# qcraftai/pillarnext

Hardware: AMD Instinct MI355X
Metric: frames/s PillarNeXt-B nuScenes 300k-pt cloud (inference, end-to-end) (higher is better)
Workload: dtype bf16

## Files before the change

include/pnx.h:

```cpp
#ifndef PNX_H
#define PNX_H

#include <stddef.h>
#include <stdint.h>

#ifdef __cplusplus
extern "C" {
#endif

typedef void* pnx_stream_t;

typedef enum pnx_status {
  PNX_OK = 0,
  PNX_ERR_INVALID = -1,
  PNX_ERR_UNSUPPORTED = -2,
  PNX_ERR_WORKSPACE = -3,
  PNX_ERR_HIP = -4
} pnx_status;

typedef enum pnx_dtype { PNX_F32 = 0, PNX_BF16 = 1, PNX_F16 = 2 } pnx_dtype;
typedef enum pnx_layout {
  PNX_NHWC = 0,
  PNX_NCHW = 1
} pnx_layout;

typedef struct pnx_geom {
  float pc_min[3];
  float voxel[3];
  int32_t gx, gy;
} pnx_geom;

const char* pnx_last_error(void);
const char* pnx_version(void);

int pnx_geom_init(const double* pc_range6_host, const double* voxel_size3_host, pnx_geom* geom_host);

#define PNX_PFN_FOLDED_FLOATS(F) (32 * ((F) + 5) + 32 + 64 * 64 + 64 + 64 * 121 + 64 * 71)

int pnx_pfn_fold_bn(int32_t num_point_features,
                    const float* w0, const float* gamma0, const float* beta0, const float* mean0, const float* var0,
                    const float* w1, const float* gamma1, const float* beta1, const float* mean1, const float* var1,
                    float eps, float* folded_out, pnx_stream_t stream);

size_t pnx_reader_workspace_bytes(int64_t n_points, int32_t batch, const pnx_geom* geom_host);

int pnx_reader_forward(const float* points, int64_t n_points, int32_t row_stride, int32_t batch, const pnx_geom* geom_host,
                       const float* pfn_folded, void* canvas, int32_t canvas_dtype, int32_t canvas_layout, uint8_t* occupancy,
                       float* feat_max, int32_t* coords, int64_t pillar_capacity, int64_t* unq_inv, int32_t* pillar_of_point,
                       int32_t* counts, void* workspace, size_t workspace_bytes, pnx_stream_t stream);

void pnx_reader_fill_split(int32_t* percent3_host);

int pnx_profile_begin(int32_t max_samples);
int pnx_profile_end(float* reader_us_avg_host, float* canvas_us_avg_host, int32_t* samples_host);
float pnx_profile_last_pfn_us(void);
float pnx_profile_last_voxelize_us(void);

size_t pnx_pfn_train_param_floats(int32_t num_point_features);
size_t pnx_pfn_train_partial_floats(int32_t num_point_features, int32_t which);
int pnx_pfn_forward_train(int32_t pass, const float* points, int64_t n_points, int32_t row_stride, int32_t batch, const pnx_geom* geom_host,
                          const float* params, float* partials, float* feat_max, int64_t pillar_capacity, int32_t* coords,
                          int32_t* pillar_of_point, int32_t* counts, void* workspace, size_t workspace_bytes, pnx_stream_t stream);
int pnx_pfn_backward(int32_t pass, int64_t n_points, int32_t row_stride, int32_t batch, const pnx_geom* geom_host, const float* params,
                     const float* grad_feat_max, const float* feat_max, float* partials, void* workspace, size_t workspace_bytes,
                     pnx_stream_t stream);

int pnx_voxelize(const float* points, int64_t n_points, int32_t row_stride, int32_t batch, const pnx_geom* geom_host,
                 float* features, int32_t* coords, int64_t pillar_capacity, int64_t* unq_inv, int32_t* pillar_of_point,
                 int32_t* counts, void* workspace, size_t workspace_bytes, pnx_stream_t stream);

typedef enum pnx_group_mode { PNX_GROUP_VOXEL = 0, PNX_GROUP_PILLAR_CLAMP = 1, PNX_GROUP_CYLINDER_CLAMP = 2 } pnx_group_mode;
typedef struct pnx_group_geom {
  float min[3], voxel[3];
  int32_t grid[3];
  int32_t mode;
  int32_t prefilter;
  float keep_min[3], keep_max[3];
} pnx_group_geom;
size_t pnx_group_workspace_bytes(int64_t n_points, int32_t row_stride, int32_t batch, const pnx_group_geom* geom_host);
int pnx_group_points(const float* points, int64_t n_points, int32_t row_stride, int32_t batch, const pnx_group_geom* geom_host, float* point_features,
                     int32_t feature_ld, int32_t* coords, int64_t group_capacity, int64_t* unq_inv, float* group_mean, int32_t* counts, void* workspace,
                     size_t workspace_bytes, pnx_stream_t stream);
int pnx_pfn_layer_eval(const float* xa, int32_t lda, int32_t ca, const float* gb, int32_t cb, const int64_t* inv, const float* wt, const float* shift,
                       int32_t cout, int64_t n, int64_t num_groups, float* y, int32_t ldy, float* gmax, pnx_stream_t stream);
int pnx_bilinear_gather(const void* image, int32_t dtype, int32_t batch, int32_t h, int32_t w, int32_t channels, const float* pos, int32_t pos_ld,
                        const float* pos_min2_host, const float* pos_voxel2_host, const int32_t* cell_coords, const int64_t* unq_inv, int32_t ds_rate,
                        int64_t n, float* out, int32_t out_ld, pnx_stream_t stream);
size_t pnx_bilinear_gather_backward_workspace_bytes(int64_t n, int32_t batch, int32_t h, int32_t w);
int pnx_bilinear_gather_backward(const float* grad_out, int32_t grad_ld, int32_t batch, int32_t h, int32_t w, int32_t channels, const float* pos,
                                 int32_t pos_ld, const float* pos_min2_host, const float* pos_voxel2_host, const int32_t* cell_coords,
                                 const int64_t* unq_inv, int32_t ds_rate, int64_t n, float* grad_image, void* workspace, size_t workspace_bytes,
                                 pnx_stream_t stream);

size_t pnx_scatter_max_workspace_bytes(int64_t n, int64_t num_pillars);
int pnx_scatter_max(const float* x, const int64_t* index, int64_t n, int32_t channels, int64_t num_pillars, float* out,
                    int64_t* argmax, void* workspace, size_t workspace_bytes, pnx_stream_t stream);
int pnx_scatter_max_backward(const float* grad_out, const int64_t* argmax, int64_t n, int32_t channels, int64_t num_pillars,
                             float* grad_x, pnx_stream_t stream);

size_t pnx_point_layer_workspace_bytes(int64_t n, int32_t cin, int32_t cout, int32_t backward);
int pnx_point_layer_stats(const float* x, int32_t ldx, int64_t n, int32_t cin, const float* w, int32_t cout, double* sums, void* workspace,
                          size_t workspace_bytes, pnx_stream_t stream);
int pnx_point_layer_forward(const float* x, int32_t ldx, int64_t n, int32_t cin, const float* w, int32_t cout, const float* prm, const int64_t* inv,
                            int64_t num_groups, float* y, int32_t ldy, float* gmax, int64_t* argmax, pnx_stream_t stream);
int pnx_point_layer_backward_stats(const float* x, int32_t ldx, int64_t n, int32_t cin, const float* w, int32_t cout, const float* prm, const float* dy,
                                   int32_t lddy, const int64_t* inv, int64_t num_groups, const float* dgmax, const int64_t* argmax, double* sums,
                                   void* workspace, size_t workspace_bytes, pnx_stream_t stream);
int pnx_point_layer_backward(const float* x, int32_t ldx, int64_t n, int32_t cin, const float* w, int32_t cout, const float* prm, const float* dy,
                             int32_t lddy, const int64_t* inv, int64_t num_groups, const float* dgmax, const int64_t* argmax, float* dx, int32_t lddx,
                             float* dw, void* workspace, size_t workspace_bytes, pnx_stream_t stream);

int pnx_scatter_canvas(const float* feat_max, const int32_t* coords, const int32_t* num_pillars_dev, int64_t pillar_capacity,
                       int32_t batch, int32_t gy, int32_t gx, void* canvas, int32_t canvas_dtype, int32_t canvas_layout,
                       pnx_stream_t stream);

size_t pnx_merge_sweeps_desc_bytes(void);
size_t pnx_merge_sweeps_workspace_bytes(int64_t n_raw);
int pnx_merge_sweeps(const float* raw, int64_t n_raw, int32_t raw_stride, int32_t n_copy, const void* seg_descs_dev, int32_t n_segments, float* out,
                     int32_t* n_out_dev, void* workspace, size_t workspace_bytes, pnx_stream_t stream);

int pnx_bias_act_mask(const void* x, const void* residual, const float* bias, const uint8_t* mask, void* out, int64_t sites,
                      int32_t channels, int32_t dtype, int32_t relu, pnx_stream_t stream);
int pnx_sum_bias_act(const void* const* srcs, int32_t n_src, const float* bias, void* out, int64_t sites, int32_t channels, int32_t dtype,
                     int32_t relu, pnx_stream_t stream);
int pnx_deconv2x2_bf16(const void* x, const void* wfrag, const float* bias, void* y, int32_t batch, int32_t h, int32_t w, int32_t cin, int32_t cout,
                       int32_t relu, pnx_stream_t stream);
int pnx_deconv2x2_f16(const void* x, const void* wfrag, const float* bias, void* y, int32_t batch, int32_t h, int32_t w, int32_t cin, int32_t cout,
                       int32_t relu, pnx_stream_t stream);
int pnx_conv3x3_bf16(const void* x, const void* wfrag, const float* bias, const void* residual, const uint8_t* mask, void* y, int32_t batch,
                     int32_t h, int32_t w, int32_t cin, int32_t cout, int32_t stride, int32_t relu, uint8_t* row_dirty, const int32_t* tile_list,
                     const int32_t* tile_count, pnx_stream_t stream);
int pnx_conv3x3_f16(const void* x, const void* wfrag, const float* bias, const void* residual, const uint8_t* mask, void* y, int32_t batch,
                    int32_t h, int32_t w, int32_t cin, int32_t cout, int32_t stride, int32_t relu, uint8_t* row_dirty, const int32_t* tile_list,
                    const int32_t* tile_count, pnx_stream_t stream);
size_t pnx_conv3x3_wgrad_workspace_bytes(int32_t cin, int32_t cout);
int pnx_conv3x3_wgrad_bf16(const void* x, const void* dy, const uint8_t* mask, float* dw, int32_t batch, int32_t h, int32_t w, int32_t cin, int32_t cout,
                           int32_t stride, void* workspace, size_t workspace_bytes, pnx_stream_t stream);
int pnx_conv3x3_wgrad_x3(const void* x_hi, const void* x_lo, const void* dy_hi, const void* dy_lo, const uint8_t* mask, float* dw, int32_t batch, int32_t h,
                         int32_t w, int32_t cin, int32_t cout, int32_t stride, void* workspace, size_t workspace_bytes, pnx_stream_t stream);
int pnx_conv3x3_wgrad_x6(const void* x_hi, const void* x_mid, const void* x_lo, const void* dy_hi, const void* dy_mid, const void* dy_lo, const uint8_t* mask,
                         float* dw, int32_t batch, int32_t h, int32_t w, int32_t cin, int32_t cout, int32_t stride, void* workspace, size_t workspace_bytes,
                         pnx_stream_t stream);
int pnx_conv3x3_pack_weights(const void* w, int32_t dtype, int32_t cout, int32_t cin, int32_t transposed, void* wfrag, pnx_stream_t stream);
int pnx_conv3x3_tile_rows(int32_t cin, int32_t cout, int32_t stride);
int pnx_conv_tile_list(const uint8_t* mask, const uint8_t* const* row_dirty, int32_t n_dirty, int32_t batch, int32_t h, int32_t w, int32_t tile_rows,
                       int32_t* tile_list, int32_t* tile_count, pnx_stream_t stream);
int pnx_sephead_out_bf16(const void* x, const void* wfrag, const float* bias, void* y, int32_t batch, int32_t h, int32_t w, int32_t n_branch,
                         pnx_stream_t stream);
int pnx_sephead_out_f16(const void* x, const void* wfrag, const float* bias, void* y, int32_t batch, int32_t h, int32_t w, int32_t n_branch,
                         pnx_stream_t stream);
typedef struct {
  const void* up;
  const void* wfrag1;
  const float* bias1;
  const float* w2c;
  const float* bias2;
  int32_t h, w;
} PnxLazyTask;
int pnx_sephead_lazy_bf16(const PnxLazyTask* tasks, int32_t n_tasks, const int32_t* class_task, int32_t nc_total, int32_t batch, const int64_t* local,
                          const int32_t* seg_len, int32_t pre_max, float* out, pnx_stream_t stream);
int pnx_sephead_lazy_f16(const PnxLazyTask* tasks, int32_t n_tasks, const int32_t* class_task, int32_t nc_total, int32_t batch, const int64_t* local,
                          const int32_t* seg_len, int32_t pre_max, float* out, pnx_stream_t stream);
int pnx_split_f32(const float* x, void* hi, void* lo, int64_t n, const uint8_t* mask, int32_t channels, pnx_stream_t stream);
int pnx_conv3x3_x3(const void* x_hi, const void* x_lo, const void* wfrag_hi, const void* wfrag_lo, const float* bias, const uint8_t* mask, float* y,
                   int32_t batch, int32_t h, int32_t w, int32_t cin, int32_t cout, int32_t stride, pnx_stream_t stream);
int pnx_split3_f32(const float* x, void* hi, void* mid, void* lo, int64_t n, const uint8_t* mask, int32_t channels, pnx_stream_t stream);
int pnx_conv3x3_x6(const void* x_hi, const void* x_mid, const void* x_lo, const void* wfrag_hi, const void* wfrag_mid, const void* wfrag_lo, const float* bias,
                   const uint8_t* mask, float* y, int32_t batch, int32_t h, int32_t w, int32_t cin, int32_t cout, int32_t stride, pnx_stream_t stream);
int pnx_conv3x3_dgrad_s2_bf16(const void* g, const void* wfrag_t, const uint8_t* mask_in, void* dx, int32_t batch, int32_t h, int32_t w, int32_t cin,
                              int32_t cout, pnx_stream_t stream);
int pnx_conv3x3_dgrad_s2_x3(const void* g_hi, const void* g_lo, const void* wfrag_t_hi, const void* wfrag_t_lo, const uint8_t* mask_in, float* dx, int32_t batch,
                            int32_t h, int32_t w, int32_t cin, int32_t cout, pnx_stream_t stream);
int pnx_conv3x3_dgrad_s2_x6(const void* g_hi, const void* g_mid, const void* g_lo, const void* wfrag_t_hi, const void* wfrag_t_mid, const void* wfrag_t_lo,
                            const uint8_t* mask_in, float* dx, int32_t batch, int32_t h, int32_t w, int32_t cin, int32_t cout, pnx_stream_t stream);
int pnx_conv3x3_smallk(const void* x, const float* weight, const float* bias, void* y, int32_t batch, int32_t h, int32_t w, int32_t cin, int32_t k,
                       int32_t dtype, pnx_stream_t stream);
size_t pnx_conv3x3_smallk_wgrad_workspace_bytes(int32_t k);
int pnx_conv3x3_smallk_wgrad(const void* x, const void* dy, float* dw, float* dbias, int32_t batch, int32_t h, int32_t w, int32_t cin, int32_t k,
                             int32_t dtype, void* workspace, size_t workspace_bytes, pnx_stream_t stream);
int pnx_mask_pool3(const uint8_t* mask_in, int32_t batch, int32_t h, int32_t w, int32_t stride, uint8_t* mask_out, pnx_stream_t stream);

int pnx_boxes_overlap_bev(const float* boxes_a, int64_t n, const float* boxes_b, int64_t m, float* out, pnx_stream_t stream);
int pnx_boxes_iou_bev(const float* boxes_a, int64_t n, const float* boxes_b, int64_t m, float* out, pnx_stream_t stream);
int pnx_boxes_aligned_overlap_bev(const float* boxes_a, const float* boxes_b, int64_t n, float* out, pnx_stream_t stream);
int pnx_boxes_aligned_iou3d(const float* boxes_a, const float* boxes_b, int64_t n, float* out, pnx_stream_t stream);

int pnx_boxes_iou_bev_cpu(const float* boxes_a_host, int64_t n, const float* boxes_b_host, int64_t m, float* out_host);
int pnx_boxes_aligned_iou_bev_cpu(const float* boxes_a_host, const float* boxes_b_host, int64_t n, float* out_host);
size_t pnx_nms_workspace_bytes(int64_t total_boxes, int32_t num_segments, int32_t max_seg_len);
int32_t pnx_debug_nms_pair_cap(int32_t cap);
int pnx_debug_detmath(const float* a, const float* b, int64_t n, float* sin_a, float* cos_a, float* atan2_ab, int32_t on_device, pnx_stream_t stream);
int pnx_nms_rotated_batched(const float* boxes, const int32_t* seg_offsets, const int32_t* seg_len, int32_t num_segments, int32_t max_seg_len,
                            const float* thresh, int32_t post_max, int32_t* keep, int32_t* keep_count, void* workspace,
                            size_t workspace_bytes, pnx_stream_t stream);
int pnx_nms_normal_batched(const float* boxes, const int32_t* seg_offsets, const int32_t* seg_len, int32_t num_segments, int32_t max_seg_len,
                           const float* thresh, int32_t post_max, int32_t* keep, int32_t* keep_count, void* workspace,
                           size_t workspace_bytes, pnx_stream_t stream);

size_t pnx_decode_task_desc_bytes(void);
size_t pnx_decode_topk_workspace_bytes(int64_t n_keys, int32_t num_segments);
int pnx_decode_topk(const uint64_t* keys, int64_t n_keys, int32_t num_segments, int32_t pre_max, uint64_t* sorted_keys, int64_t* order,
                    int64_t* seg_start, int32_t* seg_len, int32_t* seg_total, void* workspace, size_t workspace_bytes, pnx_stream_t stream);
int pnx_decode_keys(const void* packed, int32_t dtype, int32_t batch, int32_t n_classes_total, const void* task_desc_host, uint64_t* keys,
                    pnx_stream_t stream);
size_t pnx_sort_keys_workspace_bytes(int64_t n_keys);
int pnx_sort_keys(const uint64_t* keys, int64_t n_keys, int32_t num_segments, uint64_t* sorted_keys, int64_t* order, void* workspace,
                  size_t workspace_bytes, pnx_stream_t stream);
int pnx_decode_boxes(const void* const* task_ptrs_dev, const void* task_descs_dev, const int64_t* task_key_off_dev, int32_t n_tasks,
                     int32_t dtype, int32_t batch, const uint64_t* sorted_keys, const int64_t* order, const int64_t* seg_start,
                     const int32_t* seg_len, int32_t num_segments, int32_t pre_max, float* boxes9, float* boxes7, float* scores,
                     pnx_stream_t stream);
int pnx_decode_boxes_lazy(const void* task_descs_dev, const int64_t* task_key_off_dev, int32_t n_tasks, int32_t n_classes_total,
                          const uint64_t* sorted_keys, const int64_t* order, const int64_t* seg_start, int32_t* seg_len, const int32_t* seg_total,
                          int32_t num_segments, int32_t pre_max, const float* cand, float* boxes9, float* boxes7, float* scores, int32_t* flag_dev,
                          pnx_stream_t stream);
int pnx_gather_kept(const float* boxes9, const float* scores, const int32_t* keep, const int32_t* keep_count, int32_t num_segments,
                    int32_t pre_max, int32_t post_max, float* out, pnx_stream_t stream);

int32_t pnx_masked_bn_blocks(void);
int pnx_masked_bn_reduce(const float* partials, int32_t rows, int32_t cols, double* sums, pnx_stream_t stream);
int pnx_masked_bn_finalize(const double* sums, int32_t channels, const float* center, const float* weight, const float* bias, double eps, double momentum,
                           float* running_mean, float* running_var, int64_t* num_batches_tracked, float* mean, float* invstd, float* scale, float* shift,
                           float* count, pnx_stream_t stream);
int pnx_masked_bn_bwd_finalize(const double* sums_local, const double* sums_global, int32_t channels, const float* count, float* dgamma, float* dbeta,
                               float* mean_g, float* mean_gx, pnx_stream_t stream);
int pnx_masked_bn_stats(const void* x, int32_t dtype, const float* mask, int64_t n_sites, int32_t channels, const float* center, float* partials,
                        pnx_stream_t stream);
int pnx_masked_bn_apply(const void* x, const void* residual, int32_t dtype, const float* mask, int64_t n_sites, int32_t channels, const float* scale,
                        const float* shift, int32_t relu, void* y, pnx_stream_t stream);
int pnx_masked_bn_bwd_stats(const void* gy, const void* x, const void* residual, int32_t dtype, const float* mask, int64_t n_sites, int32_t channels,
                            const float* scale, const float* shift, const float* mean, const float* invstd, int32_t relu, float* partials,
                            pnx_stream_t stream);
int pnx_masked_bn_bwd_apply(const void* gy, const void* x, const void* residual, int32_t dtype, const float* mask, int64_t n_sites, int32_t channels,
                            const float* scale, const float* shift, const float* mean, const float* invstd, int32_t relu, const float* mean_g,
                            const float* mean_gx, void* dx, void* dresidual, pnx_stream_t stream);

size_t pnx_center_loss_workspace_bytes(int32_t batch, int32_t max_objs);
int pnx_center_loss_forward(const void* const* maps7, const float* hm_target, const int64_t* ind, const uint8_t* mask, const int64_t* cat,
                            const float* anno_box, const float* gt_boxes, int32_t batch, int32_t n_classes, int32_t h, int32_t w, int32_t max_objs,
                            const float* geom4_host, int32_t with_reg_iou, float* losses15, void* workspace, size_t workspace_bytes,
                            pnx_stream_t stream);
int pnx_center_loss_backward(const void* const* maps7, void* const* grads7, const float* hm_target, const int64_t* ind, const uint8_t* mask,
                             const int64_t* cat, const float* anno_box, const float* gt_boxes, int32_t batch, int32_t n_classes, int32_t h, int32_t w,
                             int32_t max_objs, const float* geom4_host, int32_t with_reg_iou, const float* losses15, const float* upstream13,
                             float* coef_scratch, void* workspace, size_t workspace_bytes, pnx_stream_t stream);

#define PNX_ASSIGN_MAX_TASKS 8
#define PNX_ASSIGN_MAX_CLASSES 32
typedef struct pnx_assign_desc {
  double lo[2];
  double voxel[2];
  double overlap;
  int32_t min_radius, max_objs, n_tasks, n_classes;
  int32_t osf[PNX_ASSIGN_MAX_TASKS], h[PNX_ASSIGN_MAX_TASKS], w[PNX_ASSIGN_MAX_TASKS], ncls[PNX_ASSIGN_MAX_TASKS];
  int32_t class_task[PNX_ASSIGN_MAX_CLASSES], class_cls[PNX_ASSIGN_MAX_CLASSES];
} pnx_assign_desc;
size_t pnx_assign_workspace_bytes(int32_t batch, int32_t n_tasks, int32_t max_objs);
int pnx_assign_labels(const float* gt_boxes, const int32_t* gt_cls, const int32_t* num_gt, int32_t batch, int32_t k, const pnx_assign_desc* desc_host,
                      float* const* hm_host, float* const* anno_box_host, int64_t* const* ind_host, uint8_t* const* mask_host, int64_t* const* cat_host,
                      float* const* gt_boxes_out_host, int32_t* counts, void* workspace, size_t workspace_bytes, pnx_stream_t stream);

enum { PNX_OP_MASK_POOL3 = 1, PNX_OP_TILE_LIST = 2, PNX_OP_CONV3X3 = 3, PNX_OP_DECONV2X2 = 4, PNX_OP_SEPHEAD_OUT = 5 };
typedef struct pnx_op {
  int32_t kind;
  int32_t i[9];
  const void* p[11];
} pnx_op;
int pnx_enqueue(const pnx_op* ops_host, int32_t n_ops, pnx_stream_t stream);
size_t pnx_op_bytes(void);

typedef struct pnx_lazy_decode {
  int32_t n_tasks, n_classes_total, batch, pre_max, post_max, dtype;
  const void* const* dense_host;
  const void* task_descs_host;
  const void* task_descs_dev;
  const int64_t* task_key_off_host;
  const int64_t* task_key_off_dev;
  const int64_t* list_key_off_dev;
  const PnxLazyTask* lazy_tasks_host;
  const int32_t* class_task_host;
  const int32_t* seg_off_dev;
// ... 89 lines not shown
```

pillarnext_amd/_lib.py:

```python
import ctypes
import os

_HERE = os.path.dirname(os.path.abspath(__file__))
LIB_PATH = os.environ.get("PNX_LIB") or os.path.join(_HERE, "libpnx_hip.so")

PNX_F32, PNX_BF16, PNX_F16 = 0, 1, 2
PNX_NHWC, PNX_NCHW = 0, 1


class PnxError(RuntimeError):
    pass


class PnxGeom(ctypes.Structure):
    _fields_ = [("pc_min", ctypes.c_float * 3), ("voxel", ctypes.c_float * 3), ("gx", ctypes.c_int32), ("gy", ctypes.c_int32)]


PNX_GROUP_VOXEL, PNX_GROUP_PILLAR_CLAMP, PNX_GROUP_CYLINDER_CLAMP = 0, 1, 2


class PnxGroupGeom(ctypes.Structure):
    _fields_ = [("min", ctypes.c_float * 3), ("voxel", ctypes.c_float * 3), ("grid", ctypes.c_int32 * 3), ("mode", ctypes.c_int32),
                ("prefilter", ctypes.c_int32), ("keep_min", ctypes.c_float * 3), ("keep_max", ctypes.c_float * 3)]


PNX_ASSIGN_MAX_TASKS, PNX_ASSIGN_MAX_CLASSES = 8, 32
PNX_PASTE_MAX_BOXES, PNX_PASTE_MAX_BATCH = 512, 64
PNX_AUG_ROTATE, PNX_AUG_SCALE, PNX_AUG_TRANSLATE, PNX_AUG_FLIP_X, PNX_AUG_FLIP_Y = 1, 2, 4, 8, 16


class PnxAssignDesc(ctypes.Structure):
    _fields_ = [("lo", ctypes.c_double * 2), ("voxel", ctypes.c_double * 2), ("overlap", ctypes.c_double), ("min_radius", ctypes.c_int32),
                ("max_objs", ctypes.c_int32), ("n_tasks", ctypes.c_int32), ("n_classes", ctypes.c_int32)] + \
               [(k, ctypes.c_int32 * PNX_ASSIGN_MAX_TASKS) for k in ("osf", "h", "w", "ncls")] + \
               [(k, ctypes.c_int32 * PNX_ASSIGN_MAX_CLASSES) for k in ("class_task", "class_cls")]


_vp = ctypes.c_void_p
_i64 = ctypes.c_int64
_i32 = ctypes.c_int32
_f32 = ctypes.c_float
_sz = ctypes.c_size_t
_i3p = ctypes.POINTER(ctypes.c_int32)

PROTOTYPES = {
    "pnx_last_error": (ctypes.c_char_p, []),
    "pnx_version": (ctypes.c_char_p, []),
    "pnx_geom_init": (ctypes.c_int, [ctypes.POINTER(ctypes.c_double), ctypes.POINTER(ctypes.c_double), ctypes.POINTER(PnxGeom)]),
    "pnx_pfn_fold_bn": (ctypes.c_int, [_i32] + [_vp] * 10 + [_f32, _vp, _vp]),
    "pnx_reader_workspace_bytes": (_sz, [_i64, _i32, ctypes.POINTER(PnxGeom)]),
    "pnx_reader_forward": (ctypes.c_int, [_vp, _i64, _i32, _i32, ctypes.POINTER(PnxGeom), _vp, _vp, _i32, _i32, _vp, _vp, _vp, _i64, _vp, _vp,
                                          _vp, _vp, _sz, _vp]),
    "pnx_reader_fill_split": (None, [ctypes.POINTER(ctypes.c_int32)]),
    "pnx_profile_begin": (ctypes.c_int, [_i32]),
    "pnx_profile_end": (ctypes.c_int, [ctypes.POINTER(ctypes.c_float), ctypes.POINTER(ctypes.c_float), ctypes.POINTER(ctypes.c_int32)]),
    "pnx_profile_last_pfn_us": (ctypes.c_float, []),
    "pnx_profile_last_voxelize_us": (ctypes.c_float, []),
    "pnx_pfn_train_param_floats": (_sz, [_i32]),
    "pnx_pfn_train_partial_floats": (_sz, [_i32, _i32]),
    "pnx_pfn_forward_train": (ctypes.c_int, [_i32, _vp, _i64, _i32, _i32, ctypes.POINTER(PnxGeom), _vp, _vp, _vp, _i64, _vp, _vp, _vp, _vp, _sz, _vp]),
    "pnx_pfn_backward": (ctypes.c_int, [_i32, _i64, _i32, _i32, ctypes.POINTER(PnxGeom), _vp, _vp, _vp, _vp, _vp, _sz, _vp]),
    "pnx_voxelize": (ctypes.c_int, [_vp, _i64, _i32, _i32, ctypes.POINTER(PnxGeom), _vp, _vp, _i64, _vp, _vp, _vp, _vp, _sz, _vp]),
    "pnx_group_workspace_bytes": (_sz, [_i64, _i32, _i32, ctypes.POINTER(PnxGroupGeom)]),
    "pnx_group_points": (ctypes.c_int, [_vp, _i64, _i32, _i32, ctypes.POINTER(PnxGroupGeom), _vp, _i32, _vp, _i64, _vp, _vp, _vp, _vp, _sz, _vp]),
    "pnx_pfn_layer_eval": (ctypes.c_int, [_vp, _i32, _i32, _vp, _i32, _vp, _vp, _vp, _i32, _i64, _i64, _vp, _i32, _vp, _vp]),
    "pnx_bilinear_gather": (ctypes.c_int, [_vp, _i32, _i32, _i32, _i32, _i32, _vp, _i32, ctypes.POINTER(ctypes.c_float), ctypes.POINTER(ctypes.c_float), _vp,
                                           _vp, _i32, _i64, _vp, _i32, _vp]),
    "pnx_bilinear_gather_backward_workspace_bytes": (_sz, [_i64, _i32, _i32, _i32]),
    "pnx_bilinear_gather_backward": (ctypes.c_int, [_vp, _i32, _i32, _i32, _i32, _i32, _vp, _i32, ctypes.POINTER(ctypes.c_float),
                                                    ctypes.POINTER(ctypes.c_float), _vp, _vp, _i32, _i64, _vp, _vp, _sz, _vp]),
    "pnx_scatter_max_workspace_bytes": (_sz, [_i64, _i64]),
    "pnx_scatter_max": (ctypes.c_int, [_vp, _vp, _i64, _i32, _i64, _vp, _vp, _vp, _sz, _vp]),
    "pnx_scatter_max_backward": (ctypes.c_int, [_vp, _vp, _i64, _i32, _i64, _vp, _vp]),
    "pnx_point_layer_workspace_bytes": (_sz, [_i64, _i32, _i32, _i32]),
    "pnx_point_layer_stats": (ctypes.c_int, [_vp, _i32, _i64, _i32, _vp, _i32, _vp, _vp, _sz, _vp]),
    "pnx_point_layer_forward": (ctypes.c_int, [_vp, _i32, _i64, _i32, _vp, _i32, _vp, _vp, _i64, _vp, _i32, _vp, _vp, _vp]),
    "pnx_point_layer_backward_stats": (ctypes.c_int, [_vp, _i32, _i64, _i32, _vp, _i32, _vp, _vp, _i32, _vp, _i64, _vp, _vp, _vp, _vp, _sz, _vp]),
    "pnx_point_layer_backward": (ctypes.c_int, [_vp, _i32, _i64, _i32, _vp, _i32, _vp, _vp, _i32, _vp, _i64, _vp, _vp, _vp, _i32, _vp, _vp, _sz, _vp]),
    "pnx_scatter_canvas": (ctypes.c_int, [_vp, _vp, _vp, _i64, _i32, _i32, _i32, _vp, _i32, _i32, _vp]),
    "pnx_merge_sweeps_desc_bytes": (_sz, []),
    "pnx_merge_sweeps_workspace_bytes": (_sz, [_i64]),
    "pnx_merge_sweeps": (ctypes.c_int, [_vp, _i64, _i32, _i32, _vp, _i32, _vp, _vp, _vp, _sz, _vp]),
    "pnx_bias_act_mask": (ctypes.c_int, [_vp, _vp, _vp, _vp, _vp, _i64, _i32, _i32, _i32, _vp]),
    "pnx_sum_bias_act": (ctypes.c_int, [_vp, _i32, _vp, _vp, _i64, _i32, _i32, _i32, _vp]),
    "pnx_deconv2x2_bf16": (ctypes.c_int, [_vp, _vp, _vp, _vp, _i32, _i32, _i32, _i32, _i32, _i32, _vp]),
    "pnx_deconv2x2_f16": (ctypes.c_int, [_vp, _vp, _vp, _vp, _i32, _i32, _i32, _i32, _i32, _i32, _vp]),
    "pnx_sephead_out_bf16": (ctypes.c_int, [_vp, _vp, _vp, _vp, _i32, _i32, _i32, _i32, _vp]),
    "pnx_sephead_out_f16": (ctypes.c_int, [_vp, _vp, _vp, _vp, _i32, _i32, _i32, _i32, _vp]),
    "pnx_masked_bn_blocks": (_i32, []),
    "pnx_masked_bn_reduce": (ctypes.c_int, [_vp, _i32, _i32, _vp, _vp]),
    "pnx_masked_bn_finalize": (ctypes.c_int, [_vp, _i32, _vp, _vp, _vp, ctypes.c_double, ctypes.c_double, _vp, _vp, _vp, _vp, _vp, _vp, _vp, _vp, _vp]),
    "pnx_masked_bn_bwd_finalize": (ctypes.c_int, [_vp, _vp, _i32, _vp, _vp, _vp, _vp, _vp, _vp]),
    "pnx_masked_bn_stats": (ctypes.c_int, [_vp, _i32, _vp, _i64, _i32, _vp, _vp, _vp]),
    "pnx_masked_bn_apply": (ctypes.c_int, [_vp, _vp, _i32, _vp, _i64, _i32, _vp, _vp, _i32, _vp, _vp]),
    "pnx_masked_bn_bwd_stats": (ctypes.c_int, [_vp, _vp, _vp, _i32, _vp, _i64, _i32, _vp, _vp, _vp, _vp, _i32, _vp, _vp]),
    "pnx_masked_bn_bwd_apply": (ctypes.c_int, [_vp, _vp, _vp, _i32, _vp, _i64, _i32, _vp, _vp, _vp, _vp, _i32, _vp, _vp, _vp, _vp, _vp]),
    "pnx_sephead_lazy_bf16": (ctypes.c_int, [_vp, _i32, _vp, _i32, _i32, _vp, _vp, _i32, _vp, _vp]),
    "pnx_sephead_lazy_f16": (ctypes.c_int, [_vp, _i32, _vp, _i32, _i32, _vp, _vp, _i32, _vp, _vp]),
    "pnx_conv3x3_bf16": (ctypes.c_int, [_vp, _vp, _vp, _vp, _vp, _vp, _i32, _i32, _i32, _i32, _i32, _i32, _i32, _vp, _vp, _vp, _vp]),
    "pnx_conv3x3_f16": (ctypes.c_int, [_vp, _vp, _vp, _vp, _vp, _vp, _i32, _i32, _i32, _i32, _i32, _i32, _i32, _vp, _vp, _vp, _vp]),
    "pnx_conv3x3_tile_rows": (ctypes.c_int, [_i32, _i32, _i32]),
    "pnx_conv3x3_pack_weights": (ctypes.c_int, [_vp, _i32, _i32, _i32, _i32, _vp, _vp]),
    "pnx_conv3x3_wgrad_workspace_bytes": (_sz, [_i32, _i32]),
    "pnx_conv3x3_wgrad_bf16": (ctypes.c_int, [_vp, _vp, _vp, _vp, _i32, _i32, _i32, _i32, _i32, _i32, _vp, _sz, _vp]),
    "pnx_conv3x3_wgrad_x3": (ctypes.c_int, [_vp, _vp, _vp, _vp, _vp, _vp, _i32, _i32, _i32, _i32, _i32, _i32, _vp, _sz, _vp]),
    "pnx_conv3x3_wgrad_x6": (ctypes.c_int, [_vp, _vp, _vp, _vp, _vp, _vp, _vp, _vp, _i32, _i32, _i32, _i32, _i32, _i32, _vp, _sz, _vp]),
    "pnx_conv3x3_dgrad_s2_bf16": (ctypes.c_int, [_vp, _vp, _vp, _vp, _i32, _i32, _i32, _i32, _i32, _vp]),
    "pnx_conv3x3_dgrad_s2_x3": (ctypes.c_int, [_vp, _vp, _vp, _vp, _vp, _vp, _i32, _i32, _i32, _i32, _i32, _vp]),
    "pnx_conv3x3_dgrad_s2_x6": (ctypes.c_int, [_vp, _vp, _vp, _vp, _vp, _vp, _vp, _vp, _i32, _i32, _i32, _i32, _i32, _vp]),
    "pnx_conv3x3_smallk": (ctypes.c_int, [_vp, _vp, _vp, _vp, _i32, _i32, _i32, _i32, _i32, _i32, _vp]),
    "pnx_conv3x3_smallk_wgrad_workspace_bytes": (_sz, [_i32]),
    "pnx_conv3x3_smallk_wgrad": (ctypes.c_int, [_vp, _vp, _vp, _vp, _i32, _i32, _i32, _i32, _i32, _i32, _vp, _sz, _vp]),
    "pnx_conv_tile_list": (ctypes.c_int, [_vp, _vp, _i32, _i32, _i32, _i32, _i32, _vp, _vp, _vp]),
    "pnx_mask_pool3": (ctypes.c_int, [_vp, _i32, _i32, _i32, _i32, _vp, _vp]),
    "pnx_split_f32": (ctypes.c_int, [_vp, _vp, _vp, _i64, _vp, _i32, _vp]),
    "pnx_conv3x3_x3": (ctypes.c_int, [_vp, _vp, _vp, _vp, _vp, _vp, _vp, _i32, _i32, _i32, _i32, _i32, _i32, _vp]),
    "pnx_split3_f32": (ctypes.c_int, [_vp, _vp, _vp, _vp, _i64, _vp, _i32, _vp]),
    "pnx_conv3x3_x6": (ctypes.c_int, [_vp, _vp, _vp, _vp, _vp, _vp, _vp, _vp, _vp, _i32, _i32, _i32, _i32, _i32, _i32, _vp]),
    "pnx_decode_task_desc_bytes": (_sz, []),
    "pnx_decode_topk_workspace_bytes": (_sz, [_i64, _i32]),
    "pnx_decode_topk": (ctypes.c_int, [_vp, _i64, _i32, _i32, _vp, _vp, _vp, _vp, _vp, _vp, _sz, _vp]),
    "pnx_decode_keys": (ctypes.c_int, [_vp, _i32, _i32, _i32, _vp, _vp, _vp]),
    "pnx_sort_keys_workspace_bytes": (ctypes.c_size_t, [_i64]),
    "pnx_sort_keys": (ctypes.c_int, [_vp, _i64, _i32, _vp, _vp, _vp, ctypes.c_size_t, _vp]),
    "pnx_decode_boxes": (ctypes.c_int, [_vp, _vp, _vp, _i32, _i32, _i32, _vp, _vp, _vp, _vp, _i32, _i32, _vp, _vp, _vp, _vp]),
    "pnx_decode_boxes_lazy": (ctypes.c_int, [_vp, _vp, _i32, _i32, _vp, _vp, _vp, _vp, _vp, _i32, _i32, _vp, _vp, _vp, _vp, _vp, _vp]),
    "pnx_gather_kept": (ctypes.c_int, [_vp, _vp, _vp, _vp, _i32, _i32, _i32, _vp, _vp]),
    "pnx_enqueue": (ctypes.c_int, [_vp, _i32, _vp]),
    "pnx_decode_lazy_enqueue": (ctypes.c_int, [_vp, _vp]),
    "pnx_op_bytes": (_sz, []),
    "pnx_lazy_decode_bytes": (_sz, []),
    "pnx_center_loss_workspace_bytes": (_sz, [_i32, _i32]),
    "pnx_center_loss_forward": (ctypes.c_int, [_vp, _vp, _vp, _vp, _vp, _vp, _vp, _i32, _i32, _i32, _i32, _i32, _vp, _i32, _vp, _vp, _sz, _vp]),
    "pnx_center_loss_backward": (ctypes.c_int, [_vp, _vp, _vp, _vp, _vp, _vp, _vp, _vp, _i32, _i32, _i32, _i32, _i32, _vp, _i32, _vp, _vp, _vp, _vp, _sz, _vp]),
    "pnx_assign_workspace_bytes": (_sz, [_i32, _i32, _i32]),
    "pnx_assign_labels": (ctypes.c_int, [_vp, _vp, _vp, _i32, _i32, ctypes.POINTER(PnxAssignDesc), _vp, _vp, _vp, _vp, _vp, _vp, _vp, _vp, _sz, _vp]),
    "pnx_paste_chunk_rows": (_i32, []),
    "pnx_paste_select": (ctypes.c_int, [_vp, _vp, _vp, _i32, _i32, _i32, _vp, _vp, _vp, _vp, _i32, _i32, _vp, _i32, _vp, _vp, _vp, _vp, _vp, _vp, _vp]),
    "pnx_paste_augment_workspace_bytes": (_sz, [_i64, _i32]),
    "pnx_paste_augment_points": (ctypes.c_int, [_vp, _i64, _i32, _i32, _vp, _vp, _vp, _vp, _i32, _i32, _vp, _vp, _i32, _i64, _vp, _vp, _i64, _vp, _vp, _vp,
                                                _sz, _vp]),
    "pnx_augment_boxes": (ctypes.c_int, [_vp, _vp, _i32, _i32, _i32, _vp, _vp]),
    "pnx_boxes_overlap_bev": (ctypes.c_int, [_vp, _i64, _vp, _i64, _vp, _vp]),
    "pnx_boxes_iou_bev": (ctypes.c_int, [_vp, _i64, _vp, _i64, _vp, _vp]),
    "pnx_boxes_aligned_overlap_bev": (ctypes.c_int, [_vp, _vp, _i64, _vp, _vp]),
    "pnx_boxes_aligned_iou3d": (ctypes.c_int, [_vp, _vp, _i64, _vp, _vp]),
    "pnx_boxes_iou_bev_cpu": (ctypes.c_int, [_vp, _i64, _vp, _i64, _vp]),
    "pnx_boxes_aligned_iou_bev_cpu": (ctypes.c_int, [_vp, _vp, _i64, _vp]),
    "pnx_nms_workspace_bytes": (_sz, [_i64, _i32, _i32]),
    "pnx_debug_nms_pair_cap": (_i32, [_i32]),
    "pnx_debug_detmath": (ctypes.c_int, [_vp, _vp, _i64, _vp, _vp, _vp, _i32, _vp]),
    "pnx_nms_rotated_batched": (ctypes.c_int, [_vp, _vp, _vp, _i32, _i32, _vp, _i32, _vp, _vp, _vp, _sz, _vp]),
    "pnx_nms_normal_batched": (ctypes.c_int, [_vp, _vp, _vp, _i32, _i32, _vp, _i32, _vp, _vp, _vp, _sz, _vp]),
    "pnx_sp3_index_bytes": (_sz, [_i32, _i3p]),
    "pnx_sp3_index_build": (ctypes.c_int, [_vp, _i64, _i32, _i3p, _vp, _sz, _vp, _vp, _vp]),
    "pnx_sp3_out_grid": (ctypes.c_int, [_i32, _i3p, _i3p, _i3p, _i3p, _i3p]),
    "pnx_sp3_out_index": (ctypes.c_int, [_vp, _i64, _i32, _i3p, _i3p, _i3p, _i3p, _vp, _sz, _vp, _vp]),
    "pnx_sp3_index_coords": (ctypes.c_int, [_vp, _sz, _i32, _i3p, _vp, _i64, _vp]),
    "pnx_sp3_neighbor_map": (ctypes.c_int, [_vp, _i64, _vp, _sz, _i32, _i3p, _vp, _i3p, _i3p, _i3p, _vp, _vp]),
    "pnx_sp3_packed_weight_floats": (_sz, [_i32, _i32, _i32]),
    "pnx_sp3_conv": (ctypes.c_int, [_vp, _i64, _i32, _vp, _i64, _i32, _vp, _vp, _vp, _i32, _vp, _i32, _vp]),
    "pnx_sp3_conv_train": (ctypes.c_int, [_vp, _i64, _i32, _vp, _i64, _i32, _vp, _vp, _vp, _i32, _vp, _i32, _vp]),
    "pnx_sp3_dense": (ctypes.c_int, [_vp, _vp, _i64, _i32, _i32, _i3p, _vp, _vp]),
    "pnx_sp3_packed_weight_halfs": (_sz, [_i32, _i32, _i32]),
    "pnx_sp3_conv_h": (ctypes.c_int, [_vp, _i64, _i32, _i32, _vp, _i64, _i32, _vp, _vp, _vp, _i32, _vp, _i32, _i32, _i32, _vp]),
    "pnx_sp3_dense_h": (ctypes.c_int, [_vp, _i32, _vp, _i64, _i32, _i32, _i32, _i3p, _vp, _vp]),
    "pnx_sp3_transpose_map": (ctypes.c_int, [_vp, _i64, _i32, _i64, _vp, _vp]),
    "pnx_sp3_wgrad_workspace_bytes": (_sz, [_i64, _i32, _i32, _i32]),
    "pnx_sp3_wgrad": (ctypes.c_int, [_vp, _i64, _i32, _vp, _i32, _vp, _i64, _i32, _vp, _vp, _sz, _vp]),
    "pnx_sp3_conv_h_f32": (ctypes.c_int, [_vp, _i64, _i32, _i32, _vp, _i64, _i32, _vp, _vp, _i32, _i32, _vp]),
    "pnx_sp3_wgrad_h_partials_bytes": (_sz, [_i64, _i32, _i32, _i32]),
    "pnx_sp3_wgrad_h": (ctypes.c_int, [_vp, _i64, _i32, _i32, _vp, _i32, _i32, _vp, _i64, _i32, _vp, _i32, _vp, _sz, _vp]),
    "pnx_sp3_dense_backward": (ctypes.c_int, [_vp, _vp, _i64, _i32, _i32, _i3p, _vp, _vp]),
    "pnx_sp3_bn_split": (ctypes.c_int, [_i64, _i32, _i3p]),
    "pnx_sp3_bn_partials_bytes": (_sz, [_i64, _i32, _i32]),
    "pnx_sp3_bn_stats": (ctypes.c_int, [_vp, _i64, _i32, _vp, _vp, _sz, _vp]),
    "pnx_sp3_bn_apply": (ctypes.c_int, [_vp, _i64, _i32, _vp, _vp, _vp, _i32, _i32, _vp, _vp, _i32, _vp]),
    "pnx_sp3_bn_bwd_stats": (ctypes.c_int, [_vp, _vp, _vp, _i32, _i64, _i32, _vp, _vp, _vp, _vp, _i32, _vp, _sz, _vp]),
    "pnx_sp3_bn_bwd_apply": (ctypes.c_int, [_vp, _vp, _vp, _i32, _i64, _i32, _vp, _vp, _vp, _vp, _i32, _vp, _vp, _vp, _vp, _vp]),
}

_LIB = None


def lib():
    global _LIB
    if _LIB is None:
        if not os.path.exists(LIB_PATH):
            raise PnxError(f"{LIB_PATH} is missing: run `python -m pillarnext_amd.build` (hipcc, gfx950). "
                           "There is no CPU fallback for the product path.")
        L = ctypes.CDLL(LIB_PATH)
        for name, (res, args) in PROTOTYPES.items():
            fn = getattr(L, name)
            fn.restype = res
            fn.argtypes = args
        _LIB = L
    return _LIB


def check(rc, what=""):
    if rc != 0:
        msg = lib().pnx_last_error().decode(errors="replace")
        raise PnxError(f"{what} failed with status {rc}: {msg}")


def make_geom(pc_range, voxel_size):
    pr = (ctypes.c_double * 6)(*[float(v) for v in pc_range])
    vs = (ctypes.c_double * 3)(*[float(v) for v in voxel_size])
    g = PnxGeom()
    check(lib().pnx_geom_init(pr, vs, ctypes.byref(g)), "pnx_geom_init")
    return g


def ptr(t):
    return None if t is None else ctypes.c_void_p(t.data_ptr())


def stream_ptr():
    import torch

    return ctypes.c_void_p(torch.cuda.current_stream().cuda_stream)
```

pillarnext_amd/csrc/conv3x3.hip:

```cpp
#include "pnx_common.h"

namespace {

#include "conv_tile.h"

template <int CIN, int COUT, int STRIDE, bool W_LDS>
__global__ __launch_bounds__(256, 2) void k_conv3x3(const uint16_t* __restrict__ x, const uint4* __restrict__ wfrag,
                                                 const float* __restrict__ bias, const uint16_t* __restrict__ res,
                                                 const uint8_t* __restrict__ mask, uint16_t* __restrict__ y, int B, int H, int W, int Ho,
                                                 int Wo, int relu, uint8_t* __restrict__ row_dirty) {
  constexpr int CB = CIN / 16, MT = COUT / 32, KSTEPS = 9 * CB;
  constexpr int NT = (MT <= 2) ? 4 : 2;
  extern __shared__ uint4 s_w[];
  const int lane = threadIdx.x & 63, wv = threadIdx.x >> 6;
  const int px = lane & 31, kb = lane >> 5;
  if (W_LDS) {
    for (int i = threadIdx.x; i < KSTEPS * MT * 64; i += 256) s_w[i] = wfrag[i];
    __syncthreads();
  }
  const int tiles_x = (Wo + 31) >> 5, tiles_y = (Ho + NT - 1) / NT;
  const int64_t n_tiles = (int64_t)B * tiles_y * tiles_x;
  for (int64_t tile = (int64_t)blockIdx.x * 4 + wv; tile < n_tiles; tile += (int64_t)gridDim.x * 4) {
    const int tx = (int)(tile % tiles_x);
    const int ty = (int)((tile / tiles_x) % tiles_y);
    const int b = (int)(tile / ((int64_t)tiles_x * tiles_y));
    const int ox = tx * 32 + px, oy0 = ty * NT;
    bool act[NT];
    bool any_row[NT];
    bool any = false;
#pragma unroll
    for (int j = 0; j < NT; j++) {
      const int oy = oy0 + j;
      const bool in = ox < Wo && oy < Ho;
      act[j] = in && (mask == nullptr || mask[((int64_t)b * Ho + oy) * Wo + ox] != 0);
      any_row[j] = __ballot(act[j]) != 0;
      any = any || any_row[j];
    }
    bool row_store[NT];
#pragma unroll
    for (int j = 0; j < NT; j++) {
      const int oy = oy0 + j;
      row_store[j] = oy < Ho;
      if (row_dirty != nullptr && oy < Ho) {
        uint8_t* d = row_dirty + ((int64_t)b * Ho + oy) * tiles_x + tx;
        const bool was = __builtin_amdgcn_readfirstlane((int)*d) != 0;
        row_store[j] = any_row[j] || was;
        if (lane == 0 && was != any_row[j]) *d = any_row[j] ? 1 : 0;
      }
    }
    v16f acc[NT][MT];
#pragma unroll
    for (int m = 0; m < MT; m++) {
      const v16f bq = bias_tile(bias, m * 32, kb);
#pragma unroll
      for (int j = 0; j < NT; j++) acc[j][m] = bq;
    }

    if (res != nullptr) {
#pragma unroll
      for (int j = 0; j < NT; j++) {
        const bool in = ox < Wo && oy0 + j < Ho;
        const uint16_t* rp = res + (in ? (((int64_t)b * Ho + oy0 + j) * Wo + ox) * COUT : 0);
#pragma unroll
        for (int m0 = 0; m0 < MT; m0 += 2) {
          uint4 rq[2][2];
          load_residual(rq, rp + m0 * 32, act[j], kb);
          v16f a2[2] = {acc[j][m0], acc[j][m0 + 1]};
          add_residual(a2, rq);
          acc[j][m0] = a2[0], acc[j][m0 + 1] = a2[1];
        }
      }
    }

    if (any) {
      for (int tap = 0; tap < 9; tap++) {
        const int dy = tap / 3 - 1, dx = tap % 3 - 1;
        const uint16_t* src[NT];
        bool ok[NT];
#pragma unroll
        for (int j = 0; j < NT; j++) {
          const int iy = (oy0 + j) * STRIDE + dy, ix = ox * STRIDE + dx;
          ok[j] = any_row[j] && ox < Wo && (oy0 + j) < Ho && iy >= 0 && iy < H && ix >= 0 && ix < W;
          src[j] = x + (((int64_t)b * H + (ok[j] ? iy : 0)) * W + (ok[j] ? ix : 0)) * CIN + 8 * kb;
        }
#pragma unroll
        for (int cb = 0; cb < CB; cb++) {
          const int ks = tap * CB + cb;
          el8 af[MT];
#pragma unroll
          for (int m = 0; m < MT; m++) {
            const uint4 wq = W_LDS ? s_w[(ks * MT + m) * 64 + lane] : wfrag[(ks * MT + m) * 64 + lane];
            af[m] = __builtin_bit_cast(el8, wq);
          }
#pragma unroll
          for (int j = 0; j < NT; j++) {
            if (!any_row[j]) continue;
            uint4 q = make_uint4(0, 0, 0, 0);
            if (ok[j]) q = *reinterpret_cast<const uint4*>(src[j] + cb * 16);
            const el8 bfr = __builtin_bit_cast(el8, q);
#pragma unroll
            for (int m = 0; m < MT; m++) acc[j][m] = PNX_MFMA32(af[m], bfr, acc[j][m]);
          }
        }
      }
    }
    const int n_valid = Wo - tx * 32;
#pragma unroll
    for (int j = 0; j < NT; j++) {
      const bool row_in = row_store[j];
      if (!row_in) continue;
      uint16_t* row = y + (((int64_t)b * Ho + (oy0 + j)) * Wo + tx * 32) * COUT;
#pragma unroll
      for (int m0 = 0; m0 < MT; m0 += 2) {
        uint4 R[4];
#pragma unroll
        for (int m = 0; m < 2; m++) {
          uint4 pk[2];
          pack_tile(acc[j][m0 + m], act[j], relu, pk);
          R[2 * m] = pk[0], R[2 * m + 1] = pk[1];
        }
        transpose_row64(R, lane);
        store_row64<COUT>(R, row + m0 * 32, row_in ? n_valid : 0, lane);
      }
    }
  }
}

#include "conv_taps.h"
#include "conv_rows.h"
#include "conv_s2.h"
#include "sephead.h"

struct DirtySet {
  const uint8_t* p[4];
};
__global__ __launch_bounds__(256) void k_tile_list(const uint8_t* __restrict__ mask, DirtySet ds, int B, int H, int W, int th, int32_t* __restrict__ list,
                                                   int32_t* __restrict__ count) {
  __shared__ int s_wave[4];
  __shared__ int s_base;
  const int t = threadIdx.x, lane = t & 63, wv = t >> 6;
  const int tiles_x = (W + 31) >> 5, tiles_y = (H + th - 1) / th;
  const int64_t n_tiles = (int64_t)B * tiles_y * tiles_x;
  const int r = lane & 15;
  const int64_t tile = ((int64_t)blockIdx.x * 4 + wv) * 4 + (lane >> 4);
  uint32_t acc = 0;
  if (tile < n_tiles && r < th) {
    const int tx = (int)(tile % tiles_x);
    const int ty = (int)((tile / tiles_x) % tiles_y);
    const int b = (int)(tile / ((int64_t)tiles_x * tiles_y));
    const int x0 = tx * 32, oy = ty * th + r;
    if (oy < H) {
      const uint8_t* row = mask + ((int64_t)b * H + oy) * W + x0;
      if ((W & 15) == 0 && x0 + 32 <= W) {
        const uint4 a = reinterpret_cast<const uint4*>(row)[0], c = reinterpret_cast<const uint4*>(row)[1];
        acc |= a.x | a.y | a.z | a.w | c.x | c.y | c.z | c.w;
      } else {
        for (int k = 0; k < 32 && x0 + k < W; k++) acc |= row[k];
      }
#pragma unroll
      for (int k = 0; k < 4; k++)
        if (ds.p[k] != nullptr) acc |= ds.p[k][((int64_t)b * H + oy) * tiles_x + tx];
    }
  }
  acc |= (uint32_t)__shfl_xor((int)acc, 1);
  acc |= (uint32_t)__shfl_xor((int)acc, 2);
  acc |= (uint32_t)__shfl_xor((int)acc, 4);
  acc |= (uint32_t)__shfl_xor((int)acc, 8);
  const bool any = acc != 0 && r == 0 && tile < n_tiles;
  const unsigned long long bal = __ballot(any);
  if (lane == 0) s_wave[wv] = __popcll(bal);
  __syncthreads();
  if (t == 0) {
    const int tot = s_wave[0] + s_wave[1] + s_wave[2] + s_wave[3];
    s_base = tot > 0 ? atomicAdd(count, tot) : 0;
  }
  __syncthreads();
  if (any) {
    int off = s_base + __popcll(bal & ((1ull << lane) - 1ull));
    for (int w = 0; w < wv; w++) off += s_wave[w];
    list[off] = (int32_t)tile;
  }
}

template <int COUT>
int launch_lds(const ConvArgs& a) {
  constexpr int TH = LDS_TH;
  const int64_t n_tiles = (int64_t)a.B * ((a.H + TH - 1) / TH) * ((a.W + 31) / 32);
  int64_t nb = n_tiles;
  const int64_t cap = 256 * 2;
  if (nb > cap) nb = cap;
  const int slot = a.mask != nullptr ? next_sched_slot() : -1;
  if constexpr (COUT == 64) {
    if (a.res != nullptr) {
      k_conv3x3_lds<COUT, true><<<(unsigned)nb, 256, 0, a.st>>>(a.x, a.wfrag, a.bias, a.res, a.mask, a.y, a.B, a.H, a.W, a.relu, a.row_dirty, slot, a.tlist,
                                                               a.tcount);
      PNX_LAUNCH_CHECK();
      return PNX_OK;
    }
  } else {
    PNX_REQUIRE(a.res == nullptr, PNX_ERR_UNSUPPORTED, "residual with %d output channels", COUT);
  }
  k_conv3x3_lds<COUT, false><<<(unsigned)nb, 256, 0, a.st>>>(a.x, a.wfrag, a.bias, nullptr, a.mask, a.y, a.B, a.H, a.W, a.relu, a.row_dirty, slot, a.tlist,
                                                            a.tcount);
  PNX_LAUNCH_CHECK();
  return PNX_OK;
}

#include "conv_pc.h"

template <int CIN, int COUT, int STRIDE>
int launch(const ConvArgs& a, int Ho, int Wo) {
  constexpr size_t wbytes = (size_t)9 * (CIN / 16) * (COUT / 32) * 64 * 16;
  constexpr bool W_LDS = wbytes <= 76 * 1024;
  constexpr int NT = (COUT / 32 <= 2) ? 4 : 2;
  const int64_t n_tiles = (int64_t)a.B * ((Ho + NT - 1) / NT) * ((Wo + 31) / 32);
  int64_t nb = (n_tiles + 3) / 4;
  if (nb > 512) nb = 512;
  constexpr auto kern = k_conv3x3<CIN, COUT, STRIDE, W_LDS>;
  if (W_LDS) {
    if (const int rc = pnx_lds_optin<kern>(wbytes); rc != PNX_OK) return rc;
  }
  kern<<<(unsigned)nb, 256, W_LDS ? wbytes : 0, a.st>>>(a.x, a.wfrag, a.bias, a.res, a.mask, a.y, a.B, a.H, a.W, Ho, Wo, a.relu, a.row_dirty);
  PNX_LAUNCH_CHECK();
  return PNX_OK;
}

}

extern "C" {

#if defined(PNX_CONV_TIMERS) && !defined(PNX_CONV_F16)
int pnx_debug_conv_timers(unsigned long long* out) {
  unsigned long long z[8] = {0, 0, 0, 0, 0, 0, 0, 0};
  PNX_CHECK_HIP(hipDeviceSynchronize());
  PNX_CHECK_HIP(hipMemcpyFromSymbol(out, HIP_SYMBOL(g_conv_T), sizeof(z)));
  PNX_CHECK_HIP(hipMemcpyToSymbol(HIP_SYMBOL(g_conv_T), z, sizeof(z)));
  return PNX_OK;
}
#endif

int PNX_CONV_FN(pnx_sephead_out)(const void* x, const void* wfrag, const float* bias, void* y, int32_t batch, int32_t h, int32_t w, int32_t n_branch,
                         pnx_stream_t stream) {
  PNX_REQUIRE(x && wfrag && bias && y && batch > 0 && h > 0 && w > 0, PNX_ERR_INVALID, "bad arguments");
  PNX_REQUIRE((((uintptr_t)x | (uintptr_t)y | (uintptr_t)wfrag | (uintptr_t)bias) & 15) == 0, PNX_ERR_INVALID, "16-byte alignment required");
  hipStream_t st = (hipStream_t)stream;
  switch (n_branch) {
    case 1: return launch_sephead<1>(x, wfrag, bias, y, batch, h, w, st);
    case 2: return launch_sephead<2>(x, wfrag, bias, y, batch, h, w, st);
    case 5: return launch_sephead<5>(x, wfrag, bias, y, batch, h, w, st);
    case 6: return launch_sephead<6>(x, wfrag, bias, y, batch, h, w, st);
    case 7: return launch_sephead<7>(x, wfrag, bias, y, batch, h, w, st);
    default: break;
  }
  pnx_set_error("pnx_sephead_out: no kernel for %d branches", n_branch);
  return PNX_ERR_UNSUPPORTED;
}

int PNX_CONV_FN(pnx_deconv2x2)(const void* x, const void* wfrag, const float* bias, void* y, int32_t batch, int32_t h, int32_t w, int32_t cin, int32_t cout,
                       int32_t relu, pnx_stream_t stream) {
  PNX_REQUIRE(x && wfrag && bias && y && batch > 0 && h > 0 && w > 0, PNX_ERR_INVALID, "bad arguments");
  PNX_REQUIRE((((uintptr_t)x | (uintptr_t)y | (uintptr_t)wfrag | (uintptr_t)bias) & 15) == 0, PNX_ERR_INVALID, "16-byte alignment required");
  if (cin != 64 || cout != 64) {
    pnx_set_error("pnx_deconv2x2: no kernel for %d -> %d channels", cin, cout);
    return PNX_ERR_UNSUPPORTED;
  }
  const int64_t n_seg = (int64_t)batch * h * ((w + 31) / 32);
  int64_t nb = (n_seg + 3) / 4;
  if (nb > 512) nb = 512;
  k_deconv2x2_64<<<(unsigned)nb, 256, 0, (hipStream_t)stream>>>((const uint16_t*)x, (const uint4*)wfrag, bias, (uint16_t*)y, batch, h, w, relu);
  PNX_LAUNCH_CHECK();
  return PNX_OK;
}

#ifndef PNX_CONV_F16
int pnx_conv3x3_tile_rows(int32_t cin, int32_t cout, int32_t stride) {
  if (stride != 1) return 0;
  if (cin == 64 && (cout == 64 || cout == 320 || cout == 384 || cout == 448)) return LDS_TH;
  if ((cin == 128 && cout == 128) || (cin == 256 && (cout == 256 || cout == 64))) return L128_TH;
  return 0;
}

static int conv_tile_list_impl(const uint8_t* mask, const uint8_t* const* row_dirty, int32_t n_dirty, int32_t batch, int32_t h, int32_t w, int32_t tile_rows,
                               int32_t* tile_list, int32_t* tile_count, pnx_stream_t stream, bool zero_count) {
  PNX_REQUIRE(mask && tile_list && tile_count && batch > 0 && h > 0 && w > 0 && tile_rows > 0, PNX_ERR_INVALID, "bad arguments");
  PNX_REQUIRE(n_dirty >= 0 && n_dirty <= 4 && (n_dirty == 0 || row_dirty != nullptr), PNX_ERR_INVALID, "0..4 row_dirty arrays");
  DirtySet ds;
  for (int k = 0; k < 4; k++) ds.p[k] = k < n_dirty ? row_dirty[k] : nullptr;
  hipStream_t st = (hipStream_t)stream;
  if (zero_count) PNX_CHECK_HIP(hipMemsetAsync(tile_count, 0, sizeof(int32_t), st));
  const int64_t n_tiles = (int64_t)batch * ((h + tile_rows - 1) / tile_rows) * ((w + 31) / 32);
  PNX_REQUIRE(tile_rows <= 16, PNX_ERR_UNSUPPORTED, "tile_rows %d (at most 16: one lane per row)", tile_rows);
  k_tile_list<<<(unsigned)((n_tiles + 15) / 16), 256, 0, st>>>(mask, ds, batch, h, w, tile_rows, tile_list, tile_count);
  PNX_LAUNCH_CHECK();
  return PNX_OK;
}
int pnx_conv_tile_list(const uint8_t* mask, const uint8_t* const* row_dirty, int32_t n_dirty, int32_t batch, int32_t h, int32_t w, int32_t tile_rows,
                       int32_t* tile_list, int32_t* tile_count, pnx_stream_t stream) {
  return conv_tile_list_impl(mask, row_dirty, n_dirty, batch, h, w, tile_rows, tile_list, tile_count, stream, true);
}
int pnx_conv_tile_list_prezeroed(const uint8_t* mask, const uint8_t* const* row_dirty, int32_t n_dirty, int32_t batch, int32_t h, int32_t w, int32_t tile_rows,
                                 int32_t* tile_list, int32_t* tile_count, pnx_stream_t stream) {
  return conv_tile_list_impl(mask, row_dirty, n_dirty, batch, h, w, tile_rows, tile_list, tile_count, stream, false);
}

#endif

int PNX_CONV_FN(pnx_conv3x3)(const void* x, const void* wfrag, const float* bias, const void* residual, const uint8_t* mask, void* y, int32_t batch,
                     int32_t h, int32_t w, int32_t cin, int32_t cout, int32_t stride, int32_t relu, uint8_t* row_dirty, const int32_t* tile_list,
                     const int32_t* tile_count, pnx_stream_t stream) {
  PNX_REQUIRE((tile_list == nullptr) == (tile_count == nullptr), PNX_ERR_INVALID, "tile_list and tile_count come together");
  PNX_REQUIRE(tile_list == nullptr || (mask != nullptr && pnx_conv3x3_tile_rows(cin, cout, stride) > 0), PNX_ERR_INVALID,
              "a tile list needs a mask and a kernel that takes one (pnx_conv3x3_tile_rows)");
  PNX_REQUIRE(x && wfrag && bias && y && batch > 0 && h > 0 && w > 0, PNX_ERR_INVALID, "bad arguments");
  PNX_REQUIRE(stride == 1 || stride == 2, PNX_ERR_UNSUPPORTED, "stride %d", stride);
  PNX_REQUIRE(row_dirty == nullptr || mask != nullptr, PNX_ERR_INVALID, "row_dirty needs an active-site mask");
  PNX_REQUIRE((((uintptr_t)x | (uintptr_t)y | (uintptr_t)wfrag | (uintptr_t)bias | (uintptr_t)residual) & 15) == 0, PNX_ERR_INVALID,
              "16-byte alignment required");
  const int ho = (h + 2 - 3) / stride + 1, wo = (w + 2 - 3) / stride + 1;
  hipStream_t st = (hipStream_t)stream;
  const ConvArgs a = {(const uint16_t*)x, (const uint4*)wfrag, bias, (const uint16_t*)residual, mask, (uint16_t*)y, batch, h, w, relu, row_dirty, tile_list,
                      tile_count, st};
  if (stride == 1 && getenv("PNX_CONV_DIRECT") == nullptr) {
    static const int pc_mode = getenv("PNX_CONV_PC") != nullptr ? atoi(getenv("PNX_CONV_PC")) : 1;
    static const int pack_mode = getenv("PNX_CONV_PACK") != nullptr ? atoi(getenv("PNX_CONV_PACK")) : 3;
    if (pc_mode != 0) {
      if (cin == 64 && cout == 64) return launch_pc<64, 64>(a, (pack_mode & 2) != 0);
      if (residual == nullptr && (pc_mode & 4)) {
        if (cin == 64 && cout == 320) return launch_pc<64, 320>(a);
        if (cin == 64 && cout == 384) return launch_pc<64, 384>(a);
        if (cin == 64 && cout == 448) return launch_pc<64, 448>(a);
      }
      if (pc_mode & 2) {
        if (cin == 128 && cout == 128) return launch_pc<128, 128>(a);
        if (cin == 256 && cout == 256) return launch_pc<256, 256>(a);
      }
    }
    if (cin == 64 && cout == 64) return launch_lds<64>(a);
    const bool pack = (pack_mode & 1) != 0;
    if (cin == 128 && cout == 128) return launch_ldsx<128, 128>(a, pack);
    if (cin == 256 && cout == 64) return launch_ldsx<256, 64>(a);
    if (cin == 256 && cout == 256) return launch_ldsx<256, 256>(a, pack);
    if (cin == 64 && cout == 384) return launch_lds<384>(a);
    if (cin == 64 && cout == 320) return launch_lds<320>(a);
    if (cin == 64 && cout == 448) return launch_lds<448>(a);
  }
  if (stride == 2 && residual == nullptr && getenv("PNX_CONV_DIRECT") == nullptr) {
    if (cin == 64 && cout == 128) return launch_s2<64, 128, 1>(x, wfrag, bias, mask, y, batch, h, w, ho, wo, relu, row_dirty, st);
    if (cin == 128 && cout == 256) return launch_s2<128, 256, 1>(x, wfrag, bias, mask, y, batch, h, w, ho, wo, relu, row_dirty, st);
    if (cin == 256 && cout == 256) return launch_s2<256, 256, 1>(x, wfrag, bias, mask, y, batch, h, w, ho, wo, relu, row_dirty, st);
  }
#define PNX_CONV_CASE(CI, CO)                             \
  if (cin == CI && cout == CO) {                          \
    if (stride == 1) return launch<CI, CO, 1>(a, ho, wo); \
    return launch<CI, CO, 2>(a, ho, wo);                  \
  }
  PNX_CONV_CASE(64, 64)
  PNX_CONV_CASE(64, 128)
  PNX_CONV_CASE(128, 128)
#undef PNX_CONV_CASE
  pnx_set_error("pnx_conv3x3: no kernel for %d -> %d channels", cin, cout);
  return PNX_ERR_UNSUPPORTED;
}

#ifndef PNX_CONV_F16
}
namespace {
#include "conv_dgrad_s2.h"

template <int NP>
int dgrad_s2_impl(const char* name, PnxPieces<NP> g, PnxPieces<NP> wfrag_t, const uint8_t* mask_in, void* dx, int32_t batch, int32_t h, int32_t w, int32_t cin,
                  int32_t cout, pnx_stream_t stream) {
  PNX_REQUIRE(g.complete() && wfrag_t.complete() && mask_in && dx && batch > 0 && h > 0 && w > 0, PNX_ERR_INVALID, "%s: bad arguments", name);
  PNX_REQUIRE(((g.bits() | wfrag_t.bits() | (uintptr_t)dx) & 15) == 0, PNX_ERR_INVALID, "16-byte alignment required");
  hipStream_t st = (hipStream_t)stream;
  if (cin == 64 && cout == 128) return launch_dgrad_s2<128, 64, NP>(g, wfrag_t, mask_in, dx, batch, h, w, st);
  if (cin == 128 && cout == 256) return launch_dgrad_s2<256, 128, NP>(g, wfrag_t, mask_in, dx, batch, h, w, st);
  if (cin == 256 && cout == 256) return launch_dgrad_s2<256, 256, NP>(g, wfrag_t, mask_in, dx, batch, h, w, st);
  pnx_set_error("%s: no kernel for %d -> %d channels", name, cin, cout);
  return PNX_ERR_UNSUPPORTED;
}

template <int NP>
int conv3x3_f32_impl(const char* name, PnxPieces<NP> x, PnxPieces<NP> wfrag, const float* bias, const uint8_t* mask, float* y, int32_t batch, int32_t h, int32_t w,
                     int32_t cin, int32_t cout, int32_t stride, pnx_stream_t stream) {
  PNX_REQUIRE(x.complete() && wfrag.complete() && y, PNX_ERR_INVALID, "null pointer");
  PNX_REQUIRE(batch > 0 && h > 0 && w > 0, PNX_ERR_INVALID, "bad shape");
  PNX_REQUIRE(stride == 1 || stride == 2, PNX_ERR_UNSUPPORTED, "stride %d", stride);
  PNX_REQUIRE(((x.bits() | wfrag.bits() | (uintptr_t)y | (uintptr_t)bias) & 15) == 0, PNX_ERR_INVALID, "16-byte alignment required");
  hipStream_t st = (hipStream_t)stream;
  if (stride == 1) {
    if (cin == 64 && cout == 64) return launch_pc_f32<64, 64, NP>(x, wfrag, bias, mask, y, batch, h, w, st);
    if (cin == 128 && cout == 128) return launch_pc_f32<128, 128, NP>(x, wfrag, bias, mask, y, batch, h, w, st);
    if (cin == 256 && cout == 256) return launch_pc_f32<256, 256, NP>(x, wfrag, bias, mask, y, batch, h, w, st);
  } else {
    const int ho = (h - 1) / 2 + 1, wo = (w - 1) / 2 + 1;
    if (cin == 64 && cout == 128) return launch_s2<64, 128, NP>(x, wfrag, bias, mask, y, batch, h, w, ho, wo, 0, nullptr, st);
    if (cin == 128 && cout == 256) return launch_s2<128, 256, NP>(x, wfrag, bias, mask, y, batch, h, w, ho, wo, 0, nullptr, st);
    if (cin == 256 && cout == 256) return launch_s2<256, 256, NP>(x, wfrag, bias, mask, y, batch, h, w, ho, wo, 0, nullptr, st);
  }
  pnx_set_error("%s: no kernel for %d -> %d channels, stride %d", name, cin, cout, stride);
  return PNX_ERR_UNSUPPORTED;
}

}
extern "C" {

int pnx_conv3x3_dgrad_s2_bf16(const void* g, const void* wfrag_t, const uint8_t* mask_in, void* dx, int32_t batch, int32_t h, int32_t w, int32_t cin, int32_t cout,
                              pnx_stream_t stream) {
  return dgrad_s2_impl<1>("pnx_conv3x3_dgrad_s2_bf16", {g}, {wfrag_t}, mask_in, dx, batch, h, w, cin, cout, stream);
}

int pnx_conv3x3_dgrad_s2_x3(const void* g_hi, const void* g_lo, const void* wfrag_t_hi, const void* wfrag_t_lo, const uint8_t* mask_in, float* dx, int32_t batch,
                            int32_t h, int32_t w, int32_t cin, int32_t cout, pnx_stream_t stream) {
  return dgrad_s2_impl<2>("pnx_conv3x3_dgrad_s2_x3", {g_hi, g_lo}, {wfrag_t_hi, wfrag_t_lo}, mask_in, dx, batch, h, w, cin, cout, stream);
}

int pnx_conv3x3_dgrad_s2_x6(const void* g_hi, const void* g_mid, const void* g_lo, const void* wfrag_t_hi, const void* wfrag_t_mid, const void* wfrag_t_lo,
                            const uint8_t* mask_in, float* dx, int32_t batch, int32_t h, int32_t w, int32_t cin, int32_t cout, pnx_stream_t stream) {
  return dgrad_s2_impl<3>("pnx_conv3x3_dgrad_s2_x6", {g_hi, g_mid, g_lo}, {wfrag_t_hi, wfrag_t_mid, wfrag_t_lo}, mask_in, dx, batch, h, w, cin, cout, stream);
}

int pnx_conv3x3_x3(const void* x_hi, const void* x_lo, const void* wfrag_hi, const void* wfrag_lo, const float* bias, const uint8_t* mask, float* y,
                   int32_t batch, int32_t h, int32_t w, int32_t cin, int32_t cout, int32_t stride, pnx_stream_t stream) {
  return conv3x3_f32_impl<2>("pnx_conv3x3_x3", {x_hi, x_lo}, {wfrag_hi, wfrag_lo}, bias, mask, y, batch, h, w, cin, cout, stride, stream);
}

int pnx_conv3x3_x6(const void* x_hi, const void* x_mid, const void* x_lo, const void* wfrag_hi, const void* wfrag_mid, const void* wfrag_lo, const float* bias,
                   const uint8_t* mask, float* y, int32_t batch, int32_t h, int32_t w, int32_t cin, int32_t cout, int32_t stride, pnx_stream_t stream) {
  return conv3x3_f32_impl<3>("pnx_conv3x3_x6", {x_hi, x_mid, x_lo}, {wfrag_hi, wfrag_mid, wfrag_lo}, bias, mask, y, batch, h, w, cin, cout, stride, stream);
}
#endif

}

namespace {

constexpr int kLzG = 32, kLzN = kLzG * 9, kLzNT = kLzN / 32;
constexpr int kLzPatch = kLzG * 25 * 8;
constexpr int kLzW2 = 10 * 9 * 32 * 3;
constexpr int kLzMaxTasks = 8, kLzMaxClasses = 32;
constexpr int kLzAhead = 2;

#include "sephead_lazy.h"

}

extern "C" int PNX_CONV_FN(pnx_sephead_lazy)(const PnxLazyTask* tasks, int32_t n_tasks, const int32_t* class_task, int32_t nc_total, int32_t batch,
                                     const int64_t* local, const int32_t* seg_len, int32_t pre_max, float* out, pnx_stream_t stream) {
  PNX_REQUIRE(tasks && class_task && local && seg_len && out && batch > 0 && pre_max > 0, PNX_ERR_INVALID, "bad arguments");
  PNX_REQUIRE(n_tasks >= 1 && n_tasks <= kLzMaxTasks && nc_total >= 1 && nc_total <= kLzMaxClasses, PNX_ERR_UNSUPPORTED, "at most 8 tasks / 32 classes");
  LazyArgs a;
  for (int i = 0; i < n_tasks; i++) {
    const PnxLazyTask& s = tasks[i];
    PNX_REQUIRE(s.up && s.wfrag1 && s.bias1 && s.w2c && s.bias2 && s.h > 0 && s.w > 0, PNX_ERR_INVALID, "bad task");
    PNX_REQUIRE((int64_t)batch * s.h * s.w < ((int64_t)1 << 31), PNX_ERR_UNSUPPORTED, "map too large for 32-bit cell indices");
    PNX_REQUIRE((((uintptr_t)s.up | (uintptr_t)s.wfrag1 | (uintptr_t)s.w2c) & 15) == 0, PNX_ERR_INVALID, "16-byte alignment required");
    a.t[i] = LazyTaskDev{(const uint16_t*)s.up, (const uint4*)s.wfrag1, s.bias1, s.w2c, s.bias2, s.h, s.w};
  }
  for (int c = 0; c < nc_total; c++) {
    PNX_REQUIRE(class_task[c] >= 0 && class_task[c] < n_tasks, PNX_ERR_INVALID, "class_task out of range");
    a.class_task[c] = (signed char)class_task[c];
  }
  a.nc_total = nc_total, a.pre_max = pre_max, a.bps = (pre_max + kLzG - 1) / kLzG;
  if (const int rc = pnx_lds_optin<&k_sephead_lazy>(kLzLds); rc != PNX_OK) return rc;
  const unsigned nb = (unsigned)((int64_t)batch * nc_total * a.bps);
  k_sephead_lazy<<<nb, 512, kLzLds, (hipStream_t)stream>>>(a, local, seg_len, out);
  PNX_LAUNCH_CHECK();
  return PNX_OK;
}
```

pillarnext_amd/csrc/conv_pc.h:

```cpp
#pragma once

__device__ __forceinline__ void pc_barrier_lds() { asm volatile("s_waitcnt lgkmcnt(0)\n\ts_barrier" ::: "memory"); }
__device__ __forceinline__ void pc_barrier_all() { asm volatile("s_waitcnt vmcnt(0) lgkmcnt(0)\n\ts_barrier" ::: "memory"); }

#ifdef PNX_CONV_TIMERS
#define PC_T_DECL unsigned long long pc_T[8] = {0, 0, 0, 0, 0, 0, 0, 0}; unsigned long long pc_tk = __builtin_amdgcn_s_memtime();
#define PC_TOCK(k)                                               \
  {                                                              \
    const unsigned long long _n = __builtin_amdgcn_s_memtime();  \
    pc_T[k] += _n - pc_tk;                                       \
    pc_tk = _n;                                                  \
  }
#define PC_T_FLUSH                                                   \
  if ((threadIdx.x & 63) == 0) {                                     \
    for (int k = 0; k < 8; k++) atomicAdd(&g_conv_T[k], pc_T[k]);    \
  }
#else
#define PC_T_DECL
#define PC_TOCK(k)
#define PC_T_FLUSH
#endif

template <int NR, int CIN, int COUT, bool HAS_RES, int NRG, int NSLOT, int SLOT_N, int NP = 1>
__device__ __forceinline__ void pc_rows(const uint4* __restrict__ s_ring, int& g, const uint4* __restrict__ wfrag, const uint4* __restrict__ wfrag2,
// ... 14 lines not shown
#pragma unroll 1
  for (int pass = 0; pass < NPASS; pass++) {
    const int mt = pass * NCG + cg;
    v16f acc[NRA][1];
    if (NR > 0) {
      v16f bq;
      if (F32 && bias == nullptr) {
#pragma unroll
        for (int i = 0; i < 16; i++) bq[i] = 0.f;
      } else {
        bq = bias_tile(bias, mt * 32, kb);
      }
#pragma unroll
      for (int j = 0; j < NR; j++) acc[j][0] = bq;
    }
    uint4 rq[2];
#pragma unroll 1
    for (int sq = 0; sq < NSLAB * NP; sq++) {
      const int sl = F32 ? sq % NSLAB : sq;
      if (NR > 0) {
        if (HAS_RES && sl == NSLAB - 1) {
          const bool a0 = (rmask[0] >> px) & 1u;
          const char* rp = reinterpret_cast<const char*>(res_t + ((int64_t)rrow[0] * W) * COUT + mt * 32) + res_off;
#pragma unroll
          for (int t = 0; t < 2; t++) {
            rq[t] = make_uint4(0, 0, 0, 0);
            if (a0) rq[t] = *reinterpret_cast<const uint4*>(rp + 32 * t);
          }
        }
        if constexpr (NP == 3) {
          const int q = sq / NSLAB;
#pragma unroll 1
          for (int k = q; k >= 0; k--)
            conv_taps<NRA, MTALL, CB, 1, 1>(acc, s_ring + (g % NSLOT) * SLOT_N, k == 0 ? wfrag : k == 1 ? wfrag2 : wfrag3, rbase, mt, px, kb, lane, 4 * sl);
        } else {
          conv_taps<NRA, MTALL, CB, 1, 1>(acc, s_ring + (g % NSLOT) * SLOT_N, wfrag, rbase, mt, px, kb, lane, 4 * sl);
          if constexpr (X3) {
            if (sq < NSLAB) conv_taps<NRA, MTALL, CB, 1, 1>(acc, s_ring + (g % NSLOT) * SLOT_N, wfrag2, rbase, mt, px, kb, lane, 4 * sl);
          }
        }
      }
      PC_TOCK(1)
      if (F32 || NSLAB > 1 || pass == NPASS - 1) {
        pc_barrier_lds();
        g++;
      }
      PC_TOCK(2)
    }
    if (NR > 0) {
#pragma unroll
      for (int j = 0; j < NR; j++) {
        const bool act = (rmask[j] >> px) & 1u;
        if constexpr (F32) {
          store_tile_f32<COUT>(acc[j][0], act, reinterpret_cast<float*>(y_t) + ((int64_t)rrow[j] * W) * COUT + mt * 32, n_valid, px, kb);
          continue;
        }
        uint4 rc[2];
        if (HAS_RES) {
          rc[0] = rq[0], rc[1] = rq[1];
          if (j + 1 < NR) {
            const bool a1 = (rmask[j + 1] >> px) & 1u;
            const char* rp = reinterpret_cast<const char*>(res_t + ((int64_t)rrow[j + 1] * W) * COUT + mt * 32) + res_off;
#pragma unroll
            for (int t = 0; t < 2; t++) {
              rq[t] = make_uint4(0, 0, 0, 0);
              if (a1) rq[t] = *reinterpret_cast<const uint4*>(rp + 32 * t);
            }
          }
        }
        uint4 pk[2];
        pack_tile(acc[j][0], act, relu, pk, HAS_RES ? rc : nullptr);
        transpose_row32(pk, lane);
        store_row32<COUT>(pk, y_t + ((int64_t)rrow[j] * W) * COUT + mt * 32, n_valid, lane);
      }
    }
    PC_TOCK(3)
  }
}

__device__ __forceinline__ uint32_t pc_pix_off64(int code, int W) { return (uint32_t)(((code >> 5) * W + (code & 31)) * 64) * 2u; }

template <int NR, bool HAS_RES, int NSLOT, int SLOT_N>
__device__ __forceinline__ void pc_pix64(const uint4* __restrict__ s_ring, int& g, const uint4* __restrict__ wfrag, const float* __restrict__ bias,
                                         const uint16_t* __restrict__ res_t, uint16_t* __restrict__ y_t, const int (&codes)[2], const int (&n_g)[4], int W,
                                         int cg, int relu, int px, int kb, int lane
#ifdef PNX_CONV_TIMERS
                                         , unsigned long long (&pc_T)[8], unsigned long long& pc_tk
#endif
) {
  constexpr int NRA = NR > 0 ? NR : 1;
  v16f acc[NRA][1];
  uint4 rq[2];
  if (NR > 0) {
    const v16f bq = bias_tile(bias, cg * 32, kb);
#pragma unroll
    for (int j = 0; j < NR; j++) acc[j][0] = bq;
    auto code = [&](int j) { return (codes[j >> 1] >> (16 * (j & 1))) & 0xffff; };
    const char* const rp = reinterpret_cast<const char*>(res_t + cg * 32) + 16 * kb;
    if (HAS_RES) {
      const uint32_t o = pc_pix_off64(code(0), W);
#pragma unroll
      for (int t = 0; t < 2; t++) {
        rq[t] = make_uint4(0, 0, 0, 0);
        if (px < n_g[0]) rq[t] = *reinterpret_cast<const uint4*>(rp + o + 32 * t);
      }
    }
    const int cw[4] = {codes[0], codes[1], 0, 0};
    conv_taps<NRA, 2, 4, 1, 1, TAPS_WD, true, 16>(acc, s_ring + (g % NSLOT) * SLOT_N, wfrag, cw, cg, px, kb, lane, 0);
  }
  PC_TOCK(1)
  pc_barrier_lds();
  g++;
  PC_TOCK(2)
  if (NR > 0) {
    auto code = [&](int j) { return (codes[j >> 1] >> (16 * (j & 1))) & 0xffff; };
    const char* const rp = reinterpret_cast<const char*>(res_t + cg * 32) + 16 * kb;
    char* const yp = reinterpret_cast<char*>(y_t + cg * 32);
#pragma unroll
    for (int j = 0; j < NR; j++) {
      const bool act = px < n_g[j];
      uint4 rc[2];
      if (HAS_RES) {
        rc[0] = rq[0], rc[1] = rq[1];
        if (j + 1 < NR) {
          const uint32_t o = pc_pix_off64(code(j + 1), W);
#pragma unroll
          for (int t = 0; t < 2; t++) {
            rq[t] = make_uint4(0, 0, 0, 0);
            if (px < n_g[j + 1]) rq[t] = *reinterpret_cast<const uint4*>(rp + o + 32 * t);
          }
        }
      }
      uint4 pk[2];
      pack_tile(acc[j][0], act, relu, pk, HAS_RES ? rc : nullptr);
      transpose_row32(pk, lane);
      int l = lane;
      asm volatile("" : "+v"(l));
      const int cj = code(j);
#pragma unroll
      for (int d = 0; d < 2; d++) {
        const int P = 16 * d + (l >> 2);
        const int pc = __builtin_amdgcn_ds_bpermute(P << 2, cj);
        if (P < n_g[j]) *reinterpret_cast<uint4*>(yp + pc_pix_off64(pc, W) + (uint32_t)((l & 3) * 16)) = pk[d];
      }
    }
  }
  PC_TOCK(3)
}

template <int CIN, int COUT, bool HAS_RES, int NP = 1, bool PACK = false>
__global__ __launch_bounds__(768, 3) void k_conv3x3_pc(const uint16_t* __restrict__ x, const uint16_t* __restrict__ x2, const uint4* __restrict__ wfrag,
                                                       const uint4* __restrict__ wfrag2, const float* __restrict__ bias,
                                                       const uint16_t* __restrict__ res, const uint8_t* __restrict__ mask, uint16_t* __restrict__ y,
                                                       int B, int H, int W, int relu, uint8_t* __restrict__ row_dirty, int slot,
                                                       const int32_t* __restrict__ tlist, const int32_t* __restrict__ tcount,
                                                       const uint16_t* __restrict__ x3 = nullptr, const uint4* __restrict__ wfrag3 = nullptr) {
  constexpr bool X3 = NP == 2, F32 = NP > 1;
  constexpr int TH = CIN == 64 ? 16 : 8;
  constexpr int NRG = TH / 4, NCG = 8 / NRG, PASS_C = NCG * 32, NPASS = COUT / PASS_C, NSLAB = CIN / 64;
  constexpr int NSLOT = CIN == 64 ? 2 : 3, DEPTH = NSLOT - 1;
  constexpr int NFILL = F32 ? NPASS * NSLAB * NP : CIN == 64 ? 1 : NPASS * NSLAB;
  constexpr int YS = F32 ? 2 : 1;
  static_assert(!F32 || (!HAS_RES && (CIN > 64 || NPASS == 1)), "fp32 product: no residual; one pass when the tile is filled once per source");
  constexpr int SLOT_N = (TH + 2) * LDS_HW * 8;
  static_assert(COUT % PASS_C == 0 && CIN % 64 == 0, "passes of NCG x 32 output channels over 64-channel input slabs");
  static_assert(!PACK || (CIN == 64 && COUT == 64 && NP == 1), "the packed-pixel form serves the bf16 / f16 64 -> 64 layers");
  __shared__ uint4 s_ring[NSLOT * SLOT_N];
  __shared__ uint16_t s_list[PACK ? 4 * TH * 32 : 1];
  __shared__ int4 s_tile[4];
  __shared__ uint32_t s_rowmask[4][TH];
  __shared__ int4 s_drow[4][NRG];
  __shared__ uint4 s_dmask[4][NRG];
  __shared__ unsigned int s_tick[4];
  const int lane = threadIdx.x & 63, wv = __builtin_amdgcn_readfirstlane((int)(threadIdx.x >> 6));
  const int tiles_x = (W + 31) >> 5, tiles_y = (H + TH - 1) / TH;
  const int64_t n_tiles = tlist != nullptr ? (int64_t)__builtin_amdgcn_readfirstlane(*tcount) : (int64_t)B * tiles_y * tiles_x;
  PC_T_DECL

  if (wv >= 8) {
    const int pw = wv - 8;
    uint32_t voff[5];
    int colv[5];
#pragma unroll
    for (int i = 0; i < 5; i++) {
      const int col = 8 * i + (lane >> 3), k = lane & 7;
      colv[i] = col;
      voff[i] = (uint32_t)(col * CIN + ((k ^ lds_swz(col)) * 8)) * 2u;
    }
    typedef __attribute__((address_space(1))) const void* gptr_t;
    typedef __attribute__((address_space(3))) void* lptr_t;

    auto tile_index = [&](int n) -> int64_t {
      const int64_t idx = (n < 3 || slot < 0) ? (int64_t)blockIdx.x + (int64_t)n * gridDim.x : (int64_t)s_tick[n & 3] + 3 * (int64_t)gridDim.x;
      return tile_at(tlist, idx, n_tiles);
    };
    uint32_t mb[TH / 2];
    uint32_t dirty = 0;
    auto load_meta = [&](int64_t t) {
#pragma unroll
      for (int k = 0; k < TH / 2; k++) mb[k] = 0;
      dirty = 0;
      if (t < 0) return;
      const int tx = (int)(t % tiles_x), ty = (int)((t / tiles_x) % tiles_y), b = (int)(t / ((int64_t)tiles_x * tiles_y));
      const int ox = tx * 32 + (lane & 31);
#pragma unroll
      for (int k = 0; k < TH / 2; k++) {
        const int oy = ty * TH + 2 * k + (lane >> 5);
        if (ox < W && oy < H) mb[k] = mask != nullptr ? (uint32_t)mask[((int64_t)b * H + oy) * W + ox] : 1u;
      }
      const int oy2 = ty * TH + lane;
      if (lane < TH && oy2 < H) dirty = row_dirty != nullptr ? (uint32_t)row_dirty[((int64_t)b * H + oy2) * tiles_x + tx] : 1u;
    };

    int n = 0, f = 0, nf = 0, g = 0;
    int64_t t_next = tile_index(0);
    load_meta(t_next);
    int cb = 0, cy0 = 0, cx0 = 0;
    uint32_t am = 0;

    auto advance = [&]() -> bool {
      const int64_t t = t_next;
      if (t < 0) {
        if (pw == 0 && lane == 0) s_tile[n & 3] = make_int4(-1, 0, 0, 0);
        return false;
      }
      const int tx = (int)(t % tiles_x), ty = (int)((t / tiles_x) % tiles_y);
      cb = (int)(t / ((int64_t)tiles_x * tiles_y));
      cx0 = tx * 32, cy0 = ty * TH;
      uint32_t my_rm = 0;
      am = 0;
      int n_px = 0;
#pragma unroll
      for (int k = 0; k < TH / 2; k++) {
        const unsigned long long bal = __ballot(mb[k] != 0);
        const uint32_t lo = (uint32_t)bal, hi = (uint32_t)(bal >> 32);
        if constexpr (PACK) {
          if (pw == 0 && mb[k] != 0)
            s_list[(n & 3) * (TH * 32) + n_px + __popcll(bal & ((1ull << lane) - 1ull))] = (uint16_t)(((2 * k + (lane >> 5)) << 5) | (lane & 31));
          n_px += __popcll(bal);
        }
        if (lane == 2 * k) my_rm = lo;
        if (lane == 2 * k + 1) my_rm = hi;
        am |= (lo != 0 ? 1u : 0u) << (2 * k) | (hi != 0 ? 1u : 0u) << (2 * k + 1);
      }
      const uint32_t was = (uint32_t)__ballot(dirty != 0) & ((1u << TH) - 1u);
      if (pw == 0) {
        if (lane < TH) s_rowmask[n & 3][lane] = my_rm;
        if (lane == 0) s_tile[n & 3] = make_int4(cb, cy0, cx0, (int)(am | (uint32_t)n_px << 16));
        if (lane < NRG * 4) {
          uint32_t rest = am;
          for (int k = 0; k < lane && rest; k++) rest &= rest - 1;
          const int row = rest != 0 ? __builtin_ctz(rest) : -1;
          const uint32_t m = row >= 0 ? s_rowmask[n & 3][row] : 0u;
          reinterpret_cast<int*>(&s_drow[n & 3][lane % NRG])[lane / NRG] = row;
          reinterpret_cast<uint32_t*>(&s_dmask[n & 3][lane % NRG])[lane / NRG] = m;
        }
      }
      if (slot >= 0 && pw == 0 && lane == 0) s_tick[(n + 3) & 3] = atomicAdd(&g_tile_ctr[slot][0], 1u);
      t_next = tile_index(n + 1);
      load_meta(t_next);
#pragma unroll 1
      for (int r = pw; r < TH; r += 4) {
        const int oy = cy0 + r;
        if (oy >= H) break;
        const bool active = (am >> r) & 1u, w = (was >> r) & 1u;
        if (!active && w) {
          char* dst = reinterpret_cast<char*>(y + (((int64_t)cb * H + oy) * W + cx0) * COUT * YS);
          const int nbytes = (W - cx0 < 32 ? W - cx0 : 32) * COUT * 2 * YS;
#pragma unroll 1
          for (int o = lane * 16; o < nbytes; o += 1024) *reinterpret_cast<uint4*>(dst + o) = make_uint4(0, 0, 0, 0);
        }
        if constexpr (PACK) {
          if (active && w) {
            const uint32_t cols = W - cx0 >= 32 ? 0xffffffffu : (1u << (W - cx0)) - 1u;
            const uint32_t idle = ~(uint32_t)__builtin_amdgcn_readlane((int)my_rm, r) & cols;
            char* dst = reinterpret_cast<char*>(y + (((int64_t)cb * H + oy) * W + cx0) * COUT);
#pragma unroll 1
            for (int c0 = 0; c0 < 32; c0 += 8) {
              if (((idle >> c0) & 255u) == 0) continue;
              const int p = c0 + (lane >> 3);
              if ((idle >> p) & 1u) *reinterpret_cast<uint4*>(dst + p * (COUT * 2) + (lane & 7) * 16) = make_uint4(0, 0, 0, 0);
            }
          }
        }
        if (row_dirty != nullptr && lane == 0 && w != active) row_dirty[((int64_t)cb * H + oy) * tiles_x + tx] = active ? 1 : 0;
      }
      nf = am != 0 ? NFILL : 1;
      f = 0;
      n++;
      return true;
    };

    auto next_fill = [&]() -> bool {
      if (f == nf && !advance()) return false;
      if (am != 0) {
        const int sl = f % NSLAB;
        uint4* dstslot = s_ring + (g % NSLOT) * SLOT_N;
        const uint16_t* xs = X3 && (f / NSLAB) % 2 == 1 ? x2 : x;
        if constexpr (NP == 3) {
          const int q = (f / NSLAB) % 3;
          xs = q == 0 ? x3 : q == 1 ? x2 : x;
        }
        const uint16_t* xt = xs + (((int64_t)cb * H + (cy0 - 1)) * W + (cx0 - 1)) * CIN + 64 * sl;
        bool col_ok[5];
#pragma unroll
        for (int i = 0; i < 5; i++) col_ok[i] = (unsigned)(cx0 - 1 + colv[i]) < (unsigned)W && (i < 4 || lane < 16);
#pragma unroll 1
        for (int r = pw; r < TH + 2; r += 4) {
          const int iy = cy0 - 1 + r;
          const bool row_ok = iy >= 0 && iy < H;
          const char* rowp = reinterpret_cast<const char*>(xt + (int64_t)r * W * CIN);
#pragma unroll
          for (int i = 0; i < 5; i++) {
            if (row_ok && col_ok[i]) {
              __builtin_amdgcn_global_load_lds((gptr_t)(rowp + voff[i]), (lptr_t)(dstslot + r * LDS_HW * 8 + 64 * i), 16, 0, 0);
            } else if (i < 4 || lane < 16) {
              dstslot[r * LDS_HW * 8 + 64 * i + lane] = make_uint4(0, 0, 0, 0);
            }
          }
        }
      }
      f++;
      g++;
      return true;
    };

    bool alive = true;
    int nbar = 0, nbar_total = 0x7fffffff;
    PC_TOCK(7)
    for (int d = 0; d < DEPTH - 1 && alive; d++) {
      alive = next_fill();
      if (!alive) nbar_total = g + 1;
    }
    for (;;) {
      if (alive) {
        alive = next_fill();
        if (!alive) nbar_total = g + 1;
      }
      PC_TOCK(5)
      pc_barrier_all();
      PC_TOCK(6)
      if (++nbar == nbar_total) break;
    }
    PC_T_FLUSH
    return;
  }

  const int rg = wv % NRG, cg = wv / NRG;
  const int px = lane & 31, kb = lane >> 5;
  pc_barrier_lds();
  int g = 0;
  PC_TOCK(7)
  for (int n = 0;; n++) {
    const int4 ti = s_tile[n & 3];
    const int b = __builtin_amdgcn_readfirstlane(ti.x);
    if (b < 0) break;
    const int y0 = __builtin_amdgcn_readfirstlane(ti.y), x0 = __builtin_amdgcn_readfirstlane(ti.z);
    if (__builtin_amdgcn_readfirstlane(ti.w) == 0) {
      pc_barrier_lds();
      g++;
      PC_TOCK(2)
      continue;
    }
    if constexpr (PACK) {
      const int n_px = __builtin_amdgcn_readfirstlane(ti.w) >> 16, n_grp = (n_px + 31) >> 5, rgu = __builtin_amdgcn_readfirstlane(rg);
      const int nr = n_grp > rgu ? (n_grp - rgu + 3) >> 2 : 0;
      int codes[2] = {0, 0}, n_g[4];
#pragma unroll
      for (int j = 0; j < 4; j++) {
        const int gi = rgu + 4 * j;
        n_g[j] = min(max(n_px - 32 * gi, 0), 32);
        if (px < n_g[j]) codes[j >> 1] |= (int)s_list[(n & 3) * (TH * 32) + 32 * gi + px] << (16 * (j & 1));
      }
      const int64_t t0 = (((int64_t)b * H + y0) * W + x0) * COUT;
      const uint16_t* res_t = HAS_RES ? res + t0 : nullptr;
      uint16_t* y_t = y + t0;
      PC_TOCK(0)
#ifdef PNX_CONV_TIMERS
#define PC_PIX(N_) pc_pix64<N_, HAS_RES, NSLOT, SLOT_N>(s_ring, g, wfrag, bias, res_t, y_t, codes, n_g, W, cg, relu, px, kb, lane, pc_T, pc_tk)
#else
#define PC_PIX(N_) pc_pix64<N_, HAS_RES, NSLOT, SLOT_N>(s_ring, g, wfrag, bias, res_t, y_t, codes, n_g, W, cg, relu, px, kb, lane)
#endif
      switch (nr) {
        case 0: PC_PIX(0); break;
        case 1: PC_PIX(1); break;
        case 2: PC_PIX(2); break;
        case 3: PC_PIX(3); break;
        default: PC_PIX(4); break;
      }
#undef PC_PIX
      continue;
    }
    const int4 dr = s_drow[n & 3][rg];
    const uint4 dm = s_dmask[n & 3][rg];
    int rrow[4] = {__builtin_amdgcn_readfirstlane(dr.x), __builtin_amdgcn_readfirstlane(dr.y), __builtin_amdgcn_readfirstlane(dr.z),
                   __builtin_amdgcn_readfirstlane(dr.w)};
    const uint32_t rmask[4] = {(uint32_t)__builtin_amdgcn_readfirstlane((int)dm.x), (uint32_t)__builtin_amdgcn_readfirstlane((int)dm.y),
                               (uint32_t)__builtin_amdgcn_readfirstlane((int)dm.z), (uint32_t)__builtin_amdgcn_readfirstlane((int)dm.w)};
    int nr = 0;
#pragma unroll
    for (int j = 0; j < 4; j++) {
      nr += rrow[j] >= 0 ? 1 : 0;
      rrow[j] = rrow[j] >= 0 ? rrow[j] : 0;
    }
    const uint16_t* res_t = HAS_RES ? res + (((int64_t)b * H + y0) * W + x0) * COUT : nullptr;
    uint16_t* y_t = y + (((int64_t)b * H + y0) * W + x0) * COUT * YS;
    const int n_valid = W - x0;
    PC_TOCK(0)
#ifdef PNX_CONV_TIMERS
#define PC_ROWS(N_) pc_rows<N_, CIN, COUT, HAS_RES, NRG, NSLOT, SLOT_N, NP>(s_ring, g, wfrag, wfrag2, wfrag3, bias, res_t, y_t, rrow, rmask, W, n_valid, cg, relu, px, kb, lane, pc_T, pc_tk)
#else
#define PC_ROWS(N_) pc_rows<N_, CIN, COUT, HAS_RES, NRG, NSLOT, SLOT_N, NP>(s_ring, g, wfrag, wfrag2, wfrag3, bias, res_t, y_t, rrow, rmask, W, n_valid, cg, relu, px, kb, lane)
#endif
    switch (nr) {
      case 0: PC_ROWS(0); break;
      case 1: PC_ROWS(1); break;
      case 2: PC_ROWS(2); break;
      case 3: PC_ROWS(3); break;
      default: PC_ROWS(4); break;
    }
#undef PC_ROWS
  }
  if (threadIdx.x == 0) sched_done(slot);
  PC_T_FLUSH
}

template <int CIN, int COUT>
int launch_pc(const ConvArgs& a, bool pack = false) {
  constexpr int TH = CIN == 64 ? 16 : 8;
  int64_t nb = (int64_t)a.B * ((a.H + TH - 1) / TH) * ((a.W + 31) / 32);
  if (nb > 256) nb = 256;
  const int slot = a.mask != nullptr ? next_sched_slot() : -1;
  if constexpr (CIN == 64 && COUT == 64) {
    if (pack && a.mask != nullptr) {
      if (a.res != nullptr)
        k_conv3x3_pc<64, 64, true, 1, true><<<(unsigned)nb, 768, 0, a.st>>>(a.x, nullptr, a.wfrag, nullptr, a.bias, a.res, a.mask, a.y, a.B, a.H, a.W, a.relu,
                                                                          a.row_dirty, slot, a.tlist, a.tcount);
      else
        k_conv3x3_pc<64, 64, false, 1, true><<<(unsigned)nb, 768, 0, a.st>>>(a.x, nullptr, a.wfrag, nullptr, a.bias, nullptr, a.mask, a.y, a.B, a.H, a.W, a.relu,
                                                                           a.row_dirty, slot, a.tlist, a.tcount);
      PNX_LAUNCH_CHECK();
      return PNX_OK;
    }
  }
  if (a.res != nullptr)
    k_conv3x3_pc<CIN, COUT, true><<<(unsigned)nb, 768, 0, a.st>>>(a.x, nullptr, a.wfrag, nullptr, a.bias, a.res, a.mask, a.y, a.B, a.H, a.W, a.relu, a.row_dirty,
                                                                slot, a.tlist, a.tcount);
  else
    k_conv3x3_pc<CIN, COUT, false><<<(unsigned)nb, 768, 0, a.st>>>(a.x, nullptr, a.wfrag, nullptr, a.bias, nullptr, a.mask, a.y, a.B, a.H, a.W, a.relu, a.row_dirty,
                                                                 slot, a.tlist, a.tcount);
  PNX_LAUNCH_CHECK();
  return PNX_OK;
}

template <int CIN, int COUT, int NP>
int launch_pc_f32(PnxPieces<NP> x, PnxPieces<NP> w, const float* bias, const uint8_t* mask, float* y, int B, int H, int W, hipStream_t st) {
  constexpr int TH = CIN == 64 ? 16 : 8;
  int64_t nb = (int64_t)B * ((H + TH - 1) / TH) * ((W + 31) / 32);
  if (nb > 256) nb = 256;
  const int slot = mask != nullptr ? next_sched_slot() : -1;
  k_conv3x3_pc<CIN, COUT, false, NP><<<(unsigned)nb, 768, 0, st>>>((const uint16_t*)x.hi, (const uint16_t*)x.slot2(), (const uint4*)w.hi, (const uint4*)w.slot2(),
                                                                   bias, nullptr, mask, (uint16_t*)y, B, H, W, 0, nullptr, slot, nullptr, nullptr,
                                                                   (const uint16_t*)x.slot3(), (const uint4*)w.slot3());
  PNX_LAUNCH_CHECK();
  return PNX_OK;
}
```

pillarnext_amd/csrc/conv_rows.h:

```cpp
#pragma once


template <int NR, int COUT, bool HAS_RES>
__device__ __forceinline__ void conv_rows(const uint4* __restrict__ s_in, const uint4* __restrict__ wfrag, const float* __restrict__ bias,
                                          const uint16_t* const (&rrow_res)[4], uint32_t res_off, const int (&rbase)[4], const uint32_t (&rmask)[4],
                                          uint16_t* const (&yrow)[4], int n_valid, int relu, int px, int kb, int lane) {
  constexpr int MTALL = COUT / 32;
#pragma unroll 1
  for (int mg = 0; mg < MTALL; mg += 2) {
    v16f acc[NR][2];
#pragma unroll
    for (int m = 0; m < 2; m++) {
      const v16f bq = bias_tile(bias, (mg + m) * 32, kb);
#pragma unroll
      for (int j = 0; j < NR; j++) acc[j][m] = bq;
    }
    uint4 rq[2][2];
    if (HAS_RES) load_residual_u(rq, rrow_res[0], res_off, rmask[0] >> px & 1u);
    conv_taps<NR, MTALL, 4, 1, 2, COUT == 64 ? 2 : TAPS_WD>(acc, s_in, wfrag, rbase, mg, px, kb, lane);
#pragma unroll
    for (int j = 0; j < NR; j++) {
      const bool act = (rmask[j] >> px) & 1u;
      uint4 rc[2][2];
      if (HAS_RES) {
#pragma unroll
        for (int m = 0; m < 2; m++)
#pragma unroll
          for (int t = 0; t < 2; t++) rc[m][t] = rq[m][t];
        if (j + 1 < NR) load_residual_u(rq, rrow_res[j + 1], res_off, rmask[j + 1] >> px & 1u);
      }
      uint4 D[4];
#pragma unroll
      for (int m = 0; m < 2; m++) {
        uint4 pk[2];
        pack_tile(acc[j][m], act, relu, pk, HAS_RES ? rc[m] : nullptr);
        D[2 * m] = pk[0], D[2 * m + 1] = pk[1];
      }
      transpose_row64(D, lane);
      store_row64<COUT>(D, yrow[j] + mg * 32, n_valid, lane);
    }
  }
}

template <int COUT, bool HAS_RES>
__global__ __launch_bounds__(256, 2) void k_conv3x3_lds(const uint16_t* __restrict__ x, const uint4* __restrict__ wfrag,
                                                     const float* __restrict__ bias, const uint16_t* __restrict__ res,
                                                     const uint8_t* __restrict__ mask, uint16_t* __restrict__ y, int B, int H, int W,
                                                     int relu, uint8_t* __restrict__ row_dirty, int slot, const int32_t* __restrict__ tlist,
                                                      const int32_t* __restrict__ tcount) {
  constexpr int CIN = 64;
  constexpr int TH = LDS_TH, HW_ = LDS_HW;
  static_assert(!HAS_RES || COUT == 64, "the residual is folded into the accumulators of a single 64-channel pass");
  __shared__ uint4 s_in[LDS_NSTAGE];
  __shared__ uint32_t s_rowmask2[2 * TH];
  __shared__ unsigned int s_next[2];
  const int lane = threadIdx.x & 63, wv = threadIdx.x >> 6;
  const int px = lane & 31, kb = lane >> 5;
  const int tiles_x = (W + 31) >> 5, tiles_y = (H + TH - 1) / TH;
  const int64_t n_tiles = tlist != nullptr ? (int64_t)__builtin_amdgcn_readfirstlane(*tcount) : (int64_t)B * tiles_y * tiles_x;
  auto load_mask = [&](int64_t t, bool (&a)[4], int (&wz)[4]) {
#pragma unroll
    for (int j = 0; j < 4; j++) a[j] = false, wz[j] = 1;
    if (t < 0) return;
    const int tx = (int)(t % tiles_x);
    const int ty = (int)((t / tiles_x) % tiles_y);
    const int b = (int)(t / ((int64_t)tiles_x * tiles_y));
    const int ox = tx * 32 + px;
#pragma unroll
    for (int j = 0; j < 4; j++) {
      const int oy = ty * TH + wv * 4 + j;
      a[j] = ox < W && oy < H && (mask == nullptr || mask[((int64_t)b * H + oy) * W + ox] != 0);
      if (row_dirty != nullptr && oy < H) wz[j] = (int)row_dirty[((int64_t)b * H + oy) * tiles_x + tx];
    }
  };
  int64_t idxB = (int64_t)blockIdx.x + gridDim.x, idxC = 0;
  int64_t tileA = tile_at(tlist, blockIdx.x, n_tiles), tileB = tile_at(tlist, idxB, n_tiles), tileC = -1;
  bool aP[4], aN[4];
  int wasP[4], wasN[4];
  load_mask(tileA, aP, wasP);
#pragma unroll
  for (int j = 0; j < 4; j++) aN[j] = false, wasN[j] = 1;
  CT_DECL
  int it = 0;
  for (; tileA >= 0; tileA = tileB, tileB = tileC, idxB = idxC, it++) {
    const int64_t tile = (int64_t)__builtin_amdgcn_readfirstlane((int)tileA);
    sched_draw(s_next, it, slot);
    uint32_t* const s_rowmask = s_rowmask2 + (it & 1) * TH;
    const int tx = (int)(tile % tiles_x);
    const int ty = (int)((tile / tiles_x) % tiles_y);
    const int b = (int)(tile / ((int64_t)tiles_x * tiles_y));
    const int x0 = tx * 32, y0 = ty * TH;
    const int ox = x0 + px;
    CT_TOCK(7)
    bool was[4];
#pragma unroll
    for (int j = 0; j < 4; j++) {
      was[j] = __builtin_amdgcn_readfirstlane(wasP[j]) != 0;
      const uint32_t bal = (uint32_t)__ballot(aP[j]);
      if (lane == 0) s_rowmask[wv * 4 + j] = bal;
    }
    __syncthreads();
    idxC = sched_next2(s_next, it, slot, idxB);
    tileC = tile_at(tlist, idxC, n_tiles);
    load_mask(tileB, aN, wasN);
#pragma unroll
    for (int j = 0; j < 4; j++) aP[j] = aN[j], wasP[j] = wasN[j];
    CT_TOCK(0)
    const uint32_t my_rm = s_rowmask[lane & 15];
    const uint32_t am = (uint32_t)__ballot(my_rm != 0) & 0xffffu;
#pragma unroll
    for (int j = 0; j < 4; j++) {
      const int rr = wv * 4 + j, oy = y0 + rr;
      const bool active = (am >> rr) & 1u;
      if (!active && was[j] && oy < H && ox < W) {
        uint4* dst = reinterpret_cast<uint4*>(y + (((int64_t)b * H + oy) * W + ox) * COUT);
#pragma unroll 1
        for (int ch = kb; ch < COUT / 8; ch += 2) dst[ch] = make_uint4(0, 0, 0, 0);
      }
      if (row_dirty != nullptr && oy < H && lane == 0 && was[j] != active) row_dirty[((int64_t)b * H + oy) * tiles_x + tx] = active ? 1 : 0;
    }
    if (am == 0) continue;
    int nr = 0;
    int rbase[4], rrow[4];
    {
      uint32_t rest = am;
      for (int k = 0; k < wv && rest; k++) rest &= rest - 1;
#pragma unroll
      for (int j = 0; j < 4; j++) {
        const bool has = rest != 0;
        rrow[j] = has ? __builtin_ctz(rest) : 0;
        nr += has ? 1 : 0;
        for (int k = 0; k < 4 && rest; k++) rest &= rest - 1;
      }
    }
    nr = __builtin_amdgcn_readfirstlane(nr);
    uint32_t rmask[4];
    uint16_t* yrow[4];
#pragma unroll
    for (int j = 0; j < 4; j++) {
      rrow[j] = __builtin_amdgcn_readfirstlane(rrow[j]);
      rbase[j] = rrow[j] * HW_ * 8;
      rmask[j] = j < nr ? __builtin_amdgcn_readfirstlane(s_rowmask[rrow[j]]) : 0u;
      yrow[j] = y + (((int64_t)b * H + (y0 + rrow[j])) * W + x0) * COUT;
    }
    const uint32_t need = am | (am << 1) | (am << 2);
    CT_TOCK(1)
    const uint16_t* rres[4];
#pragma unroll
    for (int j = 0; j < 4; j++) rres[j] = HAS_RES ? res + (((int64_t)b * H + (y0 + rrow[j])) * W + x0) * COUT : nullptr;
    const uint32_t res_off = (uint32_t)(px * COUT + 8 * kb) * 2u;
    stage_tile64<CIN>(s_in, x, b, H, W, 0, y0, x0, need);
    CT_TOCK(2)
    __syncthreads();
    CT_TOCK(3)
    const int n_valid = W - x0;
    switch (nr) {
      case 1: conv_rows<1, COUT, HAS_RES>(s_in, wfrag, bias, rres, res_off, rbase, rmask, yrow, n_valid, relu, px, kb, lane); break;
      case 2: conv_rows<2, COUT, HAS_RES>(s_in, wfrag, bias, rres, res_off, rbase, rmask, yrow, n_valid, relu, px, kb, lane); break;
      case 3: conv_rows<3, COUT, HAS_RES>(s_in, wfrag, bias, rres, res_off, rbase, rmask, yrow, n_valid, relu, px, kb, lane); break;
      case 4: conv_rows<4, COUT, HAS_RES>(s_in, wfrag, bias, rres, res_off, rbase, rmask, yrow, n_valid, relu, px, kb, lane); break;
      default: break;
    }
    CT_TOCK(4)
  }
  sched_done(slot);
  CT_FLUSH
}

constexpr int L128_TH = 8;
constexpr int L128_NSTAGE = (L128_TH + 2) * LDS_HW * 8;

int next_sched_slot() {
  static unsigned int n = 0;
  return (int)(n++ & 63u);
}

constexpr int LDSX_RES_WD = 2;
template <int NR, int CIN, int COUT, bool HAS_RES>
__device__ __forceinline__ void conv_rows_x(uint4* __restrict__ s_in, const uint16_t* __restrict__ x, const uint4* __restrict__ wfrag,
                                            const float* __restrict__ bias, const uint16_t* __restrict__ res, const int (&rrow)[4],
                                            const int (&rbase)[4], const uint32_t (&rmask)[4], uint16_t* const (&yrow)[4], int b, int H, int W,
                                            int y0, int x0, uint32_t need, int mg0, int relu, int px, int kb, int lane, int hsel) {
  constexpr int NS = CIN / 64, NRA = NR > 0 ? NR : 1;
  const int ox = x0 + px;
  {
    const int h = hsel;
    const int mg = mg0 + 4 * h;
    v16f acc[NRA][2];
    if (NR > 0) {
#pragma unroll
      for (int m = 0; m < 2; m++) {
        const v16f bq = bias_tile(bias, (mg + m) * 32, kb);
#pragma unroll
        for (int j = 0; j < NR; j++) acc[j][m] = bq;
      }
    }
    const uint16_t* rres[NRA];
    const uint32_t res_off = (uint32_t)(px * COUT + 8 * kb) * 2u;
    uint4 rq[2][2];
    if (NR > 0 && HAS_RES) {
#pragma unroll
      for (int j = 0; j < NR; j++) rres[j] = res + (((int64_t)b * H + (y0 + rrow[j])) * W + x0) * COUT + mg * 32;
    }
#pragma unroll 1
    for (int sl = 0; sl < NS; sl++) {
      if (sl) {
        __syncthreads();
        stage_tile64<CIN, L128_TH>(s_in, x, b, H, W, 64 * sl, y0, x0, need);
        __syncthreads();
      }
      if (NR > 0 && HAS_RES && sl == NS - 1) load_residual_u(rq, rres[0], res_off, rmask[0] >> px & 1u);
      if (NR > 0) conv_taps<NRA, COUT / 32, CIN / 16, 1, 2, HAS_RES ? LDSX_RES_WD : TAPS_WD>(acc, s_in, wfrag, rbase, mg, px, kb, lane, 4 * sl);
    }
    if (NR > 0) {
      const int n_valid = W - x0;
#pragma unroll
      for (int j = 0; j < NR; j++) {
        const bool act = (rmask[j] >> px) & 1u;
        uint4 rc[2][2];
        if (HAS_RES) {
#pragma unroll
          for (int m = 0; m < 2; m++)
#pragma unroll
            for (int t = 0; t < 2; t++) rc[m][t] = rq[m][t];
          if (j + 1 < NR) load_residual_u(rq, rres[j + 1], res_off, rmask[j + 1] >> px & 1u);
        }
        uint4 D[4];
#pragma unroll
        for (int m = 0; m < 2; m++) {
          uint4 pk[2];
          pack_tile(acc[j][m], act, relu, pk, HAS_RES ? rc[m] : nullptr);
          D[2 * m] = pk[0], D[2 * m + 1] = pk[1];
        }
        transpose_row64(D, lane);
        store_row64<COUT>(D, yrow[j] + mg * 32, n_valid, lane);
      }
    }
  }
}

__device__ __forceinline__ int pix_code(int row, int col) { return (row << 5) | col; }
template <int CSTRIDE>
__device__ __forceinline__ uint32_t pix_off(int code, int W) { return (uint32_t)(((code >> 5) * W + (code & 31)) * CSTRIDE) * 2u; }

template <int CSTRIDE>
__device__ __forceinline__ void store_pix64(const uint4 (&D)[4], uint16_t* __restrict__ tile, int code, int n_valid, int W, int lane) {
  int l = lane;
  asm volatile("" : "+v"(l));
#pragma unroll
  for (int d = 0; d < 4; d++) {
    const int P = 8 * d + (l >> 3);
    const int pc = __builtin_amdgcn_ds_bpermute(P << 2, code);
    if (P < n_valid) *reinterpret_cast<uint4*>(reinterpret_cast<char*>(tile) + pix_off<CSTRIDE>(pc, W) + (uint32_t)((l & 7) * 16)) = D[d];
  }
}

template <int NR, int CIN, int COUT, bool HAS_RES>
__device__ __forceinline__ void conv_pix_x(uint4* __restrict__ s_in, const uint16_t* __restrict__ x, const uint4* __restrict__ wfrag,
                                           const float* __restrict__ bias, const uint16_t* __restrict__ rtile, int codes, const int (&n_g)[4],
                                           uint16_t* __restrict__ ytile, int b, int H, int W, int y0, int x0, uint32_t need, int mg0, int relu, int px,
                                           int kb, int lane, int hsel) {
  constexpr int NS = CIN / 64, NRA = NR > 0 ? NR : 1;
  const int mg = mg0 + 4 * hsel;
  v16f acc[NRA][2];
  if (NR > 0) {
#pragma unroll
    for (int m = 0; m < 2; m++) {
      const v16f bq = bias_tile(bias, (mg + m) * 32, kb);
#pragma unroll
      for (int j = 0; j < NR; j++) acc[j][m] = bq;
    }
  }
  const uint16_t* const rres = HAS_RES ? rtile + mg * 32 : nullptr;
  auto code = [&](int j) { return (codes >> (8 * j)) & 255; };
  auto res_off = [&](int j) { return pix_off<COUT>(code(j), W) + (uint32_t)(16 * kb); };
  const int cw[4] = {codes, 0, 0, 0};
  uint4 rq[2][2];
#pragma unroll 1
  for (int sl = 0; sl < NS; sl++) {
    if (sl) {
      __syncthreads();
      stage_tile64<CIN, L128_TH>(s_in, x, b, H, W, 64 * sl, y0, x0, need);
      __syncthreads();
    }
    if (NR > 0 && HAS_RES && sl == NS - 1) load_residual_u(rq, rres, res_off(0), px < n_g[0]);
    if (NR > 0) conv_taps<NRA, COUT / 32, CIN / 16, 1, 2, HAS_RES ? LDSX_RES_WD : TAPS_WD, true>(acc, s_in, wfrag, cw, mg, px, kb, lane, 4 * sl);
  }
  if (NR > 0) {
#pragma unroll
    for (int j = 0; j < NR; j++) {
      const bool act = px < n_g[j];
      uint4 rc[2][2];
      if (HAS_RES) {
#pragma unroll
        for (int m = 0; m < 2; m++)
#pragma unroll
          for (int t = 0; t < 2; t++) rc[m][t] = rq[m][t];
        if (j + 1 < NR) load_residual_u(rq, rres, res_off(j + 1), px < n_g[j + 1]);
      }
      uint4 D[4];
#pragma unroll
      for (int m = 0; m < 2; m++) {
        uint4 pk[2];
        pack_tile(acc[j][m], act, relu, pk, HAS_RES ? rc[m] : nullptr);
        D[2 * m] = pk[0], D[2 * m + 1] = pk[1];
      }
      transpose_row64(D, lane);
      store_pix64<COUT>(D, ytile + mg * 32, code(j), n_g[j], W, lane);
    }
  }
}

template <int CIN, int COUT, bool HAS_RES, bool PACK = false>
__global__ __launch_bounds__(256, 2) void k_conv3x3_ldsx(const uint16_t* __restrict__ x, const uint4* __restrict__ wfrag,
                                                      const float* __restrict__ bias, const uint16_t* __restrict__ res,
                                                      const uint8_t* __restrict__ mask, uint16_t* __restrict__ y, int B, int H, int W,
                                                      int relu, uint8_t* __restrict__ row_dirty, int slot, const int32_t* __restrict__ tlist,
                                                      const int32_t* __restrict__ tcount) {
  static_assert(CIN % 64 == 0 && (COUT % 128 == 0 || COUT == 64), "64-channel input slabs, 128-channel output passes (or one of 64)");
  constexpr int TH = L128_TH, HW_ = LDS_HW;
  constexpr int NRG = COUT == 64 ? 4 : 2, NRMAX = TH / NRG;
  static_assert(!PACK || (CIN == COUT && NRG == 2), "the packed-pixel form serves 128 -> 128 and 256 -> 256");
  __shared__ uint4 s_in[L128_NSTAGE];
  __shared__ uint16_t s_list[PACK ? TH * 32 : 1];
  __shared__ uint32_t s_rowmask2[2 * TH];
  __shared__ unsigned int s_next[2];
  const int lane = threadIdx.x & 63, wv = threadIdx.x >> 6;
  const int px = lane & 31, kb = lane >> 5;
  const int rg = wv % NRG, mg0 = 2 * (wv / NRG);
  const int tiles_x = (W + 31) >> 5, tiles_y = (H + TH - 1) / TH;
  const int n_tiles = tlist != nullptr ? __builtin_amdgcn_readfirstlane(*tcount) : B * tiles_y * tiles_x;
  constexpr int NH = (COUT + 127) / 128;
  const int n_units = n_tiles * NH;
  auto unit_at = [&](int64_t idx) -> int {
    if (idx >= n_units) return -1;
    const int i = (int)idx;
    const int t = tlist != nullptr ? tlist[i / NH] : i / NH;
    return t * NH + i % NH;
  };
  auto load_mask = [&](int t, bool (&a)[2], int (&wz)[2]) {
#pragma unroll
    for (int j = 0; j < 2; j++) a[j] = false, wz[j] = 1;
    if (t < 0) return;
    const int tx = (int)(t % tiles_x);
    const int ty = (int)((t / tiles_x) % tiles_y);
    const int b = (int)(t / ((int64_t)tiles_x * tiles_y));
    const int ox = tx * 32 + px;
#pragma unroll
    for (int j = 0; j < 2; j++) {
      const int oy = ty * TH + wv * 2 + j;
      a[j] = ox < W && oy < H && (mask == nullptr || mask[((int64_t)b * H + oy) * W + ox] != 0);
      if (row_dirty != nullptr && oy < H) wz[j] = (int)row_dirty[((int64_t)b * H + oy) * tiles_x + tx];
    }
  };
  int64_t idxB = (int64_t)blockIdx.x + gridDim.x, idxC = 0;
  int tileA = unit_at(blockIdx.x), tileB = unit_at(idxB), tileC = -1;
  bool aP[2], aN[2];
  int wasP[2], wasN[2];
  load_mask(tileA >= 0 ? tileA / NH : -1, aP, wasP);
#pragma unroll
  for (int j = 0; j < 2; j++) aN[j] = false, wasN[j] = 1;
  int it = 0;
  for (; tileA >= 0; tileA = tileB, tileB = tileC, idxB = idxC, it++) {
    const int unit = __builtin_amdgcn_readfirstlane(tileA);
    const int tile = unit / NH;
    const int hsel = unit - tile * NH;
    sched_draw(s_next, it, slot);
    uint32_t* const s_rowmask = s_rowmask2 + (it & 1) * TH;
    const int tx = (int)(tile % tiles_x);
    const int ty = (int)((tile / tiles_x) % tiles_y);
    const int b = (int)(tile / ((int64_t)tiles_x * tiles_y));
    const int x0 = tx * 32, y0 = ty * TH;
    const int ox = x0 + px;
    bool was[2];
    uint32_t bal[2];
#pragma unroll
    for (int j = 0; j < 2; j++) {
      was[j] = __builtin_amdgcn_readfirstlane(wasP[j]) != 0;
      bal[j] = (uint32_t)__ballot(aP[j]);
      if (lane == 0) s_rowmask[wv * 2 + j] = bal[j];
    }
    __syncthreads();
    idxC = sched_next2(s_next, it, slot, idxB);
    tileC = unit_at(idxC);
    load_mask(tileB >= 0 ? tileB / NH : -1, aN, wasN);
#pragma unroll
    for (int j = 0; j < 2; j++) aP[j] = aN[j], wasP[j] = wasN[j];
    const uint32_t my_rm = s_rowmask[lane & 7];
    const uint32_t am = (uint32_t)__ballot(my_rm != 0) & 0xffu;
#pragma unroll
    for (int j = 0; j < 2; j++) {
      const int rr = wv * 2 + j, oy = y0 + rr;
      const bool active = (am >> rr) & 1u;
      if (hsel != 0) continue;
      if (!active && was[j] && oy < H && ox < W) {
        uint4* dst = reinterpret_cast<uint4*>(y + (((int64_t)b * H + oy) * W + ox) * COUT);
#pragma unroll 1
        for (int ch = kb; ch < COUT / 8; ch += 2) dst[ch] = make_uint4(0, 0, 0, 0);
      }
      if (row_dirty != nullptr && oy < H && lane == 0 && was[j] != active) row_dirty[((int64_t)b * H + oy) * tiles_x + tx] = active ? 1 : 0;
    }
    if (am == 0) continue;
    if constexpr (PACK) {
      const int wvu = __builtin_amdgcn_readfirstlane(wv);
      int n_px = 0, pos = 0;
#pragma unroll
      for (int k = 0; k < TH; k++) {
        const int n = __builtin_popcount(__builtin_amdgcn_readlane(my_rm, k));
        n_px += n;
        pos += k < 2 * wvu ? n : 0;
      }
#pragma unroll
      for (int j = 0; j < 2; j++) {
        if (kb == 0 && ((bal[j] >> px) & 1u)) s_list[pos + __builtin_popcount(bal[j] & ((1u << px) - 1u))] = (uint16_t)pix_code(wvu * 2 + j, px);
        pos += __builtin_popcount(bal[j]);
      }
      const int n_grp = (n_px + 31) >> 5, rgu = __builtin_amdgcn_readfirstlane(rg);
      const int nr = n_grp > rgu ? (n_grp - rgu + 1) >> 1 : 0;
      const uint32_t need = am | (am << 1) | (am << 2);
      stage_tile64<CIN, TH>(s_in, x, b, H, W, 0, y0, x0, need);
      __syncthreads();
      int codes = 0, n_g[4];
#pragma unroll
      for (int j = 0; j < 4; j++) {
        const int g = rgu + 2 * j;
        n_g[j] = min(max(n_px - 32 * g, 0), 32);
        if (j < nr && px < n_g[j]) codes |= (int)s_list[32 * g + px] << (8 * j);
      }
      const int64_t t0 = (((int64_t)b * H + y0) * W + x0) * COUT;
#define PNX_PIX_X(N_) conv_pix_x<N_, CIN, COUT, HAS_RES>(s_in, x, wfrag, bias, HAS_RES ? res + t0 : nullptr, codes, n_g, y + t0, b, H, W, y0, x0, need, mg0, relu, px, kb, lane, hsel)
      switch (nr) {
        case 0: PNX_PIX_X(0); break;
        case 1: PNX_PIX_X(1); break;
        case 2: PNX_PIX_X(2); break;
        case 3: PNX_PIX_X(3); break;
        default: PNX_PIX_X(4); break;
      }
#undef PNX_PIX_X
      int l = lane;
      asm volatile("" : "+v"(l));
      const uint32_t cols = W - x0 >= 32 ? 0xffffffffu : (1u << (W - x0)) - 1u;
#pragma unroll
      for (int j = 0; j < 2; j++) {
        const int rr = wvu * 2 + j;
        const uint32_t idle = ~bal[j] & cols;
        if (!((am >> rr) & 1u) || !was[j] || y0 + rr >= H || idle == 0) continue;
        char* const row = reinterpret_cast<char*>(y + t0) + (uint32_t)(rr * W * COUT * 2 + hsel * 256);
#pragma unroll 1
        for (int c0 = 0; c0 < 32; c0 += 4) {
          if (((idle >> c0) & 15u) == 0) continue;
          const int p = c0 + (l >> 4);
          if ((idle >> p) & 1u) *reinterpret_cast<uint4*>(row + (uint32_t)(p * COUT * 2 + (l & 15) * 16)) = make_uint4(0, 0, 0, 0);
        }
      }
      continue;
    }
    int nr = 0;
    int rbase[4], rrow[4];
    {
      uint32_t rest = am;
      for (int k = 0; k < rg && rest; k++) rest &= rest - 1;
#pragma unroll
      for (int j = 0; j < 4; j++) {
        const bool has = j < NRMAX && rest != 0;
        rrow[j] = has ? __builtin_ctz(rest) : 0;
        nr += has ? 1 : 0;
        for (int k = 0; k < NRG && rest; k++) rest &= rest - 1;
      }
    }
    nr = __builtin_amdgcn_readfirstlane(nr);
    uint32_t rmask[4];
    uint16_t* yrow[4];
#pragma unroll
    for (int j = 0; j < 4; j++) {
      rrow[j] = __builtin_amdgcn_readfirstlane(rrow[j]);
      rbase[j] = rrow[j] * HW_ * 8;
      rmask[j] = j < nr ? __builtin_amdgcn_readfirstlane(s_rowmask[rrow[j]]) : 0u;
      yrow[j] = y + (((int64_t)b * H + (y0 + rrow[j])) * W + x0) * COUT;
    }
    const uint32_t need = am | (am << 1) | (am << 2);
    stage_tile64<CIN, TH>(s_in, x, b, H, W, 0, y0, x0, need);
    __syncthreads();
#define PNX_ROWS_X(N_) conv_rows_x<(N_ <= NRMAX ? N_ : NRMAX), CIN, COUT, HAS_RES>(s_in, x, wfrag, bias, res, rrow, rbase, rmask, yrow, b, H, W, y0, x0, need, mg0, relu, px, kb, lane, hsel)
    switch (nr) {
      case 0: PNX_ROWS_X(0); break;
      case 1: PNX_ROWS_X(1); break;
      case 2: PNX_ROWS_X(2); break;
      case 3: PNX_ROWS_X(3); break;
      default: PNX_ROWS_X(4); break;
    }
#undef PNX_ROWS_X
  }
  sched_done(slot);
}

template <int CIN, int COUT>
int launch_ldsx(const ConvArgs& a, bool pack = false) {
  const int slot = a.mask != nullptr ? next_sched_slot() : -1;
  int64_t nb = (int64_t)a.B * ((a.H + L128_TH - 1) / L128_TH) * ((a.W + 31) / 32) * ((COUT + 127) / 128);
  if (nb > 512) nb = 512;
  if constexpr (CIN == COUT) {
    if (pack && a.mask != nullptr) {
      if (a.res != nullptr)
        k_conv3x3_ldsx<CIN, COUT, true, true><<<(unsigned)nb, 256, 0, a.st>>>(a.x, a.wfrag, a.bias, a.res, a.mask, a.y, a.B, a.H, a.W, a.relu, a.row_dirty, slot,
                                                                            a.tlist, a.tcount);
      else
        k_conv3x3_ldsx<CIN, COUT, false, true><<<(unsigned)nb, 256, 0, a.st>>>(a.x, a.wfrag, a.bias, nullptr, a.mask, a.y, a.B, a.H, a.W, a.relu, a.row_dirty, slot,
                                                                             a.tlist, a.tcount);
      PNX_LAUNCH_CHECK();
      return PNX_OK;
    }
  }
  if (a.res != nullptr)
    k_conv3x3_ldsx<CIN, COUT, true><<<(unsigned)nb, 256, 0, a.st>>>(a.x, a.wfrag, a.bias, a.res, a.mask, a.y, a.B, a.H, a.W, a.relu, a.row_dirty, slot, a.tlist,
                                                                   a.tcount);
  else
    k_conv3x3_ldsx<CIN, COUT, false><<<(unsigned)nb, 256, 0, a.st>>>(a.x, a.wfrag, a.bias, nullptr, a.mask, a.y, a.B, a.H, a.W, a.relu, a.row_dirty, slot, a.tlist,
                                                                    a.tcount);
  PNX_LAUNCH_CHECK();
  return PNX_OK;
}
```

pillarnext_amd/csrc/conv_s2.h:

```cpp
#pragma once

constexpr int S2_TH = 4;
constexpr int S2_ROWS = 2 * S2_TH + 1;
constexpr int S2_NSTAGE = S2_ROWS * S2_RS * 8;

template <int CSTRIDE>
__device__ __forceinline__ void stage_tile64_s2(uint4* __restrict__ s_in, const uint16_t* __restrict__ x, int b, int H, int W, int ch0, int iy0,
                                                int ix0, uint32_t need) {
  typedef __attribute__((address_space(1))) const void* gptr_t;
  typedef __attribute__((address_space(3))) void* lptr_t;
  int tid = threadIdx.x;
  asm volatile("" : "+v"(tid));
  const int slot = tid & 7, col = tid >> 3, wbase = (tid >> 6) * 8;
  const uint16_t* xb = x + (int64_t)b * H * W * CSTRIDE + ch0;
#pragma unroll
  for (int pl = 0; pl < 2; pl++) {
    const int ls = pl * 32 + col;
    const int ix = ix0 + 2 * col + (1 - pl);
    const bool col_ok = (unsigned)ix < (unsigned)W;
    const int chunk = slot ^ lds_swz(ls);
#pragma unroll
    for (int r = 0; r < S2_ROWS; r++) {
      if (!((need >> r) & 1u)) continue;
      const int iy = iy0 + r;
      if ((unsigned)iy < (unsigned)H && col_ok) {
        __builtin_amdgcn_global_load_lds((gptr_t)(xb + ((int64_t)iy * W + ix) * CSTRIDE + chunk * 8),
                                         (lptr_t)(s_in + (r * S2_RS + pl * 32 + wbase) * 8), 16, 0, 0);
      } else {
        s_in[(r * S2_RS + ls) * 8 + slot] = make_uint4(0, 0, 0, 0);
      }
    }
  }
  if (tid < S2_ROWS * 8) {
    const int re = tid >> 3, ce = tid & 7;
    if ((need >> re) & 1u) {
      const int iy = iy0 + re, ix = ix0 + 64;
      uint4 qe = make_uint4(0, 0, 0, 0);
      if ((unsigned)iy < (unsigned)H && (unsigned)ix < (unsigned)W) qe = *reinterpret_cast<const uint4*>(xb + ((int64_t)iy * W + ix) * CSTRIDE + ce * 8);
      s_in[(re * S2_RS + 64) * 8 + (ce ^ lds_swz(64))] = qe;
    }
  }
}

template <int NR, int CIN, int COUT, int MB, int NP = 1>
__device__ __forceinline__ void conv_rows_s2(uint4* __restrict__ s_in, const uint16_t* __restrict__ x, const uint16_t* __restrict__ x2,
                                             const uint16_t* __restrict__ x3, const uint4* __restrict__ wfrag, const uint4* __restrict__ wfrag2,
                                             const uint4* __restrict__ wfrag3, const float* __restrict__ bias, const int (&rbase)[4], const uint32_t (&rmask)[4],
                                             uint16_t* const (&yrow)[4], int b, int H, int W, int iy0, int ix0, int n_valid, uint32_t need, int mg,
                                             int relu, int px, int kb, int lane) {
  constexpr int NS = CIN / 64, NRA = NR > 0 ? NR : 1;
  constexpr bool X3 = NP == 2, F32 = NP > 1;
  v16f acc[NRA][MB];
  if (NR > 0) {
#pragma unroll
    for (int m = 0; m < MB; m++) {
      v16f bq;
      if (F32 && bias == nullptr) {
#pragma unroll
        for (int i = 0; i < 16; i++) bq[i] = 0.f;
      } else {
        bq = bias_tile(bias, (mg + m) * 32, kb);
      }
#pragma unroll
      for (int j = 0; j < NR; j++) acc[j][m] = bq;
    }
  }
#pragma unroll 1
  for (int sq = 0; sq < NS * NP; sq++) {
    const int sl = F32 ? sq % NS : sq;
    if (sq) {
      __syncthreads();
      const uint16_t* xs = X3 && sq >= NS ? x2 : x;
      if constexpr (NP == 3) xs = sq < NS ? x3 : sq < 2 * NS ? x2 : x;
      stage_tile64_s2<CIN>(s_in, xs, b, H, W, 64 * sl, iy0, ix0, need);
      __syncthreads();
    }
    if (NR > 0) {
      if constexpr (NP == 3) {
        const int q = sq / NS;
#pragma unroll 1
        for (int k = q; k >= 0; k--)
          conv_taps<NRA, COUT / 32, CIN / 16, 2, MB>(acc, s_in, k == 0 ? wfrag : k == 1 ? wfrag2 : wfrag3, rbase, mg, px, kb, lane, 4 * sl);
      } else {
        conv_taps<NRA, COUT / 32, CIN / 16, 2, MB>(acc, s_in, wfrag, rbase, mg, px, kb, lane, 4 * sl);
        if constexpr (X3) {
          if (sq < NS) conv_taps<NRA, COUT / 32, CIN / 16, 2, MB>(acc, s_in, wfrag2, rbase, mg, px, kb, lane, 4 * sl);
        }
      }
    }
  }
  if (NR > 0) {
#pragma unroll
    for (int j = 0; j < NR; j++) {
      const bool act = (rmask[j] >> px) & 1u;
      if constexpr (F32) {
#pragma unroll
        for (int m = 0; m < MB; m++) store_tile_f32<COUT>(acc[j][m], act, reinterpret_cast<float*>(yrow[j]) + (mg + m) * 32, n_valid, px, kb);
      } else if constexpr (MB == 2) {
        uint4 D[4];
#pragma unroll
        for (int m = 0; m < 2; m++) {
          uint4 pk[2];
          pack_tile(acc[j][m], act, relu, pk);
          D[2 * m] = pk[0], D[2 * m + 1] = pk[1];
        }
        transpose_row64(D, lane);
        store_row64<COUT>(D, yrow[j] + mg * 32, n_valid, lane);
      } else {
        uint4 pk[2];
        pack_tile(acc[j][0], act, relu, pk);
        transpose_row32(pk, lane);
        store_row32<COUT>(pk, yrow[j] + mg * 32, n_valid, lane);
      }
    }
  }
}

template <int CIN, int COUT, int NP = 1>
__global__ __launch_bounds__(256, 2) void k_conv3x3_s2(const uint16_t* __restrict__ x, const uint16_t* __restrict__ x2, const uint4* __restrict__ wfrag,
                                                    const uint4* __restrict__ wfrag2, const float* __restrict__ bias,
                                                    const uint8_t* __restrict__ mask, uint16_t* __restrict__ y, int B, int H, int W, int Ho, int Wo,
                                                    int relu, uint8_t* __restrict__ row_dirty, int slot, const uint16_t* __restrict__ x3 = nullptr,
                                                    const uint4* __restrict__ wfrag3 = nullptr) {
  static_assert(CIN % 64 == 0 && (COUT == 128 || COUT == 256), "64-channel input slabs; 4 groups of 32 or of 64 output channels");
  constexpr int TH = S2_TH, MB = COUT / 128, NCG = 4, NRG = 1, NRMAX = TH / NRG;
  constexpr int YS = NP > 1 ? 2 : 1;
  extern __shared__ uint4 s_in[];
  __shared__ uint32_t s_rowmask2[2 * TH];
  __shared__ unsigned int s_next[2];
  const int lane = threadIdx.x & 63, wv = threadIdx.x >> 6;
  const int px = lane & 31, kb = lane >> 5;
  const int rg = wv % NRG, mg = MB * (wv / NRG);
  static_assert(NCG * NRG == 4, "four waves");
  const int tiles_x = (Wo + 31) >> 5, tiles_y = (Ho + TH - 1) / TH;
  const int64_t n_tiles = (int64_t)B * tiles_y * tiles_x;
  int64_t next = 0;
  int it = 0;
  for (int64_t tile = blockIdx.x; tile < n_tiles; tile = next, it++) {
    sched_draw(s_next, it, slot);
    uint32_t* const s_rowmask = s_rowmask2 + (it & 1) * TH;
    const int tx = (int)(tile % tiles_x);
    const int ty = (int)((tile / tiles_x) % tiles_y);
    const int b = (int)(tile / ((int64_t)tiles_x * tiles_y));
    const int x0 = tx * 32, y0 = ty * TH;
    const int ox = x0 + px;
    bool was = true;
    {
      const int oy = y0 + wv;
      const bool a = ox < Wo && oy < Ho && (mask == nullptr || mask[((int64_t)b * Ho + oy) * Wo + ox] != 0);
      if (row_dirty != nullptr && oy < Ho) was = __builtin_amdgcn_readfirstlane((int)row_dirty[((int64_t)b * Ho + oy) * tiles_x + tx]) != 0;
      const uint32_t bal = (uint32_t)__ballot(a);
      if (lane == 0) s_rowmask[wv] = bal;
    }
    __syncthreads();
    next = sched_next(s_next, it, slot, tile);
    const uint32_t my_rm = s_rowmask[lane & 3];
    const uint32_t am = (uint32_t)__ballot(my_rm != 0) & 0xfu;
    {
      const int oy = y0 + wv;
      const bool active = (am >> wv) & 1u;
      if (!active && was && oy < Ho && ox < Wo) {
        uint4* dst = reinterpret_cast<uint4*>(y + (((int64_t)b * Ho + oy) * Wo + ox) * COUT * YS);
#pragma unroll 1
        for (int ch = kb; ch < COUT * YS / 8; ch += 2) dst[ch] = make_uint4(0, 0, 0, 0);
      }
      if (row_dirty != nullptr && oy < Ho && lane == 0 && was != active) row_dirty[((int64_t)b * Ho + oy) * tiles_x + tx] = active ? 1 : 0;
    }
    if (am == 0) continue;
    int nr = 0;
    int rbase[4], rrow[4];
    {
      uint32_t rest = am;
      for (int k = 0; k < rg && rest; k++) rest &= rest - 1;
#pragma unroll
      for (int j = 0; j < 4; j++) {
        const bool has = j < NRMAX && rest != 0;
        rrow[j] = has ? __builtin_ctz(rest) : 0;
        nr += has ? 1 : 0;
        for (int k = 0; k < NRG && rest; k++) rest &= rest - 1;
      }
    }
    nr = __builtin_amdgcn_readfirstlane(nr);
    uint32_t rmask[4];
    uint16_t* yrow[4];
#pragma unroll
    for (int j = 0; j < 4; j++) {
      rrow[j] = __builtin_amdgcn_readfirstlane(rrow[j]);
      rbase[j] = 2 * rrow[j] * S2_RS * 8;
      rmask[j] = j < nr ? __builtin_amdgcn_readfirstlane(s_rowmask[rrow[j]]) : 0u;
      yrow[j] = y + (((int64_t)b * Ho + (y0 + rrow[j])) * Wo + x0) * COUT * YS;
    }
    uint32_t need = 0;
#pragma unroll
    for (int r = 0; r < TH; r++)
      if ((am >> r) & 1u) need |= 7u << (2 * r);
    const int iy0 = 2 * y0 - 1, ix0 = 2 * x0 - 1;
    stage_tile64_s2<CIN>(s_in, NP == 3 ? x3 : x, b, H, W, 0, iy0, ix0, need);
    __syncthreads();
#define PNX_ROWS_S2(N_) conv_rows_s2<(N_ <= NRMAX ? N_ : NRMAX), CIN, COUT, MB, NP>(s_in, x, x2, x3, wfrag, wfrag2, wfrag3, bias, rbase, rmask, yrow, b, H, W, iy0, ix0, Wo - x0, need, mg, relu, px, kb, lane)
    switch (nr) {
      case 0: PNX_ROWS_S2(0); break;
      case 1: PNX_ROWS_S2(1); break;
      case 2: PNX_ROWS_S2(2); break;
      case 3: PNX_ROWS_S2(3); break;
      default: PNX_ROWS_S2(4); break;
    }
#undef PNX_ROWS_S2
  }
  sched_done(slot);
}

template <int CIN, int COUT, int NP>
int launch_s2(PnxPieces<NP> x, PnxPieces<NP> wfrag, const float* bias, const uint8_t* mask, void* y, int B, int H, int W, int Ho, int Wo, int relu,
              uint8_t* row_dirty, hipStream_t st) {
  const int slot = mask != nullptr ? next_sched_slot() : -1;
  int64_t nb = (int64_t)B * ((Ho + S2_TH - 1) / S2_TH) * ((Wo + 31) / 32);
  if (nb > 512) nb = 512;
  constexpr auto kern = k_conv3x3_s2<CIN, COUT, NP>;
  constexpr int lds = S2_NSTAGE * 16;
  if (const int rc = pnx_lds_optin<kern>(lds); rc != PNX_OK) return rc;
  kern<<<(unsigned)nb, 256, lds, st>>>((const uint16_t*)x.hi, (const uint16_t*)x.slot2(), (const uint4*)wfrag.hi, (const uint4*)wfrag.slot2(), bias, mask,
                                       (uint16_t*)y, B, H, W, Ho, Wo, relu, row_dirty, slot, (const uint16_t*)x.slot3(), (const uint4*)wfrag.slot3());
  PNX_LAUNCH_CHECK();
  return PNX_OK;
}
```

pillarnext_amd/csrc/conv_tile.h:

```cpp
#pragma once

typedef float v16f __attribute__((ext_vector_type(16)));
typedef float f32x2 __attribute__((ext_vector_type(2)));

#ifdef PNX_CONV_F16
typedef _Float16 el8 __attribute__((ext_vector_type(8)));
typedef _Float16 el2 __attribute__((ext_vector_type(2)));
#define PNX_MFMA32(a, b, c) __builtin_amdgcn_mfma_f32_32x32x16_f16(a, b, c, 0, 0, 0)
#define PNX_MFMA16(a, b, c) __builtin_amdgcn_mfma_f32_16x16x32_f16(a, b, c, 0, 0, 0)
#define PNX_CONV_FN(name) name##_f16
__device__ __forceinline__ uint32_t el_lo_bits(uint32_t w) { return __float_as_uint((float)__builtin_bit_cast(el2, w)[0]); }
__device__ __forceinline__ uint32_t el_hi_bits(uint32_t w) { return __float_as_uint((float)__builtin_bit_cast(el2, w)[1]); }
#else
typedef __bf16 el8 __attribute__((ext_vector_type(8)));
typedef __bf16 el2 __attribute__((ext_vector_type(2)));
#define PNX_MFMA32(a, b, c) __builtin_amdgcn_mfma_f32_32x32x16_bf16(a, b, c, 0, 0, 0)
#define PNX_MFMA16(a, b, c) __builtin_amdgcn_mfma_f32_16x16x32_bf16(a, b, c, 0, 0, 0)
#define PNX_CONV_FN(name) name##_bf16
__device__ __forceinline__ uint32_t el_lo_bits(uint32_t w) { return w << 16; }
__device__ __forceinline__ uint32_t el_hi_bits(uint32_t w) { return w & 0xffff0000u; }
#endif
__device__ __forceinline__ uint32_t pack_el(float lo, float hi) {
  const f32x2 v = {lo, hi};
  return __builtin_bit_cast(uint32_t, __builtin_convertvector(v, el2));
}
__device__ __forceinline__ float round_el(float x) { return __uint_as_float(el_lo_bits(pack_el(x, 0.f))); }

typedef unsigned int u32x2 __attribute__((ext_vector_type(2)));
__device__ __forceinline__ void pack_tile(const v16f& a, bool act, int relu, uint4 (&out)[2], const uint4* res = nullptr) {
#pragma unroll
  for (int t = 0; t < 2; t++) {
    float v[8];
#pragma unroll
    for (int i = 0; i < 4; i++) {
      const u32x2 r = __builtin_amdgcn_permlane32_swap(__float_as_uint(a[8 * t + i]), __float_as_uint(a[8 * t + 4 + i]), false, false);
      v[i] = __uint_as_float(r.x);
      v[4 + i] = __uint_as_float(r.y);
    }
    if (res != nullptr) {
      const uint4 q = res[t];
      v[0] += __uint_as_float(el_lo_bits(q.x)), v[1] += __uint_as_float(el_hi_bits(q.x)), v[2] += __uint_as_float(el_lo_bits(q.y)), v[3] += __uint_as_float(el_hi_bits(q.y));
      v[4] += __uint_as_float(el_lo_bits(q.z)), v[5] += __uint_as_float(el_hi_bits(q.z)), v[6] += __uint_as_float(el_lo_bits(q.w)), v[7] += __uint_as_float(el_hi_bits(q.w));
    }
    if (relu) {
#pragma unroll
      for (int i = 0; i < 8; i++) v[i] = fmaxf(v[i], 0.f);
    }
    uint4 p;
    p.x = pack_el(v[0], v[1]);
    p.y = pack_el(v[2], v[3]);
    p.z = pack_el(v[4], v[5]);
    p.w = pack_el(v[6], v[7]);
    if (!act) p = make_uint4(0, 0, 0, 0);
    out[t] = p;
  }
}

__device__ __forceinline__ void cswap(bool c, uint4& x, uint4& y) {
  const uint4 a = x, b = y;
  x.x = c ? b.x : a.x, x.y = c ? b.y : a.y, x.z = c ? b.z : a.z, x.w = c ? b.w : a.w;
  y.x = c ? a.x : b.x, y.y = c ? a.y : b.y, y.z = c ? a.z : b.z, y.w = c ? a.w : b.w;
}

__device__ __forceinline__ void transpose_row64(uint4 (&R)[4], int lane) {
  const int a_src = (lane & 31) >> 3;
  const int s_dst = (lane & 7) >> 1;
  cswap(a_src & 1, R[0], R[1]);
  cswap(a_src & 1, R[2], R[3]);
  cswap(a_src & 2, R[0], R[2]);
  cswap(a_src & 2, R[1], R[3]);
#pragma unroll
  for (int k = 0; k < 4; k++) {
    const int src = (8 * (k ^ s_dst) + (lane >> 3)) + 32 * (lane & 1);
    R[k].x = (uint32_t)__builtin_amdgcn_ds_bpermute(src << 2, (int)R[k].x);
    R[k].y = (uint32_t)__builtin_amdgcn_ds_bpermute(src << 2, (int)R[k].y);
    R[k].z = (uint32_t)__builtin_amdgcn_ds_bpermute(src << 2, (int)R[k].z);
    R[k].w = (uint32_t)__builtin_amdgcn_ds_bpermute(src << 2, (int)R[k].w);
  }
  cswap(s_dst & 1, R[0], R[1]);
  cswap(s_dst & 1, R[2], R[3]);
  cswap(s_dst & 2, R[0], R[2]);
  cswap(s_dst & 2, R[1], R[3]);
}

template <int CSTRIDE>
__device__ __forceinline__ void store_row64(const uint4 (&D)[4], uint16_t* __restrict__ row, int n_valid, int lane) {
  const uint32_t voff = (uint32_t)((lane >> 3) * CSTRIDE + (lane & 7) * 8) * 2u;
#pragma unroll
  for (int d = 0; d < 4; d++) {
    const int P = 8 * d + (lane >> 3);
    if (P < n_valid) *reinterpret_cast<uint4*>(reinterpret_cast<char*>(row) + voff + (uint32_t)(d * 8 * CSTRIDE * 2)) = D[d];
  }
}

__device__ __forceinline__ void transpose_row32(uint4 (&R)[2], int lane) {
  cswap((lane & 16) != 0, R[0], R[1]);
  const int T = (lane >> 1) & 1;
#pragma unroll
  for (int k = 0; k < 2; k++) {
    const int src = 16 * (k ^ T) + (lane >> 2) + 32 * (lane & 1);
    R[k].x = (uint32_t)__builtin_amdgcn_ds_bpermute(src << 2, (int)R[k].x);
    R[k].y = (uint32_t)__builtin_amdgcn_ds_bpermute(src << 2, (int)R[k].y);
    R[k].z = (uint32_t)__builtin_amdgcn_ds_bpermute(src << 2, (int)R[k].z);
    R[k].w = (uint32_t)__builtin_amdgcn_ds_bpermute(src << 2, (int)R[k].w);
  }
  cswap(T != 0, R[0], R[1]);
}

template <int CSTRIDE>
__device__ __forceinline__ void store_row32(const uint4 (&D)[2], uint16_t* __restrict__ row, int n_valid, int lane) {
  const uint32_t voff = (uint32_t)((lane >> 2) * CSTRIDE + (lane & 3) * 8) * 2u;
#pragma unroll
  for (int d = 0; d < 2; d++) {
    const int P = 16 * d + (lane >> 2);
    if (P < n_valid) *reinterpret_cast<uint4*>(reinterpret_cast<char*>(row) + voff + (uint32_t)(d * 16 * CSTRIDE * 2)) = D[d];
  }
}

template <int COUT>
__device__ __forceinline__ void store_tile_f32(const v16f& a, bool act, float* __restrict__ row, int n_valid, int px, int kb) {
  if (px >= n_valid) return;
  float* p = row + (int64_t)px * COUT + 4 * kb;
#pragma unroll
  for (int g = 0; g < 4; g++) {
    float4 v = make_float4(a[4 * g], a[4 * g + 1], a[4 * g + 2], a[4 * g + 3]);
    if (!act) v = make_float4(0.f, 0.f, 0.f, 0.f);
    *reinterpret_cast<float4*>(p + 8 * g) = v;
  }
}

__device__ __forceinline__ v16f bias_tile(const float* __restrict__ bias, int cbase, int kb) {
  v16f r;
#pragma unroll
  for (int g = 0; g < 4; g++) {
    const float4 q = *reinterpret_cast<const float4*>(bias + cbase + 8 * g + 4 * kb);
    r[4 * g + 0] = q.x, r[4 * g + 1] = q.y, r[4 * g + 2] = q.z, r[4 * g + 3] = q.w;
  }
  return r;
}

__device__ __forceinline__ void load_residual(uint4 (&rq)[2][2], const uint16_t* __restrict__ res_px, bool act, int kb) {
#pragma unroll
  for (int m = 0; m < 2; m++)
#pragma unroll
    for (int t = 0; t < 2; t++) {
      rq[m][t] = make_uint4(0, 0, 0, 0);
      if (act) rq[m][t] = *reinterpret_cast<const uint4*>(res_px + m * 32 + 16 * t + 8 * kb);
    }
}
__device__ __forceinline__ void load_residual_u(uint4 (&rq)[2][2], const uint16_t* __restrict__ row, uint32_t lane_off, bool act) {
#pragma unroll
  for (int m = 0; m < 2; m++)
#pragma unroll
    for (int t = 0; t < 2; t++) {
      rq[m][t] = make_uint4(0, 0, 0, 0);
      if (act) rq[m][t] = *reinterpret_cast<const uint4*>(reinterpret_cast<const char*>(row) + lane_off + (uint32_t)((m * 32 + 16 * t) * 2));
    }
}
__device__ __forceinline__ void add_residual(v16f (&acc2)[2], const uint4 (&rq)[2][2]) {
#pragma unroll
  for (int m = 0; m < 2; m++)
#pragma unroll
    for (int t = 0; t < 2; t++) {
      const uint4 r = rq[m][t];
      const uint32_t lo[4] = {el_lo_bits(r.x), el_hi_bits(r.x), el_lo_bits(r.y), el_hi_bits(r.y)};
      const uint32_t hi[4] = {el_lo_bits(r.z), el_hi_bits(r.z), el_lo_bits(r.w), el_hi_bits(r.w)};
#pragma unroll
      for (int i = 0; i < 4; i++) {
        const u32x2 q = __builtin_amdgcn_permlane32_swap(lo[i], hi[i], false, false);
        acc2[m][8 * t + i] += __uint_as_float(q.x);
        acc2[m][8 * t + 4 + i] += __uint_as_float(q.y);
      }
    }
}

struct ConvArgs {
  const uint16_t* x;
  const uint4* wfrag;
  const float* bias;
  const uint16_t* res;
  const uint8_t* mask;
  uint16_t* y;
  int B, H, W, relu;
  uint8_t* row_dirty;
  const int32_t *tlist, *tcount;
  hipStream_t st;
};
```

pillarnext_amd/ops.py:

```python
import ctypes

import torch

from . import _lib
from ._lib import PNX_BF16, PNX_F16, PNX_F32, PNX_NCHW, PNX_NHWC, PnxError, check, lib, ptr, stream_ptr

_DT = {torch.float32: PNX_F32, torch.bfloat16: PNX_BF16, torch.float16: PNX_F16}


def _need_cuda(t, name):
    if not t.is_cuda:
        raise PnxError(f"{name} must be a CUDA (ROCm) tensor; the PillarNeXt hot path has no CPU implementation")
    if not t.is_contiguous():
        raise PnxError(f"{name} must be contiguous")


class Workspace:

    def __init__(self, headroom=1.25):
        self._bufs, self._headroom = {}, headroom

    @staticmethod
    def _key(device=None):
        dev = torch.cuda.current_device() if device is None or device.index is None else device.index
# ... 557 lines not shown
    return arr


def sephead_lazy(tasks, class_task, batch, local, seg_len, pre_max):
    dt = tasks[0][0].dtype
    arr = lazy_task_table(tasks, batch, dt)
    nc = len(class_task)
    ct = (ctypes.c_int32 * nc)(*[int(v) for v in class_task])
    S = batch * nc
    if not (local.is_cuda and local.dtype == torch.int64 and local.numel() == S * pre_max and seg_len.dtype == torch.int32 and seg_len.numel() == S):
        raise PnxError("sephead_lazy: local must be int64 (lists*pre_max), seg_len int32 (lists)")
    local, seg_len = local.contiguous(), seg_len.contiguous()
    out = torch.empty((S, pre_max, 10), dtype=torch.float32, device=local.device)
    check(_conv_fn("sephead_lazy", dt)(arr, len(tasks), ct, nc, batch, ptr(local), ptr(seg_len), pre_max, ptr(out), stream_ptr()), "pnx_sephead_lazy_bf16")
    return out


_PARTIALS_WS = Workspace(headroom=1.0)


_PIECES_TAG = {1: "bf16", 2: "x3", 3: "x6"}


def _pieces(t):
    return (t,) if isinstance(t, torch.Tensor) else tuple(t)


def _bf16_maps(tensors, what):
    for tns in tensors:
        if not (tns.is_cuda and tns.dtype == torch.bfloat16 and tns.dim() == 4 and tns.is_contiguous(memory_format=torch.channels_last)
                and tns.shape == tensors[0].shape):
            raise PnxError(f"{what} needs channels_last bf16 CUDA pieces of one shape")


def _bf16_packs(wfrags, n, what):
    if len(wfrags) != n or any(w.dtype != torch.bfloat16 or w.numel() != wfrags[0].numel() for w in wfrags):
        raise PnxError(f"{what}: the weights must be {n} packed bf16 piece(s) of one size, one per piece of the other operand")


def split_f32(x, mask=None, pieces=2):
    if pieces not in (2, 3):
        raise PnxError(f"split_f32: 2 or 3 pieces, got {pieces!r}")
    if not (x.is_cuda and x.dtype == torch.float32 and x.numel() % 8 == 0):
        raise PnxError("split_f32 needs an fp32 CUDA tensor with a multiple of 8 elements")
    if not (x.is_contiguous() or (x.dim() == 4 and x.is_contiguous(memory_format=torch.channels_last))):
        raise PnxError("split_f32 needs a dense tensor (contiguous or channels_last)")
    c = 0
    if mask is not None:
        if not (x.dim() == 4 and x.is_contiguous(memory_format=torch.channels_last) and mask.dtype == torch.uint8 and mask.is_contiguous()
                and tuple(mask.shape) == (x.shape[0], x.shape[2], x.shape[3]) and x.shape[1] % 8 == 0):
            raise PnxError("split_f32: mask needs a channels_last (B,C,H,W) tensor with C % 8 == 0 and a contiguous uint8 (B,H,W) mask")
        c = x.shape[1]
    out = tuple(torch.empty_like(x, dtype=torch.bfloat16) for _ in range(pieces))
    name = "pnx_split_f32" if pieces == 2 else "pnx_split3_f32"
    check(getattr(lib(), name)(ptr(x), *map(ptr, out), x.numel(), ptr(mask), c, stream_ptr()), name)
    return out


CONV3X3_X3_SHAPES = {1: {(64, 64), (128, 128), (256, 256)}, 2: {(64, 128), (128, 256), (256, 256)}}


def conv3x3_f32(x_pieces, wfrag_pieces, cout, stride, mask, bias=None):
    xs, ws = tuple(x_pieces), tuple(wfrag_pieces)
    if len(xs) not in (2, 3):
        raise PnxError(f"conv3x3_f32: 2 or 3 pieces per operand, got {len(xs)}")
    if bias is not None and not (bias.is_cuda and bias.dtype == torch.float32 and bias.numel() == cout and bias.is_contiguous()):
        raise PnxError("conv3x3_f32: bias must be a contiguous fp32 CUDA vector of Cout values")
    _bf16_maps(xs, "conv3x3_f32")
    _bf16_packs(ws, len(xs), "conv3x3_f32")
    B, ci, H, W = xs[0].shape
    Ho, Wo = (H - 1) // stride + 1, (W - 1) // stride + 1
    if mask is not None and (tuple(mask.shape) != (B, Ho, Wo) or mask.dtype != torch.uint8):
        raise PnxError("conv3x3_f32: mask must be uint8 (B,Ho,Wo)")
    y = torch.empty((B, cout, Ho, Wo), dtype=torch.float32, device=xs[0].device, memory_format=torch.channels_last)
    name = "pnx_conv3x3_" + _PIECES_TAG[len(xs)]
    check(getattr(lib(), name)(*map(ptr, xs), *map(ptr, ws), ptr(bias), ptr(mask), ptr(y), B, H, W, ci, cout, stride, stream_ptr()), name)
    return y


def conv3x3_wgrad(x, dy, mask, stride=1):
    xs, gs = _pieces(x), _pieces(dy)
    if len(xs) not in _PIECES_TAG or len(gs) != len(xs):
        raise PnxError("conv3x3_wgrad: x and dy must be one bf16 tensor each or tuples of 2 or 3 pieces of equal length")
    _bf16_maps(xs, "conv3x3_wgrad: x")
    _bf16_maps(gs, "conv3x3_wgrad: dy")
    B, ci, H, W = xs[0].shape
    co = gs[0].shape[1]
    Ho, Wo = (H - 1) // stride + 1, (W - 1) // stride + 1
    if stride not in (1, 2) or tuple(gs[0].shape) != (B, co, Ho, Wo) or tuple(mask.shape) != (B, Ho, Wo) or mask.dtype != torch.uint8:
        raise PnxError("conv3x3_wgrad: stride 1 or 2, dy (B,Cout,Ho,Wo) and a uint8 (B,Ho,Wo) mask of the output sites")
    nbytes = int(lib().pnx_conv3x3_wgrad_workspace_bytes(ci, co))
    if nbytes == 0:
        raise PnxError(f"conv3x3_wgrad: no kernel for {ci} -> {co} channels")
    ws = _PARTIALS_WS.get(nbytes, xs[0].device)
    dw = torch.empty((co, ci, 3, 3), dtype=torch.float32, device=xs[0].device)
    name = "pnx_conv3x3_wgrad_" + _PIECES_TAG[len(xs)]
    check(getattr(lib(), name)(*map(ptr, xs), *map(ptr, gs), ptr(mask), ptr(dw), B, H, W, ci, co, stride, ptr(ws), ws.numel(), stream_ptr()), name)
    return dw


def conv3x3_dgrad_s2(g, wfrag_t, cin, in_hw, mask_in):
    gs, ws = _pieces(g), _pieces(wfrag_t)
    if len(gs) not in _PIECES_TAG:
        raise PnxError("conv3x3_dgrad_s2: g must be one bf16 tensor or a tuple of 2 or 3 pieces")
    _bf16_maps(gs, "conv3x3_dgrad_s2")
    _bf16_packs(ws, len(gs), "conv3x3_dgrad_s2")
    H, W = in_hw
    B, co, Ho, Wo = gs[0].shape
    if (Ho, Wo) != ((H - 1) // 2 + 1, (W - 1) // 2 + 1) or tuple(mask_in.shape) != (B, H, W) or mask_in.dtype != torch.uint8 or not mask_in.is_contiguous():
        raise PnxError("conv3x3_dgrad_s2: g (B,cout,Ho,Wo) with Ho = (H - 1) // 2 + 1 and a contiguous uint8 (B,H,W) mask of the input sites")
    dx = torch.empty((B, cin, H, W), dtype=torch.bfloat16 if len(gs) == 1 else torch.float32, device=gs[0].device, memory_format=torch.channels_last)
    name = "pnx_conv3x3_dgrad_s2_" + _PIECES_TAG[len(gs)]
    check(getattr(lib(), name)(*map(ptr, gs), *map(ptr, ws), ptr(mask_in), ptr(dx), B, H, W, cin, co, stream_ptr()), name)
    return dx


def _smallk_check(x, what):
    if not (x.is_cuda and x.dim() == 4 and x.dtype in (torch.float32, torch.bfloat16) and x.is_contiguous(memory_format=torch.channels_last)):
        raise PnxError(f"{what} must be a channels_last fp32 / bf16 CUDA tensor")


def conv3x3_smallk(x, weight, bias=None):
    _smallk_check(x, "conv3x3_smallk: x")
    k = weight.shape[0]
    if not (weight.is_cuda and weight.dtype == torch.float32 and tuple(weight.shape[1:]) == (64, 3, 3) and weight.is_contiguous() and 1 <= k <= 4
            and x.shape[1] == 64 and (bias is None or (bias.is_cuda and bias.dtype == torch.float32 and bias.numel() == k and bias.is_contiguous()))):
        raise PnxError("conv3x3_smallk: weight must be a contiguous fp32 (k,64,3,3) with k <= 4, bias fp32 (k)")
    B, _, H, W = x.shape
    y = torch.empty((B, k, H, W), dtype=x.dtype, device=x.device, memory_format=torch.channels_last)
    if k == 1:
        y = torch.empty((B, H, W, 1), dtype=x.dtype, device=x.device).permute(0, 3, 1, 2)
    check(lib().pnx_conv3x3_smallk(ptr(x), ptr(weight), ptr(bias), ptr(y), B, H, W, 64, k, 0 if x.dtype == torch.float32 else 1, stream_ptr()), "pnx_conv3x3_smallk")
    return y


def conv3x3_smallk_wgrad(x, dy, want_bias=True):
    _smallk_check(x, "conv3x3_smallk_wgrad: x")
    B, c, H, W = x.shape
    k = dy.shape[1]
    if not (c == 64 and 1 <= k <= 4 and dy.is_cuda and dy.dtype == x.dtype and tuple(dy.shape) == (B, k, H, W)):
        raise PnxError("conv3x3_smallk_wgrad: x (B,64,H,W), dy (B,k,H,W) of the same dtype, k <= 4")
    dyc = dy.permute(0, 2, 3, 1).contiguous()
    nbytes = int(lib().pnx_conv3x3_smallk_wgrad_workspace_bytes(k))
    ws = _PARTIALS_WS.get(nbytes, x.device)
    dw = torch.empty((k, 64, 3, 3), dtype=torch.float32, device=x.device)
    db = torch.empty((k,), dtype=torch.float32, device=x.device) if want_bias else None
    check(lib().pnx_conv3x3_smallk_wgrad(ptr(x), ptr(dyc), ptr(dw), ptr(db), B, H, W, 64, k, 0 if x.dtype == torch.float32 else 1, ptr(ws), ws.numel(), stream_ptr()),
          "pnx_conv3x3_smallk_wgrad")
    return dw, db


def conv3x3_workspace(batch, cout, ho, wo, device, dtype=torch.bfloat16):
    y = torch.zeros((batch, cout, ho, wo), dtype=dtype, device=device).contiguous(memory_format=torch.channels_last)
    return y, torch.zeros((batch, ho, (wo + 31) // 32), dtype=torch.uint8, device=device)


def conv_tile_rows(cin, cout, stride=1):
    return int(lib().pnx_conv3x3_tile_rows(cin, cout, stride))


def conv_tile_buffers(mask, tile_rows, out=None):
    B, H, W = _like(mask).shape
    n_tiles = B * ((H + tile_rows - 1) // tile_rows) * ((W + 31) // 32)
    if out is None:
        return torch.empty((n_tiles,), dtype=torch.int32, device=mask.device), torch.zeros((1,), dtype=torch.int32, device=mask.device)
    if out[0].numel() < n_tiles or out[0].dtype != torch.int32 or out[1].dtype != torch.int32:
        raise PnxError("conv_tile_list: needs an int32 list of >= n_tiles entries + an int32 count")
    return out


def conv_tile_list(mask, dirties, tile_rows, out=None):
    B, H, W = mask.shape
    out = conv_tile_buffers(mask, tile_rows, out)
    arr = (ctypes.c_void_p * max(len(dirties), 1))(*[d.data_ptr() for d in dirties])
    check(lib().pnx_conv_tile_list(ptr(mask), arr, len(dirties), B, H, W, tile_rows, ptr(out[0]), ptr(out[1]), stream_ptr()), "pnx_conv_tile_list")
    return out


def _conv3x3_dims(x, wfrag, cout, stride, mask, residual, out, cuda=False):
    xs = _half_nhwc(x, "conv3x3", cuda=cuda)
    if wfrag.dtype != xs.dtype or (residual is not None and _like(residual).dtype != xs.dtype):
        raise PnxError("conv3x3: weights / residual of another dtype than the input")
    B, ci, H, W = xs.shape
    Ho, Wo = _out_hw(H, W, stride)
    if out is not None:
        y, dirty = out
        if (tuple(_half_nhwc(y, "conv3x3 output", xs.dtype).shape) != (B, cout, Ho, Wo)
                or (dirty is not None and (mask is None or tuple(dirty.shape) != (B, Ho, (Wo + 31) // 32)))):
            raise PnxError("conv3x3: output / workspace of the wrong shape (a workspace needs a mask)")
    return B, H, W, ci, _DT[xs.dtype], Ho, Wo


def conv3x3_masked(x, wfrag, bias, cout, stride=1, mask=None, residual=None, relu=True, out=None, tiles=None):
    B, H, W, ci, _, Ho, Wo = _conv3x3_dims(x, wfrag, cout, stride, mask, residual, out, cuda=True)
    y, dirty = out if out is not None else (torch.empty((B, cout, Ho, Wo), dtype=x.dtype, device=x.device, memory_format=torch.channels_last), None)
    tl, tc = tiles if tiles is not None else (None, None)
    check(_conv_fn("conv3x3", x.dtype)(ptr(x), ptr(wfrag), ptr(bias), ptr(residual), ptr(mask), ptr(y), B, H, W, ci, cout, stride, 1 if relu else 0,
                                       ptr(dirty), ptr(tl), ptr(tc), stream_ptr()), "pnx_conv3x3")
    return y


MASKED_BN_CHANNELS = (8, 16, 32, 64, 128, 256)


def _bn_maps(what, x, mask, *like_x):
    if not (x.is_cuda and x.dim() == 4 and x.dtype in (torch.bfloat16, torch.float32) and x.shape[1] in MASKED_BN_CHANNELS
            and x.is_contiguous(memory_format=torch.channels_last)):
        raise PnxError(f"{what}: x must be a channels_last bf16 / fp32 CUDA map (B,C,H,W) with C in {MASKED_BN_CHANNELS}")
    n = x.shape[0] * x.shape[2] * x.shape[3]
    if mask is not None and not (mask.is_cuda and mask.dtype == torch.float32 and mask.dim() == 1 and mask.numel() == n and mask.is_contiguous()):
        raise PnxError(f"{what}: the mask must be a flat fp32 CUDA vector of B*H*W = {n} values, or None")
    for t in like_x:
        if t is not None and not (t.is_cuda and t.dtype == x.dtype and t.shape == x.shape and t.is_contiguous(memory_format=torch.channels_last)):
            raise PnxError(f"{what}: the residual and the gradient must have x's dtype, shape and channels_last layout")
    return n, x.shape[1], _DT[x.dtype]


def _bn_vecs(what, n, *vecs, dtype=torch.float32):
    for v in vecs:
        if v is not None and not (v.is_cuda and v.dtype == dtype and v.dim() == 1 and v.numel() == n and v.is_contiguous()):
            raise PnxError(f"{what}: needs contiguous {str(dtype).split('.')[-1]} CUDA vectors of {n} values")


def masked_bn_blocks():
    return int(lib().pnx_masked_bn_blocks())


def masked_bn_stats(x, mask, center):
    n, C, dt = _bn_maps("masked_bn_stats", x, mask)
    _bn_vecs("masked_bn_stats", C, center)
    part = torch.empty((masked_bn_blocks(), 2 * C + 1), dtype=torch.float32, device=x.device)
    check(lib().pnx_masked_bn_stats(ptr(x), dt, ptr(mask), n, C, ptr(center), ptr(part), stream_ptr()), "pnx_masked_bn_stats")
    return part


def _masked_channels(c):
    return c in MASKED_BN_CHANNELS


def _bn_reduce(what, part, channels_ok, channels):
    if not (part.is_cuda and part.dtype == torch.float32 and part.dim() == 2 and part.is_contiguous() and channels_ok(part.shape[1] // 2)):
        raise PnxError(f"{what}: the partials must be a contiguous fp32 CUDA matrix of 2C or 2C + 1 columns with {channels}")
    rows, cols = part.shape
    if rows == 0:
        return torch.zeros((cols,), dtype=torch.float64, device=part.device)
    s = torch.empty((cols,), dtype=torch.float64, device=part.device)
    check(lib().pnx_masked_bn_reduce(ptr(part), rows, cols, ptr(s), stream_ptr()), "pnx_masked_bn_reduce")
    return s


def _bn_finalize(what, channels_ok, channels, sums, center, weight, bias, eps, momentum, running_mean, running_var, num_batches_tracked):
    C = (sums.numel() - 1) // 2
    _bn_vecs(what, 2 * C + 1, sums, dtype=torch.float64)
    _bn_vecs(what, C, center, weight, bias, running_mean, running_var)
    nbt = num_batches_tracked
    if not channels_ok(C) or (nbt is not None and not (nbt.is_cuda and nbt.dtype == torch.int64 and nbt.numel() == 1)):
        raise PnxError(f"{what}: 2C + 1 sums with {channels}, num_batches_tracked an int64 CUDA scalar")
    vec = torch.empty((4 * C + 1,), dtype=torch.float32, device=sums.device)
    mean, invstd, scale, shift, cnt = vec[:C], vec[C:2 * C], vec[2 * C:3 * C], vec[3 * C:4 * C], vec[4 * C:]
    check(lib().pnx_masked_bn_finalize(ptr(sums), C, ptr(center), ptr(weight), ptr(bias), float(eps), float(momentum), ptr(running_mean), ptr(running_var),
                                       ptr(nbt), ptr(mean), ptr(invstd), ptr(scale), ptr(shift), ptr(cnt), stream_ptr()), "pnx_masked_bn_finalize")
    return mean, invstd, scale, shift, cnt


def _bn_bwd_finalize(what, channels_ok, channels, sums_local, sums_global, count):
    C = sums_local.numel() // 2
    _bn_vecs(what, 2 * C, sums_local, sums_global, dtype=torch.float64)
    _bn_vecs(what, 1, count)
    if not channels_ok(C):
        raise PnxError(f"{what}: 2C sums with {channels}")
    vec = torch.empty((4 * C,), dtype=torch.float32, device=sums_local.device)
    dgamma, dbeta, mg, mgx = vec[:C], vec[C:2 * C], vec[2 * C:3 * C], vec[3 * C:]
    check(lib().pnx_masked_bn_bwd_finalize(ptr(sums_local), ptr(sums_global), C, ptr(count), ptr(dgamma), ptr(dbeta), ptr(mg), ptr(mgx), stream_ptr()),
          "pnx_masked_bn_bwd_finalize")
    return dgamma, dbeta, mg, mgx


def masked_bn_reduce(part):
    return _bn_reduce("masked_bn_reduce", part, _masked_channels, f"C in {MASKED_BN_CHANNELS}")


def masked_bn_finalize(sums, center, weight, bias, eps, momentum, running_mean, running_var, num_batches_tracked):
    return _bn_finalize("masked_bn_finalize", _masked_channels, f"C in {MASKED_BN_CHANNELS}", sums, center, weight, bias, eps, momentum, running_mean,
                        running_var, num_batches_tracked)


def masked_bn_apply(x, residual, mask, scale, shift, relu):
    n, C, dt = _bn_maps("masked_bn_apply", x, mask, residual)
    _bn_vecs("masked_bn_apply", C, scale, shift)
    y = torch.empty_like(x)
    check(lib().pnx_masked_bn_apply(ptr(x), ptr(residual), dt, ptr(mask), n, C, ptr(scale), ptr(shift), 1 if relu else 0, ptr(y), stream_ptr()),
          "pnx_masked_bn_apply")
    return y


def masked_bn_bwd_stats(gy, x, residual, mask, scale, shift, mean, invstd, relu):
    n, C, dt = _bn_maps("masked_bn_bwd_stats", x, mask, residual, gy)
    _bn_vecs("masked_bn_bwd_stats", C, scale, shift, mean, invstd)
    part = torch.empty((masked_bn_blocks(), 2 * C), dtype=torch.float32, device=x.device)
    check(lib().pnx_masked_bn_bwd_stats(ptr(gy), ptr(x), ptr(residual), dt, ptr(mask), n, C, ptr(scale), ptr(shift), ptr(mean), ptr(invstd), 1 if relu else 0,
                                        ptr(part), stream_ptr()), "pnx_masked_bn_bwd_stats")
    return part


def masked_bn_bwd_finalize(sums_local, sums_global, count):
    return _bn_bwd_finalize("masked_bn_bwd_finalize", _masked_channels, f"C in {MASKED_BN_CHANNELS}", sums_local, sums_global, count)


def masked_bn_bwd_apply(gy, x, residual, mask, scale, shift, mean, invstd, relu, mean_g, mean_gx, want_residual_grad=False):
    n, C, dt = _bn_maps("masked_bn_bwd_apply", x, mask, residual, gy)
    _bn_vecs("masked_bn_bwd_apply", C, scale, shift, mean, invstd, mean_g, mean_gx)
    dx = torch.empty_like(x)
    gres = torch.empty_like(residual) if residual is not None and want_residual_grad else None
    check(lib().pnx_masked_bn_bwd_apply(ptr(gy), ptr(x), ptr(residual), dt, ptr(mask), n, C, ptr(scale), ptr(shift), ptr(mean), ptr(invstd), 1 if relu else 0,
                                        ptr(mean_g), ptr(mean_gx), ptr(dx), ptr(gres), stream_ptr()), "pnx_masked_bn_bwd_apply")
    return dx, gres


def _i3(v):
    return (ctypes.c_int32 * 3)(*[int(a) for a in v])


class Sp3Index:

    def __init__(self, batch, grid, device):
        self.batch, self.grid = int(batch), tuple(int(g) for g in grid)
        self.nbytes = lib().pnx_sp3_index_bytes(self.batch, _i3(self.grid))
        if self.nbytes == 0:
            raise PnxError(f"sparse3d: bad grid {self.batch} x {self.grid}")
        self.buf = torch.empty((self.nbytes,), dtype=torch.uint8, device=device)


def _need_coords(coords):
    _need_cuda(coords, "coords")
    if coords.dtype != torch.int32 or coords.dim() != 2 or coords.shape[1] != 4:
        raise PnxError("coords must be (N, 4) int32 [b, z, y, x]")


def sp3_out_grid(batch, grid, kernel, stride, pad):
    out = _i3((0, 0, 0))
    check(lib().pnx_sp3_out_grid(int(batch), _i3(grid), _i3(kernel), _i3(stride), _i3(pad), out), "pnx_sp3_out_grid")
    return tuple(out)


def sp3_index_build(coords, batch, grid, want_rows=False):
    _need_coords(coords)
    ix = Sp3Index(batch, grid, coords.device)
    n = coords.shape[0]
# ... 486 lines not shown
```

Before: 757.2.

## Track per-pixel written masks so persistent conv outputs zero only stale pixels

Replaces the per-row-segment dirty byte with a flag plus a 32-bit mask of which pixels in each 32-wide segment were written last frame. Conv kernels (lds, ldsx, pc, s2, direct) now zero only the pixels that were written before and are inactive now, not whole segments or all idle columns. This aims to cut redundant zero-fill stores into the reused output canvases. In exchange it adds a larger workspace carve, a 256-byte alignment requirement, extra mask loads and stores per tile row, and an env-selected stale mode.

```diff
diff --git a/include/pnx.h b/include/pnx.h
--- a/include/pnx.h
+++ b/include/pnx.h
@@ -127,6 +127,7 @@
                        int32_t relu, pnx_stream_t stream);
 int pnx_deconv2x2_f16(const void* x, const void* wfrag, const float* bias, void* y, int32_t batch, int32_t h, int32_t w, int32_t cin, int32_t cout,
                        int32_t relu, pnx_stream_t stream);
+size_t pnx_conv3x3_row_dirty_bytes(int32_t batch, int32_t ho, int32_t wo);
 int pnx_conv3x3_bf16(const void* x, const void* wfrag, const float* bias, const void* residual, const uint8_t* mask, void* y, int32_t batch,
                      int32_t h, int32_t w, int32_t cin, int32_t cout, int32_t stride, int32_t relu, uint8_t* row_dirty, const int32_t* tile_list,
                      const int32_t* tile_count, pnx_stream_t stream);
diff --git a/pillarnext_amd/_lib.py b/pillarnext_amd/_lib.py
--- a/pillarnext_amd/_lib.py
+++ b/pillarnext_amd/_lib.py
@@ -100,6 +100,7 @@
     "pnx_conv3x3_bf16": (ctypes.c_int, [_vp, _vp, _vp, _vp, _vp, _vp, _i32, _i32, _i32, _i32, _i32, _i32, _i32, _vp, _vp, _vp, _vp]),
     "pnx_conv3x3_f16": (ctypes.c_int, [_vp, _vp, _vp, _vp, _vp, _vp, _i32, _i32, _i32, _i32, _i32, _i32, _i32, _vp, _vp, _vp, _vp]),
     "pnx_conv3x3_tile_rows": (ctypes.c_int, [_i32, _i32, _i32]),
+    "pnx_conv3x3_row_dirty_bytes": (_sz, [_i32, _i32, _i32]),
     "pnx_conv3x3_pack_weights": (ctypes.c_int, [_vp, _i32, _i32, _i32, _i32, _vp, _vp]),
     "pnx_conv3x3_wgrad_workspace_bytes": (_sz, [_i32, _i32]),
     "pnx_conv3x3_wgrad_bf16": (ctypes.c_int, [_vp, _vp, _vp, _vp, _i32, _i32, _i32, _i32, _i32, _i32, _vp, _sz, _vp]),
diff --git a/pillarnext_amd/csrc/conv3x3.hip b/pillarnext_amd/csrc/conv3x3.hip
--- a/pillarnext_amd/csrc/conv3x3.hip
+++ b/pillarnext_amd/csrc/conv3x3.hip
@@ -8,7 +8,7 @@
 __global__ __launch_bounds__(256, 2) void k_conv3x3(const uint16_t* __restrict__ x, const uint4* __restrict__ wfrag,
                                                  const float* __restrict__ bias, const uint16_t* __restrict__ res,
                                                  const uint8_t* __restrict__ mask, uint16_t* __restrict__ y, int B, int H, int W, int Ho,
-                                                 int Wo, int relu, uint8_t* __restrict__ row_dirty) {
+                                                 int Wo, int relu, RowDirty row_dirty) {
   constexpr int CB = CIN / 16, MT = COUT / 32, KSTEPS = 9 * CB;
   constexpr int NT = (MT <= 2) ? 4 : 2;
   extern __shared__ uint4 s_w[];
@@ -41,11 +41,12 @@
     for (int j = 0; j < NT; j++) {
       const int oy = oy0 + j;
       row_store[j] = oy < Ho;
-      if (row_dirty != nullptr && oy < Ho) {
-        uint8_t* d = row_dirty + ((int64_t)b * Ho + oy) * tiles_x + tx;
-        const bool was = __builtin_amdgcn_readfirstlane((int)*d) != 0;
-        row_store[j] = any_row[j] || was;
-        if (lane == 0 && was != any_row[j]) *d = any_row[j] ? 1 : 0;
+      const uint32_t now = (uint32_t)__ballot(act[j]);
+      if (row_dirty.flag != nullptr && oy < Ho) {
+        const int64_t seg = ((int64_t)b * Ho + oy) * tiles_x + tx;
+        const uint32_t was = (uint32_t)__builtin_amdgcn_readfirstlane((int)rd_load(row_dirty, seg));
+        row_store[j] = any_row[j] || was != 0;
+        if (lane == 0) rd_store(row_dirty, seg, was, now);
       }
     }
     v16f acc[NT][MT];
@@ -273,6 +274,11 @@
 }
 
 #ifndef PNX_CONV_F16
+size_t pnx_conv3x3_row_dirty_bytes(int32_t batch, int32_t ho, int32_t wo) {
+  if (batch <= 0 || ho <= 0 || wo <= 0) return 0;
+  return row_dirty_carve(nullptr, (int64_t)batch * ho * ((wo + 31) / 32)).bytes;
+}
+
 int pnx_conv3x3_tile_rows(int32_t cin, int32_t cout, int32_t stride) {
   if (stride != 1) return 0;
   if (cin == 64 && (cout == 64 || cout == 320 || cout == 384 || cout == 448)) return LDS_TH;
@@ -318,7 +324,14 @@
               "16-byte alignment required");
   const int ho = (h + 2 - 3) / stride + 1, wo = (w + 2 - 3) / stride + 1;
   hipStream_t st = (hipStream_t)stream;
-  const ConvArgs a = {(const uint16_t*)x, (const uint4*)wfrag, bias, (const uint16_t*)residual, mask, (uint16_t*)y, batch, h, w, relu, row_dirty, tile_list,
+  static const int stale_mode = getenv("PNX_CONV_STALE") != nullptr ? atoi(getenv("PNX_CONV_STALE")) : 1;
+  RowDirty rd = {nullptr, nullptr, stale_mode != 0 ? 1 : 0};
+  if (row_dirty != nullptr) {
+    PNX_REQUIRE(((uintptr_t)row_dirty & 255) == 0, PNX_ERR_INVALID, "row_dirty must be 256-byte aligned (pnx_conv3x3_row_dirty_bytes: flags, then written masks)");
+    const RowDirtyWs rw = row_dirty_carve(row_dirty, (int64_t)batch * ho * ((wo + 31) / 32));
+    rd.flag = rw.flag, rd.written = rw.written;
+  }
+  const ConvArgs a = {(const uint16_t*)x, (const uint4*)wfrag, bias, (const uint16_t*)residual, mask, (uint16_t*)y, batch, h, w, relu, rd, tile_list,
                       tile_count, st};
   if (stride == 1 && getenv("PNX_CONV_DIRECT") == nullptr) {
     static const int pc_mode = getenv("PNX_CONV_PC") != nullptr ? atoi(getenv("PNX_CONV_PC")) : 1;
@@ -345,9 +358,9 @@
     if (cin == 64 && cout == 448) return launch_lds<448>(a);
   }
   if (stride == 2 && residual == nullptr && getenv("PNX_CONV_DIRECT") == nullptr) {
-    if (cin == 64 && cout == 128) return launch_s2<64, 128, 1>(x, wfrag, bias, mask, y, batch, h, w, ho, wo, relu, row_dirty, st);
-    if (cin == 128 && cout == 256) return launch_s2<128, 256, 1>(x, wfrag, bias, mask, y, batch, h, w, ho, wo, relu, row_dirty, st);
-    if (cin == 256 && cout == 256) return launch_s2<256, 256, 1>(x, wfrag, bias, mask, y, batch, h, w, ho, wo, relu, row_dirty, st);
+    if (cin == 64 && cout == 128) return launch_s2<64, 128, 1>(x, wfrag, bias, mask, y, batch, h, w, ho, wo, relu, rd, st);
+    if (cin == 128 && cout == 256) return launch_s2<128, 256, 1>(x, wfrag, bias, mask, y, batch, h, w, ho, wo, relu, rd, st);
+    if (cin == 256 && cout == 256) return launch_s2<256, 256, 1>(x, wfrag, bias, mask, y, batch, h, w, ho, wo, relu, rd, st);
   }
 #define PNX_CONV_CASE(CI, CO)                             \
   if (cin == CI && cout == CO) {                          \
@@ -394,9 +407,9 @@
     if (cin == 256 && cout == 256) return launch_pc_f32<256, 256, NP>(x, wfrag, bias, mask, y, batch, h, w, st);
   } else {
     const int ho = (h - 1) / 2 + 1, wo = (w - 1) / 2 + 1;
-    if (cin == 64 && cout == 128) return launch_s2<64, 128, NP>(x, wfrag, bias, mask, y, batch, h, w, ho, wo, 0, nullptr, st);
-    if (cin == 128 && cout == 256) return launch_s2<128, 256, NP>(x, wfrag, bias, mask, y, batch, h, w, ho, wo, 0, nullptr, st);
-    if (cin == 256 && cout == 256) return launch_s2<256, 256, NP>(x, wfrag, bias, mask, y, batch, h, w, ho, wo, 0, nullptr, st);
+    if (cin == 64 && cout == 128) return launch_s2<64, 128, NP>(x, wfrag, bias, mask, y, batch, h, w, ho, wo, 0, RowDirty{nullptr, nullptr, 1}, st);
+    if (cin == 128 && cout == 256) return launch_s2<128, 256, NP>(x, wfrag, bias, mask, y, batch, h, w, ho, wo, 0, RowDirty{nullptr, nullptr, 1}, st);
+    if (cin == 256 && cout == 256) return launch_s2<256, 256, NP>(x, wfrag, bias, mask, y, batch, h, w, ho, wo, 0, RowDirty{nullptr, nullptr, 1}, st);
   }
   pnx_set_error("%s: no kernel for %d -> %d channels, stride %d", name, cin, cout, stride);
   return PNX_ERR_UNSUPPORTED;
diff --git a/pillarnext_amd/csrc/conv_pc.h b/pillarnext_amd/csrc/conv_pc.h
--- a/pillarnext_amd/csrc/conv_pc.h
+++ b/pillarnext_amd/csrc/conv_pc.h
@@ -190,7 +190,7 @@
 __global__ __launch_bounds__(768, 3) void k_conv3x3_pc(const uint16_t* __restrict__ x, const uint16_t* __restrict__ x2, const uint4* __restrict__ wfrag,
                                                        const uint4* __restrict__ wfrag2, const float* __restrict__ bias,
                                                        const uint16_t* __restrict__ res, const uint8_t* __restrict__ mask, uint16_t* __restrict__ y,
-                                                       int B, int H, int W, int relu, uint8_t* __restrict__ row_dirty, int slot,
+                                                       int B, int H, int W, int relu, RowDirty row_dirty, int slot,
                                                        const int32_t* __restrict__ tlist, const int32_t* __restrict__ tcount,
                                                        const uint16_t* __restrict__ x3 = nullptr, const uint4* __restrict__ wfrag3 = nullptr) {
   constexpr bool X3 = NP == 2, F32 = NP > 1;
@@ -233,11 +233,11 @@
       return tile_at(tlist, idx, n_tiles);
     };
     uint32_t mb[TH / 2];
-    uint32_t dirty = 0;
+    uint32_t wrt = 0;
     auto load_meta = [&](int64_t t) {
 #pragma unroll
       for (int k = 0; k < TH / 2; k++) mb[k] = 0;
-      dirty = 0;
+      wrt = 0;
       if (t < 0) return;
       const int tx = (int)(t % tiles_x), ty = (int)((t / tiles_x) % tiles_y), b = (int)(t / ((int64_t)tiles_x * tiles_y));
       const int ox = tx * 32 + (lane & 31);
@@ -247,7 +247,7 @@
         if (ox < W && oy < H) mb[k] = mask != nullptr ? (uint32_t)mask[((int64_t)b * H + oy) * W + ox] : 1u;
       }
       const int oy2 = ty * TH + lane;
-      if (lane < TH && oy2 < H) dirty = row_dirty != nullptr ? (uint32_t)row_dirty[((int64_t)b * H + oy2) * tiles_x + tx] : 1u;
+      if (lane < TH && oy2 < H) wrt = rd_load(row_dirty, ((int64_t)b * H + oy2) * tiles_x + tx);
     };
 
     int n = 0, f = 0, nf = 0, g = 0;
@@ -281,7 +281,8 @@
         if (lane == 2 * k + 1) my_rm = hi;
         am |= (lo != 0 ? 1u : 0u) << (2 * k) | (hi != 0 ? 1u : 0u) << (2 * k + 1);
       }
-      const uint32_t was = (uint32_t)__ballot(dirty != 0) & ((1u << TH) - 1u);
+      const uint32_t was = (uint32_t)__ballot(wrt != 0) & ((1u << TH) - 1u);
+      const uint32_t my_wr = wrt;
       if (pw == 0) {
         if (lane < TH) s_rowmask[n & 3][lane] = my_rm;
         if (lane == 0) s_tile[n & 3] = make_int4(cb, cy0, cx0, (int)(am | (uint32_t)n_px << 16));
@@ -297,31 +298,33 @@
       if (slot >= 0 && pw == 0 && lane == 0) s_tick[(n + 3) & 3] = atomicAdd(&g_tile_ctr[slot][0], 1u);
       t_next = tile_index(n + 1);
       load_meta(t_next);
+      const uint32_t cols = W - cx0 >= 32 ? 0xffffffffu : (1u << (W - cx0)) - 1u;
+      const uint32_t my_stale = rd_held(row_dirty, my_wr) & ~my_rm & cols;
 #pragma unroll 1
       for (int r = pw; r < TH; r += 4) {
         const int oy = cy0 + r;
         if (oy >= H) break;
         const bool active = (am >> r) & 1u, w = (was >> r) & 1u;
-        if (!active && w) {
+        if (!PACK && !active && w) {
           char* dst = reinterpret_cast<char*>(y + (((int64_t)cb * H + oy) * W + cx0) * COUT * YS);
           const int nbytes = (W - cx0 < 32 ? W - cx0 : 32) * COUT * 2 * YS;
 #pragma unroll 1
           for (int o = lane * 16; o < nbytes; o += 1024) *reinterpret_cast<uint4*>(dst + o) = make_uint4(0, 0, 0, 0);
         }
         if constexpr (PACK) {
-          if (active && w) {
-            const uint32_t cols = W - cx0 >= 32 ? 0xffffffffu : (1u << (W - cx0)) - 1u;
-            const uint32_t idle = ~(uint32_t)__builtin_amdgcn_readlane((int)my_rm, r) & cols;
+          const uint32_t stale = (uint32_t)__builtin_amdgcn_readlane((int)my_stale, r);
+          if (stale != 0) {
             char* dst = reinterpret_cast<char*>(y + (((int64_t)cb * H + oy) * W + cx0) * COUT);
 #pragma unroll 1
             for (int c0 = 0; c0 < 32; c0 += 8) {
-              if (((idle >> c0) & 255u) == 0) continue;
+              if (((stale >> c0) & 255u) == 0) continue;
               const int p = c0 + (lane >> 3);
-              if ((idle >> p) & 1u) *reinterpret_cast<uint4*>(dst + p * (COUT * 2) + (lane & 7) * 16) = make_uint4(0, 0, 0, 0);
+              if ((stale >> p) & 1u) *reinterpret_cast<uint4*>(dst + p * (COUT * 2) + (lane & 7) * 16) = make_uint4(0, 0, 0, 0);
             }
           }
         }
-        if (row_dirty != nullptr && lane == 0 && w != active) row_dirty[((int64_t)cb * H + oy) * tiles_x + tx] = active ? 1 : 0;
+        const uint32_t wr_r = (uint32_t)__builtin_amdgcn_readlane((int)my_wr, r), rm_r = (uint32_t)__builtin_amdgcn_readlane((int)my_rm, r);
+        if (lane == 0) rd_store(row_dirty, ((int64_t)cb * H + oy) * tiles_x + tx, wr_r, rm_r);
       }
       nf = am != 0 ? NFILL : 1;
       f = 0;
@@ -498,7 +501,7 @@
   if (nb > 256) nb = 256;
   const int slot = mask != nullptr ? next_sched_slot() : -1;
   k_conv3x3_pc<CIN, COUT, false, NP><<<(unsigned)nb, 768, 0, st>>>((const uint16_t*)x.hi, (const uint16_t*)x.slot2(), (const uint4*)w.hi, (const uint4*)w.slot2(),
-                                                                   bias, nullptr, mask, (uint16_t*)y, B, H, W, 0, nullptr, slot, nullptr, nullptr,
+                                                                   bias, nullptr, mask, (uint16_t*)y, B, H, W, 0, RowDirty{nullptr, nullptr, 1}, slot, nullptr, nullptr,
                                                                    (const uint16_t*)x.slot3(), (const uint4*)w.slot3());
   PNX_LAUNCH_CHECK();
   return PNX_OK;
diff --git a/pillarnext_amd/csrc/conv_rows.h b/pillarnext_amd/csrc/conv_rows.h
--- a/pillarnext_amd/csrc/conv_rows.h
+++ b/pillarnext_amd/csrc/conv_rows.h
@@ -46,7 +46,7 @@
 __global__ __launch_bounds__(256, 2) void k_conv3x3_lds(const uint16_t* __restrict__ x, const uint4* __restrict__ wfrag,
                                                      const float* __restrict__ bias, const uint16_t* __restrict__ res,
                                                      const uint8_t* __restrict__ mask, uint16_t* __restrict__ y, int B, int H, int W,
-                                                     int relu, uint8_t* __restrict__ row_dirty, int slot, const int32_t* __restrict__ tlist,
+                                                     int relu, RowDirty row_dirty, int slot, const int32_t* __restrict__ tlist,
                                                       const int32_t* __restrict__ tcount) {
   constexpr int CIN = 64;
   constexpr int TH = LDS_TH, HW_ = LDS_HW;
@@ -60,7 +60,7 @@
   const int64_t n_tiles = tlist != nullptr ? (int64_t)__builtin_amdgcn_readfirstlane(*tcount) : (int64_t)B * tiles_y * tiles_x;
   auto load_mask = [&](int64_t t, bool (&a)[4], int (&wz)[4]) {
 #pragma unroll
-    for (int j = 0; j < 4; j++) a[j] = false, wz[j] = 1;
+    for (int j = 0; j < 4; j++) a[j] = false, wz[j] = -1;
     if (t < 0) return;
     const int tx = (int)(t % tiles_x);
     const int ty = (int)((t / tiles_x) % tiles_y);
@@ -70,7 +70,7 @@
     for (int j = 0; j < 4; j++) {
       const int oy = ty * TH + wv * 4 + j;
       a[j] = ox < W && oy < H && (mask == nullptr || mask[((int64_t)b * H + oy) * W + ox] != 0);
-      if (row_dirty != nullptr && oy < H) wz[j] = (int)row_dirty[((int64_t)b * H + oy) * tiles_x + tx];
+      if (oy < H) wz[j] = (int)rd_load(row_dirty, ((int64_t)b * H + oy) * tiles_x + tx);
     }
   };
   int64_t idxB = (int64_t)blockIdx.x + gridDim.x, idxC = 0;
@@ -79,7 +79,7 @@
   int wasP[4], wasN[4];
   load_mask(tileA, aP, wasP);
 #pragma unroll
-  for (int j = 0; j < 4; j++) aN[j] = false, wasN[j] = 1;
+  for (int j = 0; j < 4; j++) aN[j] = false, wasN[j] = -1;
   CT_DECL
   int it = 0;
   for (; tileA >= 0; tileA = tileB, tileB = tileC, idxB = idxC, it++) {
@@ -92,12 +92,12 @@
     const int x0 = tx * 32, y0 = ty * TH;
     const int ox = x0 + px;
     CT_TOCK(7)
-    bool was[4];
+    uint32_t was[4], bal[4];
 #pragma unroll
     for (int j = 0; j < 4; j++) {
-      was[j] = __builtin_amdgcn_readfirstlane(wasP[j]) != 0;
-      const uint32_t bal = (uint32_t)__ballot(aP[j]);
-      if (lane == 0) s_rowmask[wv * 4 + j] = bal;
+      was[j] = (uint32_t)__builtin_amdgcn_readfirstlane(wasP[j]);
+      bal[j] = (uint32_t)__ballot(aP[j]);
+      if (lane == 0) s_rowmask[wv * 4 + j] = bal[j];
     }
     __syncthreads();
     idxC = sched_next2(s_next, it, slot, idxB);
@@ -112,12 +112,12 @@
     for (int j = 0; j < 4; j++) {
       const int rr = wv * 4 + j, oy = y0 + rr;
       const bool active = (am >> rr) & 1u;
-      if (!active && was[j] && oy < H && ox < W) {
+      if (!active && ((rd_held(row_dirty, was[j]) >> px) & 1u) && oy < H && ox < W) {
         uint4* dst = reinterpret_cast<uint4*>(y + (((int64_t)b * H + oy) * W + ox) * COUT);
 #pragma unroll 1
         for (int ch = kb; ch < COUT / 8; ch += 2) dst[ch] = make_uint4(0, 0, 0, 0);
       }
-      if (row_dirty != nullptr && oy < H && lane == 0 && was[j] != active) row_dirty[((int64_t)b * H + oy) * tiles_x + tx] = active ? 1 : 0;
+      if (oy < H && lane == 0) rd_store(row_dirty, ((int64_t)b * H + oy) * tiles_x + tx, was[j], bal[j]);
     }
     if (am == 0) continue;
     int nr = 0;
@@ -315,7 +315,7 @@
 __global__ __launch_bounds__(256, 2) void k_conv3x3_ldsx(const uint16_t* __restrict__ x, const uint4* __restrict__ wfrag,
                                                       const float* __restrict__ bias, const uint16_t* __restrict__ res,
                                                       const uint8_t* __restrict__ mask, uint16_t* __restrict__ y, int B, int H, int W,
-                                                      int relu, uint8_t* __restrict__ row_dirty, int slot, const int32_t* __restrict__ tlist,
+                                                      int relu, RowDirty row_dirty, int slot, const int32_t* __restrict__ tlist,
                                                       const int32_t* __restrict__ tcount) {
   static_assert(CIN % 64 == 0 && (COUT % 128 == 0 || COUT == 64), "64-channel input slabs, 128-channel output passes (or one of 64)");
   constexpr int TH = L128_TH, HW_ = LDS_HW;
@@ -340,7 +340,7 @@
   };
   auto load_mask = [&](int t, bool (&a)[2], int (&wz)[2]) {
 #pragma unroll
-    for (int j = 0; j < 2; j++) a[j] = false, wz[j] = 1;
+    for (int j = 0; j < 2; j++) a[j] = false, wz[j] = -1;
     if (t < 0) return;
     const int tx = (int)(t % tiles_x);
     const int ty = (int)((t / tiles_x) % tiles_y);
@@ -350,7 +350,7 @@
     for (int j = 0; j < 2; j++) {
       const int oy = ty * TH + wv * 2 + j;
       a[j] = ox < W && oy < H && (mask == nullptr || mask[((int64_t)b * H + oy) * W + ox] != 0);
-      if (row_dirty != nullptr && oy < H) wz[j] = (int)row_dirty[((int64_t)b * H + oy) * tiles_x + tx];
+      if (oy < H) wz[j] = (int)rd_load(row_dirty, ((int64_t)b * H + oy) * tiles_x + tx);
     }
   };
   int64_t idxB = (int64_t)blockIdx.x + gridDim.x, idxC = 0;
@@ -359,7 +359,7 @@
   int wasP[2], wasN[2];
   load_mask(tileA >= 0 ? tileA / NH : -1, aP, wasP);
 #pragma unroll
-  for (int j = 0; j < 2; j++) aN[j] = false, wasN[j] = 1;
+  for (int j = 0; j < 2; j++) aN[j] = false, wasN[j] = -1;
   int it = 0;
   for (; tileA >= 0; tileA = tileB, tileB = tileC, idxB = idxC, it++) {
     const int unit = __builtin_amdgcn_readfirstlane(tileA);
@@ -372,11 +372,10 @@
     const int b = (int)(tile / ((int64_t)tiles_x * tiles_y));
     const int x0 = tx * 32, y0 = ty * TH;
     const int ox = x0 + px;
-    bool was[2];
-    uint32_t bal[2];
+    uint32_t was[2], bal[2];
 #pragma unroll
     for (int j = 0; j < 2; j++) {
-      was[j] = __builtin_amdgcn_readfirstlane(wasP[j]) != 0;
+      was[j] = (uint32_t)__builtin_amdgcn_readfirstlane(wasP[j]);
       bal[j] = (uint32_t)__ballot(aP[j]);
       if (lane == 0) s_rowmask[wv * 2 + j] = bal[j];
     }
@@ -393,12 +392,12 @@
       const int rr = wv * 2 + j, oy = y0 + rr;
       const bool active = (am >> rr) & 1u;
       if (hsel != 0) continue;
-      if (!active && was[j] && oy < H && ox < W) {
+      if (!active && ((rd_held(row_dirty, was[j]) >> px) & 1u) && oy < H && ox < W) {
         uint4* dst = reinterpret_cast<uint4*>(y + (((int64_t)b * H + oy) * W + ox) * COUT);
 #pragma unroll 1
         for (int ch = kb; ch < COUT / 8; ch += 2) dst[ch] = make_uint4(0, 0, 0, 0);
       }
-      if (row_dirty != nullptr && oy < H && lane == 0 && was[j] != active) row_dirty[((int64_t)b * H + oy) * tiles_x + tx] = active ? 1 : 0;
+      if (oy < H && lane == 0) rd_store(row_dirty, ((int64_t)b * H + oy) * tiles_x + tx, was[j], bal[j]);
     }
     if (am == 0) continue;
     if constexpr (PACK) {
@@ -437,20 +436,24 @@
         default: PNX_PIX_X(4); break;
       }
 #undef PNX_PIX_X
+      if (hsel != 0) continue;
       int l = lane;
       asm volatile("" : "+v"(l));
       const uint32_t cols = W - x0 >= 32 ? 0xffffffffu : (1u << (W - x0)) - 1u;
 #pragma unroll
       for (int j = 0; j < 2; j++) {
         const int rr = wvu * 2 + j;
-        const uint32_t idle = ~bal[j] & cols;
-        if (!((am >> rr) & 1u) || !was[j] || y0 + rr >= H || idle == 0) continue;
-        char* const row = reinterpret_cast<char*>(y + t0) + (uint32_t)(rr * W * COUT * 2 + hsel * 256);
+        const uint32_t stale = rd_held(row_dirty, was[j]) & ~bal[j] & cols;
+        if (!((am >> rr) & 1u) || y0 + rr >= H || stale == 0) continue;
+        char* const row = reinterpret_cast<char*>(y + t0) + (uint32_t)(rr * W * COUT * 2);
 #pragma unroll 1
         for (int c0 = 0; c0 < 32; c0 += 4) {
-          if (((idle >> c0) & 15u) == 0) continue;
+          if (((stale >> c0) & 15u) == 0) continue;
           const int p = c0 + (l >> 4);
-          if ((idle >> p) & 1u) *reinterpret_cast<uint4*>(row + (uint32_t)(p * COUT * 2 + (l & 15) * 16)) = make_uint4(0, 0, 0, 0);
+          if ((stale >> p) & 1u) {
+#pragma unroll
+            for (int h = 0; h < NH; h++) *reinterpret_cast<uint4*>(row + (uint32_t)(p * COUT * 2 + h * 256 + (l & 15) * 16)) = make_uint4(0, 0, 0, 0);
+          }
         }
       }
       continue;
diff --git a/pillarnext_amd/csrc/conv_s2.h b/pillarnext_amd/csrc/conv_s2.h
--- a/pillarnext_amd/csrc/conv_s2.h
+++ b/pillarnext_amd/csrc/conv_s2.h
@@ -120,7 +120,7 @@
 __global__ __launch_bounds__(256, 2) void k_conv3x3_s2(const uint16_t* __restrict__ x, const uint16_t* __restrict__ x2, const uint4* __restrict__ wfrag,
                                                     const uint4* __restrict__ wfrag2, const float* __restrict__ bias,
                                                     const uint8_t* __restrict__ mask, uint16_t* __restrict__ y, int B, int H, int W, int Ho, int Wo,
-                                                    int relu, uint8_t* __restrict__ row_dirty, int slot, const uint16_t* __restrict__ x3 = nullptr,
+                                                    int relu, RowDirty row_dirty, int slot, const uint16_t* __restrict__ x3 = nullptr,
                                                     const uint4* __restrict__ wfrag3 = nullptr) {
   static_assert(CIN % 64 == 0 && (COUT == 128 || COUT == 256), "64-channel input slabs; 4 groups of 32 or of 64 output channels");
   constexpr int TH = S2_TH, MB = COUT / 128, NCG = 4, NRG = 1, NRMAX = TH / NRG;
@@ -144,12 +144,12 @@
     const int b = (int)(tile / ((int64_t)tiles_x * tiles_y));
     const int x0 = tx * 32, y0 = ty * TH;
     const int ox = x0 + px;
-    bool was = true;
+    uint32_t was = 0xffffffffu, bal;
     {
       const int oy = y0 + wv;
       const bool a = ox < Wo && oy < Ho && (mask == nullptr || mask[((int64_t)b * Ho + oy) * Wo + ox] != 0);
-      if (row_dirty != nullptr && oy < Ho) was = __builtin_amdgcn_readfirstlane((int)row_dirty[((int64_t)b * Ho + oy) * tiles_x + tx]) != 0;
-      const uint32_t bal = (uint32_t)__ballot(a);
+      if (oy < Ho) was = (uint32_t)__builtin_amdgcn_readfirstlane((int)rd_load(row_dirty, ((int64_t)b * Ho + oy) * tiles_x + tx));
+      bal = (uint32_t)__ballot(a);
       if (lane == 0) s_rowmask[wv] = bal;
     }
     __syncthreads();
@@ -159,12 +159,12 @@
     {
       const int oy = y0 + wv;
       const bool active = (am >> wv) & 1u;
-      if (!active && was && oy < Ho && ox < Wo) {
+      if (!active && ((rd_held(row_dirty, was) >> px) & 1u) && oy < Ho && ox < Wo) {
         uint4* dst = reinterpret_cast<uint4*>(y + (((int64_t)b * Ho + oy) * Wo + ox) * COUT * YS);
 #pragma unroll 1
         for (int ch = kb; ch < COUT * YS / 8; ch += 2) dst[ch] = make_uint4(0, 0, 0, 0);
       }
-      if (row_dirty != nullptr && oy < Ho && lane == 0 && was != active) row_dirty[((int64_t)b * Ho + oy) * tiles_x + tx] = active ? 1 : 0;
+      if (oy < Ho && lane == 0) rd_store(row_dirty, ((int64_t)b * Ho + oy) * tiles_x + tx, was, bal);
     }
     if (am == 0) continue;
     int nr = 0;
@@ -212,7 +212,7 @@
 
 template <int CIN, int COUT, int NP>
 int launch_s2(PnxPieces<NP> x, PnxPieces<NP> wfrag, const float* bias, const uint8_t* mask, void* y, int B, int H, int W, int Ho, int Wo, int relu,
-              uint8_t* row_dirty, hipStream_t st) {
+              RowDirty row_dirty, hipStream_t st) {
   const int slot = mask != nullptr ? next_sched_slot() : -1;
   int64_t nb = (int64_t)B * ((Ho + S2_TH - 1) / S2_TH) * ((Wo + 31) / 32);
   if (nb > 512) nb = 512;
diff --git a/pillarnext_amd/csrc/conv_tile.h b/pillarnext_amd/csrc/conv_tile.h
--- a/pillarnext_amd/csrc/conv_tile.h
+++ b/pillarnext_amd/csrc/conv_tile.h
@@ -174,6 +174,32 @@
     }
 }
 
+struct RowDirtyWs {
+  uint8_t* flag;
+  uint32_t* written;
+  size_t bytes;
+};
+inline RowDirtyWs row_dirty_carve(void* base, int64_t n_seg) {
+  RowDirtyWs w;
+  PnxCarver c(base);
+  w.flag = c.take<uint8_t>((size_t)n_seg);
+  w.written = c.take<uint32_t>((size_t)n_seg);
+  w.bytes = c.used();
+  return w;
+}
+struct RowDirty {
+  uint8_t* flag;
+  uint32_t* written;
+  int stale;
+};
+__device__ __forceinline__ uint32_t rd_load(const RowDirty& rd, int64_t i) { return rd.written != nullptr ? rd.written[i] : 0xffffffffu; }
+__device__ __forceinline__ uint32_t rd_held(const RowDirty& rd, uint32_t w) { return rd.stale != 0 || w == 0 ? w : 0xffffffffu; }
+__device__ __forceinline__ void rd_store(const RowDirty& rd, int64_t i, uint32_t was, uint32_t now) {
+  if (rd.written == nullptr) return;
+  if ((was != 0) != (now != 0)) rd.flag[i] = now != 0 ? 1 : 0;
+  if (was != now) rd.written[i] = now;
+}
+
 struct ConvArgs {
   const uint16_t* x;
   const uint4* wfrag;
@@ -182,7 +208,7 @@
   const uint8_t* mask;
   uint16_t* y;
   int B, H, W, relu;
-  uint8_t* row_dirty;
+  RowDirty row_dirty;
   const int32_t *tlist, *tcount;
   hipStream_t st;
 };
diff --git a/pillarnext_amd/ops.py b/pillarnext_amd/ops.py
--- a/pillarnext_amd/ops.py
+++ b/pillarnext_amd/ops.py
@@ -733,7 +733,28 @@
 
 def conv3x3_workspace(batch, cout, ho, wo, device, dtype=torch.bfloat16):
     y = torch.zeros((batch, cout, ho, wo), dtype=dtype, device=device).contiguous(memory_format=torch.channels_last)
-    return y, torch.zeros((batch, ho, (wo + 31) // 32), dtype=torch.uint8, device=device)
+    segs = (wo + 31) // 32
+    arr = torch.zeros((row_dirty_bytes(batch, ho, wo),), dtype=torch.uint8, device=device)
+    return y, arr[: batch * ho * segs].view(batch, ho, segs)
+
+
+def row_dirty_bytes(batch, ho, wo):
+    return int(lib().pnx_conv3x3_row_dirty_bytes(batch, ho, wo))
+
+
+def _row_dirty_check(flags, batch, ho, wo):
+    need = row_dirty_bytes(batch, ho, wo)
+    if (flags.dtype != torch.uint8 or tuple(flags.shape) != (batch, ho, (wo + 31) // 32) or not flags.is_contiguous()
+            or flags.untyped_storage().nbytes() - flags.storage_offset() < need):
+        raise PnxError(f"conv3x3: row_dirty must be the flags of conv3x3_workspace ({need} bytes: flags + written masks)")
+
+
+def row_dirty_written(flags, wo):
+    B, ho, segs = flags.shape
+    _row_dirty_check(flags, B, ho, wo)
+    off = (B * ho * segs + 255) // 256 * 256
+    whole = torch.empty(0, dtype=torch.uint8, device=flags.device).set_(flags.untyped_storage(), flags.storage_offset(), (row_dirty_bytes(B, ho, wo),))
+    return whole[off: off + 4 * B * ho * segs].view(torch.int32).view(B, ho, segs)
 
 
 def conv_tile_rows(cin, cout, stride=1):
@@ -775,6 +796,8 @@
 def conv3x3_masked(x, wfrag, bias, cout, stride=1, mask=None, residual=None, relu=True, out=None, tiles=None):
     B, H, W, ci, _, Ho, Wo = _conv3x3_dims(x, wfrag, cout, stride, mask, residual, out, cuda=True)
     y, dirty = out if out is not None else (torch.empty((B, cout, Ho, Wo), dtype=x.dtype, device=x.device, memory_format=torch.channels_last), None)
+    if dirty is not None:
+        _row_dirty_check(dirty, B, Ho, Wo)
     tl, tc = tiles if tiles is not None else (None, None)
     check(_conv_fn("conv3x3", x.dtype)(ptr(x), ptr(wfrag), ptr(bias), ptr(residual), ptr(mask), ptr(y), B, H, W, ci, cout, stride, 1 if relu else 0,
                                        ptr(dirty), ptr(tl), ptr(tc), stream_ptr()), "pnx_conv3x3")
```

New measurement: 776.8, median of 6. 2.6% higher.
